# MasonMcGill/multipath-nn

Hardware: AMD Instinct MI355X
Metric: images/sec training CIFAR-10 actor-net (higher is better)
Workload: dtype f32; 1 GPU; cifar10-ac: ac_chain(k_cpt=0) 8-block actor-routed chain, 32x32x3, 10 classes; global_batch=128, per_gpu_batch=128, parallelism=dp1, rccl_ranks=1, hip_graph=True, steps_per_graph=4, streams=1, clock_warmup_steps=96

## Files before the change

include/mpnn_hip.h:

```cpp
#ifndef MPNN_HIP_H
#define MPNN_HIP_H

#ifdef __cplusplus
extern "C" {
#endif

#define MPNN_MAX_NODES 128
#define MPNN_MAX_SINKS 4

#define MPNN_E_SHAPE   (-1)
#define MPNN_E_ARG     (-2)

#define MPNN_BN_SLOTS 16

#define MPNN_ACT_IDENTITY 0
#define MPNN_ACT_BN_BATCH 1
#define MPNN_ACT_BN_MOVING 2
#define MPNN_ACT_RELU 3

typedef struct {
    const float  *x;
    const double *sum;
    const float  *gamma, *beta, *m_avg, *v_avg;
    float eps;
    int   cnt;
    int   C;
    int   shift;
    int   mode;
    int   nslot;
} mpnn_act;

int mpnn_bn_relu_fwd(const mpnn_act *a, float *y, long n_pix, void *stream);

int mpnn_pack_weights(const float *params, float *packs, const int *desc,
                      int n_desc, void *stream);

int mpnn_step_begin(const float *params, float *packs, const int *desc, int n_desc,
                    void *zero, long zero_bytes, void *stream);

typedef struct {
    mpnn_act a;
    const float *v;  int Cv;
    const float *wa_pack;  const float *wv_pack;
    const float *bias;
    float  *out;
    float  *pool_out;
    double *out_sum;
    int out_nslot;
    int n, H, W, Cout;
    const int *idx;
    const int *cnt;
} mpnn_conv_fwd_args;
int mpnn_msconv_fwd(const mpnn_conv_fwd_args *args, void *stream);
int mpnn_msconv_fwd_group(const mpnn_conv_fwd_args *args, const mpnn_conv_fwd_args *dev_args, int count,
                          void *stream);
int mpnn_msconv_fwd_group_rep(const mpnn_conv_fwd_args *args, const mpnn_conv_fwd_args *dev_args, int count,
                              int reps, int share, void *stream);

typedef struct {
    const float *s;
    mpnn_act bn;
    const double *red;
    int red_nslot;
} mpnn_bn_ctx;
int mpnn_bn_bwd_reduce(const float *dy, const mpnn_bn_ctx *ctx, float *dz,
                       double *red_out, long n_pix, void *stream);
int mpnn_bn_bwd_apply(float *dz_inout, const mpnn_bn_ctx *ctx, long n_pix,
                      void *stream);

typedef struct {
    const float *g;  int Cg;
    const mpnn_bn_ctx *g_ctx;
    const float *w_pack;
    const float *dy_extra;
    const mpnn_bn_ctx *prev;
    float  *out;
    double *red_out;
    int n, H, W, Cout;
    int accumulate;
} mpnn_dgrad_horz_args;
int mpnn_msconv_dgrad_horz(const mpnn_dgrad_horz_args *args, void *stream);

typedef struct {
    const float *g;  int Cg;
    const mpnn_bn_ctx *g_ctx;
    const float *w_pack;
    const mpnn_bn_ctx *fine;
    int fine_has_dz;
    float *dz_g_fine;
    int n, H, W, Cout;
} mpnn_dgrad_vert_args;
int mpnn_msconv_dgrad_vert(const mpnn_dgrad_vert_args *args, void *stream);
int mpnn_msconv_dgrad_pair(const mpnn_dgrad_horz_args *horz, const mpnn_dgrad_vert_args *vert,
                           void *stream);

typedef struct {
    mpnn_act a;
    const float *v;  int Cv;
    const float *g;
    const mpnn_bn_ctx *g_ctx;
    float *dwa;  float *dwv;  float *db;
    long split_stride;
    int n, H, W, Cout;
    int n_split;
} mpnn_wgrad_args;
int mpnn_msconv_wgrad(const mpnn_wgrad_args *args, void *stream);
int mpnn_msconv_bwd_scale(const mpnn_dgrad_horz_args *horz, const mpnn_dgrad_vert_args *vert,
                          const mpnn_wgrad_args *wgrad, void *stream);
#define MPNN_BWD_LEVEL_MAX 4
typedef struct {
    const mpnn_dgrad_horz_args *horz;
    const mpnn_dgrad_vert_args *vert;
    const mpnn_wgrad_args *wgrad;
    int wg_horz, wg_vert;
} mpnn_bwd_member;
int mpnn_msconv_bwd_level_record_size(void);
int mpnn_msconv_bwd_level_slots(const int *H, const int *W, const int *Cout, int count);
int mpnn_msconv_bwd_level_prepare(const mpnn_bwd_member *members, int count, void *host_records);
int mpnn_msconv_bwd_level(const mpnn_bwd_member *members, int count, const void *dev_records, void *stream);
int mpnn_msconv_bwd_level_prepare_rep(const mpnn_bwd_member *members, int count, int reps, void *host_records);
int mpnn_msconv_bwd_level_rep(const mpnn_bwd_member *members, int count, int reps, const void *dev_records, void *stream);
int mpnn_wgrad_tiles(int n, int H, int W);
#define MPNN_SLAB_ITEM 1024
int mpnn_slab_reduce(const float *slabs, float *grads, const int *table, int n_items,
                     void *stream);

int mpnn_msconv_gen_check(int H, int W, int Cin, int Cv, int Cout, int kh, int kw, int kvh, int kvw);
int mpnn_msconv_gen_tiles(int n, int H, int W);
int mpnn_msconv_fwd_gen(const mpnn_conv_fwd_args *args, int kh, int kw, int kvh, int kvw, void *stream);
int mpnn_msconv_dgrad_horz_gen(const mpnn_dgrad_horz_args *args, int kh, int kw, void *stream);
int mpnn_msconv_dgrad_vert_gen(const mpnn_dgrad_vert_args *args, int kvh, int kvw, void *stream);
int mpnn_msconv_wgrad_gen(const mpnn_wgrad_args *args, int kh, int kw, int kvh, int kvw, void *stream);

int mpnn_msconv_hw_check(int H, int W, int Cin, int Cv, int Cout, int kh, int kw, int kvh, int kvw);
int mpnn_msconv_hw_tiles(int n, int H, int W);
int mpnn_msconv_fwd_hw(const mpnn_conv_fwd_args *args, int kh, int kw, int kvh, int kvw, void *stream);
int mpnn_msconv_dgrad_horz_hw(const mpnn_dgrad_horz_args *args, int kh, int kw, void *stream);
int mpnn_msconv_dgrad_vert_hw(const mpnn_dgrad_vert_args *args, int kvh, int kvw, void *stream);
int mpnn_msconv_wgrad_hw(const mpnn_wgrad_args *args, int kh, int kw, int kvh, int kvw, void *stream);

int mpnn_msconv_ch_check(int H, int W, int Cin, int Cv, int Cout, int kh, int kw, int kvh, int kvw);
int mpnn_msconv_fwd_ch(const mpnn_conv_fwd_args *args, int kh, int kw, int kvh, int kvw, void *stream);
int mpnn_msconv_dgrad_horz_ch(const mpnn_dgrad_horz_args *args, int kh, int kw, void *stream);
int mpnn_msconv_dgrad_vert_ch(const mpnn_dgrad_vert_args *args, int kvh, int kvw, void *stream);
int mpnn_msconv_wgrad_ch(const mpnn_wgrad_args *args, int kh, int kw, int kvh, int kvw, void *stream);

typedef struct {
    mpnn_act a;  const float *w;  const float *bias;  float *out;
    int n, H, W, Cout;  int supp;
} mpnn_conv_nhwc_fwd_args;
int mpnn_conv_nhwc_fwd(const mpnn_conv_nhwc_fwd_args *args, void *stream);
typedef struct {
    const float *g;  int Cg;  const float *w;
    const float *relu_src;
    double *scratch;
    float *dx;
    int n, H, W, Cin;  int supp;
} mpnn_conv_nhwc_dgrad_args;
int mpnn_conv_nhwc_dgrad(const mpnn_conv_nhwc_dgrad_args *args, void *stream);
typedef struct {
    mpnn_act a;  const float *g;  float *dw;  float *db;
    long split_stride;  int n_split;
    int n, H, W, Cout;  int supp;
} mpnn_conv_nhwc_wgrad_args;
int mpnn_conv_nhwc_wgrad(const mpnn_conv_nhwc_wgrad_args *args, void *stream);

typedef struct {
    mpnn_act a;  int HW;
    const float *w[2];  const float *b[2];  float *y[2];  int M[2];
    const float *k_cpt;  float alpha_cpt;  int extra_col[2];
    int n;
    float *kpart;  int *kcnt;
} mpnn_lin_fwd_args;
#define MPNN_LIN_KSLICES 8
int mpnn_lin_fwd(const mpnn_lin_fwd_args *dev_table, int count, int n_max, void *stream);
int mpnn_lin_fwd_ks(const mpnn_lin_fwd_args *dev_table, int count, int n_max, int k_max, void *stream);

typedef struct {
    mpnn_act a;  int HW;
    const float *w[2];  const float *dy[2];  int M[2];
    float *dw[2];  float *db[2];
    float *dx;
    const float *k_cpt;  float alpha_cpt;  int extra_col[2];
    int n;
    float *dz_out;  double *red_out;  int red_nslot;
    float *kpart;  int *kcnt;
} mpnn_lin_bwd_args;
#define MPNN_LIN_RSPLIT 8
#define MPNN_LIN_RS_TILE 2080
int mpnn_lin_bwd(const mpnn_lin_bwd_args *dev_table, int count, int n_max, int k_max,
                 void *stream);
int mpnn_lin_bwd_rs(const mpnn_lin_bwd_args *dev_table, int count, int n_max, int k_max,
                    void *stream);

typedef struct {
    const float *z;  const float *y;  int n_cls;  float eps_ce;
    float *c_err;  float *d_cor;
    const float *h1;  int R;  int n_sinks;
    const float *g1, *b1;  float *m1, *v1;
    const float *w2, *bias2;
    const float *g2, *b2;  float *m2, *v2;
    const float *w3, *bias3;
    float *h2;  float *r;  int r_stride;
    float *bn_save;
    float bn_eps, bn_decay;
    int mode;
    int n;
    float *clear_f;  int n_clear_f;  double *clear_d;  int n_clear_d;
    int R2;
    const float *hyp_src;  float *hyp_dst;
    float bn_eps2, bn_decay2;
} mpnn_exit_tail_args;
int mpnn_exit_tail_fwd(const mpnn_exit_tail_args *dev_table, int count, int n_max,
                       void *stream);

typedef struct {
    mpnn_exit_tail_args f;
    const float *w_cerr;
    const float *dr;
    float *dz;
    float *dh1;
    float *dg1, *db1, *dw2, *dbias2, *dg2, *db2, *dw3, *dbias3;
    float *dh2;
} mpnn_exit_tail_bwd_args;
int mpnn_exit_tail_bwd(const mpnn_exit_tail_bwd_args *dev_table, int count, int n_max,
                       void *stream);

typedef struct {
    mpnn_act a;  int HW;
    const float *w_head, *b_head;  int n_cls;
    const float *y;  float eps_ce;  float *c_err, *d_cor;
    const float *w1, *b1;  int R;  int n_sinks;
    int extra_col;  const float *k_cpt;  float alpha_cpt;
    const float *g1, *be1, *m1, *v1;  const float *w2, *bias2;
    const float *g2, *be2, *m2, *v2;  const float *w3, *bias3;
    float bn_eps;
    float *r;  int r_stride;
    const int *idx;  const int *cnt;  int n;
    int *child_idx[MPNN_MAX_SINKS];  int *child_cnt[MPNN_MAX_SINKS];
    int R2;
    float *z, *h1;
    float bn_eps2;
    int *cls;  float *conf;
    float *p_cls;  int p_stride;
} mpnn_exit_ev_args;
int mpnn_exit_ev(const mpnn_exit_ev_args *dev_table, int count, int n_max, void *stream);
int mpnn_exit_ev_check(const mpnn_exit_ev_args *host_record);

#define MPNN_PREFIX_MAX 64
typedef struct {
    int n, count, n_front, pad_;
    int parent[MPNN_PREFIX_MAX], parent_sink[MPNN_PREFIX_MAX], n_sinks[MPNN_PREFIX_MAX], r_stride[MPNN_PREFIX_MAX];
    float *r[MPNN_PREFIX_MAX];
    float *c_err[MPNN_PREFIX_MAX];
    float *d_cor[MPNN_PREFIX_MAX];
    int front_parent[MPNN_PREFIX_MAX], front_sink[MPNN_PREFIX_MAX];
    int *front_idx[MPNN_PREFIX_MAX];
    int *front_cnt[MPNN_PREFIX_MAX];
} mpnn_ev_prefix_args;
int mpnn_ev_prefix_walk(const mpnn_ev_prefix_args *host_rec, const mpnn_ev_prefix_args *dev_rec, void *stream);

typedef struct {
    int n, n_nodes, n_leaves, n_cls;
    const float *p_ev;
    const long long *node_ops;
    const int *leaf_node;
    const int *leaf_cls;  const float *leaf_conf;
    const float *leaf_p;
    int leaf_stride, p_stride;
// ... 112 lines not shown
```

multipath-nn_amd/csrc/bwd_bodies.h:

```cpp
#pragma once
#include "conv_kernel.h"

struct WgP {
    ConvP c;
    const float *g;
    const float *g_s;  mpnn_act g_bn;  const double *g_red;  int g_nslot;  int g_on;
    float *dwa, *dwv, *db;
    long split_stride;
    int n_tiles;
};

template <int GK> struct WGeom;
template <> struct WGeom<0> { static constexpr int PS = 113; };
template <> struct WGeom<1> { static constexpr int PS = 113; };
template <> struct WGeom<2> { static constexpr int PS = 145; };

template <int GK, int OT, int PART, bool SMALLC = false>
__device__ __forceinline__ void wgrad_body(const WgP &p, f32x4 *tile, float *gt, float *cA,
                                           const int bx, const int by, const int bz, const int gx) {
    static_assert(!SMALLC || (PART == 0 && OT == 1), "SMALLC: the image chunk of a 16-channel group");
    using G = Geom<GK>;
    constexpr int PS = WGeom<GK>::PS, R = G::R, HR = G::TH + 2;
    constexpr int GS = OT * 16 + 4;
    constexpr int XN = XItems<GK>::N;
    const ConvP &c = p.c;
    const int tid = threadIdx.x, lane = tid & 63;
    const int wid = __builtin_amdgcn_readfirstlane(tid >> 6);
    const int g = lane >> 4, li = lane & 15;
    const int nchA = (c.a.C + 15) >> 4;
    constexpr int part = PART;
    const int ch = part ? by - nchA : by;
    const int C = part ? c.Cv : c.a.C;
    const int co0 = bz * OT * 16;
    int np = (C - ch * 16 + 3) >> 2;
    np = np > 4 ? 4 : np;
    const bool bias_wave = wid == 1 && by == 0;
    const bool xa = c.xcd != 0 && (c.n & 31) == 0 && (gx & 7) == 0;
    const int xcd_id = blockIdx.x & 7;
    const int tpi = GK == 0 ? (c.W >> 4) * (c.H >> 2) : 1;
    const int sq0 = xa ? (bx >> 3) : bx, sqd = xa ? (gx >> 3) : gx, sqn = xa ? (p.n_tiles >> 3) : p.n_tiles;
    trace_stamp(0);

    constexpr bool NINE = OT == 1 || OT == 4;
    f32x4 acc[NINE ? 1 : 3][OT];
    f32x4 acc9[(NINE && !SMALLC) ? 9 : 1];
    [[maybe_unused]] f32x4 accS[2] = {f32x4{0.f, 0.f, 0.f, 0.f}, f32x4{0.f, 0.f, 0.f, 0.f}};
    [[maybe_unused]] int offS[2];
    [[maybe_unused]] bool onS[2];
    if constexpr (SMALLC) {
#pragma unroll
        for (int nt = 0; nt < 2; ++nt) {
            const int idx = nt * 16 + li, n9 = 9 * c.a.C;
            onS[nt] = idx < n9;
            const int ic = onS[nt] ? idx : 0, tap = ic / c.a.C, cc = ic - tap * c.a.C;
            offS[nt] = ((tap / 3) * R + (tap % 3)) * 4 + cc;
        }
    }
    float bsum = 0.f;
#pragma unroll
    for (int ti = 0; ti < (NINE ? 1 : 3); ++ti)
#pragma unroll
        for (int nt = 0; nt < OT; ++nt) acc[ti][nt] = f32x4{0.f, 0.f, 0.f, 0.f};
#pragma unroll
    for (int tap = 0; tap < ((NINE && !SMALLC) ? 9 : 1); ++tap) acc9[tap] = f32x4{0.f, 0.f, 0.f, 0.f};
    const float *tf = (const float *)tile;
    const int a_lane = (li >> 2) * PS * 4 + (li & 3);
    const float one_hot = li == 0 ? 1.f : 0.f;
    int tap_off[3];
#pragma unroll
    for (int ti = 0; ti < 3; ++ti) {
        const int tap = min(wid + 4 * ti, 8);
        tap_off[ti] = (tap / 3) * R + (tap % 3);
    }

    [[maybe_unused]] int slot9[4];
#pragma unroll
    for (int j = 0; j < 4; ++j) {
        int img, ty, tx;
        mtile_pix<GK>(wid, 4 * g + j, img, ty, tx);
        slot9[j] = (img * HR + ty) * R + tx;
    }

    if (part == 0 && c.a.mode != MPNN_ACT_IDENTITY) {
        for (int cc = tid; cc < c.a.C; cc += 256) {
            const BnC k = bn_coef(c.a, cc);
            cA[cc * 3] = k.m; cA[cc * 3 + 1] = k.gamma * k.rstd; cA[cc * 3 + 2] = k.beta;
        }
    }

    float *cG = cA + 128 * 3;
    if (p.g_on && p.g_bn.mode == MPNN_ACT_BN_BATCH) {
        for (int cc = tid - 128; cc >= 0 && cc < OT * 16; cc += 256) bn_bwd_row(p.g_bn, p.g_red, p.g_nslot, co0 + cc, false, cG + cc * 5);
    } else if (p.g_on) {
        const double inv = 1.0 / (double)p.g_bn.cnt;
        for (int cc = tid - 128; cc >= 0 && cc < OT * 16; cc += 256) {
            const int co = co0 + cc;
            const BnC k = bn_coef(p.g_bn, co);
            float *e = cG + cc * 5;
            e[0] = k.m; e[1] = k.rstd; e[2] = k.gamma * k.rstd;
            double r0, r1;
            slot_sum2(p.g_red, 2 * c.Cout, co, c.Cout + co, p.g_nslot, r0, r1);
            e[3] = (float)(r0 * inv); e[4] = (float)(r1 * inv);
        }
    }

    if constexpr (XItems<GK>::INTERIOR) zero_halo(tile, 4 * PS, tid, 256);
    __syncthreads();
    trace_stamp(1);
    f32x4 xr[XN][1], gr[OT], gs[OT];
    int on0;
    unsigned inbS;
    ItemK<GK> ik;
    item_consts<GK, PS>(ik, tid);
    int g_geo[OT], g_lds[OT], g_c4[OT];
#pragma unroll
    for (int k = 0; k < OT; ++k) {
        const int i = tid + k * 256;
        const int q = i % (OT * 4), pi = i / (OT * 4);
        int img, ty, tx;
        mtile_pix<GK>(pi >> 4, pi & 15, img, ty, tx);
        g_geo[k] = (img << 16) | (ty << 8) | tx;
        g_lds[k] = pi * GS + q * 4;
        g_c4[k] = q * 4;
    }
    const int xc = ch * 16 + ik.q * 4;
    const bool xq_in = ik.q < np;
    const int sh = PART == 0 ? c.a.shift : 0;
    const int xC = PART == 0 ? c.a.C : c.Cv;
    const float *const xsrc = PART == 0 ? c.a.x : c.v;
    auto request = [&](int t) {
        int n0, y0, x0;
        tile_origin<GK>(c, xa ? xcd_tile<GK>(t, xcd_id, tpi) : t, n0, y0, x0);
        on0 = n0;
        unsigned inb = 0;
#pragma unroll
        for (int k = 0; k < XN; ++k) {
            const int n = n0 + (ik.geo[k] >> 16), y = y0 + ((ik.geo[k] >> 8) & 255) - 1, x = x0 + (ik.geo[k] & 255) - 1;
            const bool ok = ((ik.ok >> k) & 1) && xq_in && n < c.n &&
                            (XItems<GK>::INTERIOR || ((unsigned)y < (unsigned)c.H && (unsigned)x < (unsigned)c.W));
            inb |= (ok ? 1u : 0u) << k;
            const unsigned pix = ok ? (((unsigned)n * (c.H << sh) + (y << sh)) * (c.W << sh) + (x << sh)) * xC : 0u;
            if (PART == 1 || (xC & 3) == 0) {
                xr[k][0] = *(const f32x4 *)((const char *)xsrc + (pix + (ok ? xc : 0)) * 4u);
            } else {
#pragma unroll
                for (int j = 0; j < 4; ++j) xr[k][0][j] = xsrc[pix + (ok && xc + j < xC ? xc + j : 0)];
            }
        }
        inbS = inb;
#pragma unroll
        for (int k = 0; k < OT; ++k) {
            const int n = n0 + (g_geo[k] >> 16);
            const bool live = n < c.n;
            const unsigned off = live ? (((unsigned)n * c.H + y0 + ((g_geo[k] >> 8) & 255)) * c.W + x0 + (g_geo[k] & 255)) * c.Cout + co0 + g_c4[k] : 0u;
            gr[k] = *(const f32x4 *)((const char *)p.g + off * 4u);
            if (p.g_on) gs[k] = *(const f32x4 *)((const char *)p.g_s + off * 4u);
        }
    };
    auto tile_step = [&](int t) {
        const int o_n0 = on0;
        const unsigned inb = inbS;
        lds_barrier();
#pragma unroll
        for (int k = 0; k < XN; ++k) {
            const bool live = (inb >> k) & 1;
            f32x4 v = xr[k][0];
            if (PART == 0) {
                if (c.a.mode != MPNN_ACT_IDENTITY) {
#pragma unroll
                    for (int j = 0; j < 4; ++j) {
                        const float *cc = cA + (xc + j) * 3;
                        const float tv = fmaxf((v[j] - cc[0]) * cc[1] + cc[2], 0.f);
                        v[j] = (xc + j < xC) ? tv : 0.f;
                    }
                } else if (xC & 3) {
#pragma unroll
                    for (int j = 0; j < 4; ++j) v[j] = (xc + j < xC) ? v[j] : 0.f;
                }
            }
#pragma unroll
            for (int j = 0; j < 4; ++j) v[j] = live ? v[j] : 0.f;
            if ((ik.ok >> k) & 1) tile[ik.slot[k]] = v;
        }
#pragma unroll
        for (int k = 0; k < OT; ++k) {
            f32x4 v = {0.f, 0.f, 0.f, 0.f};
            if (o_n0 + (g_geo[k] >> 16) < c.n) {
                v = gr[k];
                if (p.g_on) {
#pragma unroll
// ... 2 lines not shown
                        const float xh = (gs[k][j] - e[0]) * e[1];
                        v[j] = e[2] * (v[j] - e[3] - xh * e[4]);
                    }
                }
            }
            *(f32x4 *)(gt + g_lds[k]) = v;
        }
        lds_barrier();
        if (t == sq0) trace_stamp(2);
        if (t + sqd < sqn) request(t + sqd);
        if constexpr (SMALLC) {
            float gq[4], xq[4][2];
#pragma unroll
            for (int j = 0; j < 4; ++j) {
                gq[j] = gt[(wid * 16 + 4 * g + j) * GS + li];
#pragma unroll
                for (int nt = 0; nt < 2; ++nt) xq[j][nt] = tf[slot9[j] * 4 + offS[nt]];
            }
#pragma unroll
            for (int j = 0; j < 4; ++j) {
                bsum += gq[j];
#pragma unroll
                for (int nt = 0; nt < 2; ++nt)
                    accS[nt] = __builtin_amdgcn_mfma_f32_16x16x4f32(gq[j], onS[nt] ? xq[j][nt] : 0.f, accS[nt], 0, 0, 0);
            }
        } else
        if constexpr (NINE) {
#pragma unroll
            for (int kk = 0; kk < (OT == 4 ? 4 : 1); ++kk) {
                const int kc = OT == 4 ? kk : wid;
                float bq[4], aq[4][9];
                if constexpr (OT == 4) {
#pragma unroll
                    for (int j = 0; j < 4; ++j) {
                        int img, ty, tx;
                        mtile_pix<GK>(kk, 4 * g + j, img, ty, tx);
                        const int slot = (img * HR + ty) * R + tx;
                        bq[j] = gt[(kk * 16 + 4 * g + j) * GS + wid * 16 + li];
#pragma unroll
                        for (int tap = 0; tap < 9; ++tap) aq[j][tap] = tf[(slot + (tap / 3) * R + (tap % 3)) * 4 + a_lane];
                    }
                } else {
#pragma unroll
                    for (int j = 0; j < 4; ++j) {
                        bq[j] = gt[(kc * 16 + 4 * g + j) * GS + li];
#pragma unroll
                        for (int tap = 0; tap < 9; ++tap) aq[j][tap] = tf[(slot9[j] + (tap / 3) * R + (tap % 3)) * 4 + a_lane];
                    }
                }
#pragma unroll
                for (int j = 0; j < 4; ++j) {
                    bsum += bq[j];
#pragma unroll
                    for (int tap = 0; tap < 9; ++tap)
                        acc9[tap] = __builtin_amdgcn_mfma_f32_16x16x4f32(aq[j][tap], bq[j], acc9[tap], 0, 0, 0);
                }
            }
        } else {
#pragma unroll
        for (int kc = 0; kc < 4; ++kc) {
            float bq[4][OT], aq[4][3];
#pragma unroll
            for (int j = 0; j < 4; ++j) {
                int img, ty, tx;
                mtile_pix<GK>(kc, 4 * g + j, img, ty, tx);
                const int slot = (img * HR + ty) * R + tx;
#pragma unroll
                for (int nt = 0; nt < OT; ++nt) bq[j][nt] = gt[(kc * 16 + 4 * g + j) * GS + nt * 16 + li];
#pragma unroll
                for (int ti = 0; ti < 3; ++ti) aq[j][ti] = tf[(slot + tap_off[ti]) * 4 + a_lane];
                if (bias_wave) aq[j][2] = one_hot;
            }
#pragma unroll
            for (int j = 0; j < 4; ++j)
#pragma unroll
                for (int ti = 0; ti < 3; ++ti)
#pragma unroll
                    for (int nt = 0; nt < OT; ++nt)
                        acc[ti][nt] = __builtin_amdgcn_mfma_f32_16x16x4f32(aq[j][ti], bq[j][nt], acc[ti][nt], 0, 0, 0);
        }
        }
    };
    if (sq0 < sqn) request(sq0);
    for (int t = sq0; t < sqn; t += sqd) tile_step(t);

    trace_stamp(4);
    mfma_drain();
    const size_t soff = (size_t)bx * p.split_stride;
    float *dw = (part ? p.dwv : p.dwa) + soff;
    if constexpr (NINE && OT == 4) {
#pragma unroll
        for (int tap = 0; tap < 9; ++tap)
#pragma unroll
            for (int r = 0; r < 4; ++r) {
                const int cin = ch * 16 + g * 4 + r;
                if (cin < C) dw[((size_t)tap * C + cin) * c.Cout + co0 + wid * 16 + li] = acc9[tap][r];
            }
        if (by == 0) {
            float b = bsum;
            b += __shfl_xor(b, 16);
            b += __shfl_xor(b, 32);
            if (g == 0) p.db[soff + co0 + wid * 16 + li] = b;
        }
    } else if constexpr (SMALLC) {
        f32x4 *part4 = tile;
        float *partf = (float *)tile;
        lds_barrier();
#pragma unroll
        for (int nt = 0; nt < 2; ++nt) part4[(wid * 2 + nt) * 64 + lane] = accS[nt];
        lds_barrier();
        {
            const int r = wid, n9 = 9 * C;
#pragma unroll
            for (int nt = 0; nt < 2; ++nt) {
                float v = 0.f;
#pragma unroll
                for (int w = 0; w < 4; ++w) v += partf[((w * 2 + nt) * 64 + lane) * 4 + r];
                const int idx = nt * 16 + li, co = 4 * g + r;
                if (idx < n9) dw[(size_t)idx * c.Cout + co0 + co] = v;
            }
        }
        if (by == 0) {
            float b = bsum;
            b += __shfl_xor(b, 16);
            b += __shfl_xor(b, 32);
            lds_barrier();
            if (g == 0) partf[wid * 16 + li] = b;
            lds_barrier();
            if (tid < 16) p.db[soff + co0 + tid] = (partf[tid] + partf[16 + tid]) + (partf[32 + tid] + partf[48 + tid]);
        }
    } else if constexpr (NINE) {
        f32x4 *part4 = tile;
        float *partf = (float *)tile;
        const int cl = (tid >> 4) & 15, tl = tid >> 8;
        (void)tl;
#pragma unroll
        for (int rd = 0; rd < 3; ++rd) {
            lds_barrier();
#pragma unroll
            for (int q = 0; q < 3; ++q) part4[(wid * 3 + q) * 64 + lane] = acc9[rd * 3 + q];
            lds_barrier();
            const int cin = ch * 16 + cl;
#pragma unroll
            for (int q = 0; q < 3; ++q) {
                float v = 0.f;
#pragma unroll
                for (int w = 0; w < 4; ++w) v += partf[((w * 3 + q) * 64 + (cl >> 2) * 16 + li) * 4 + (cl & 3)];
                if (cin < C) dw[((size_t)(rd * 3 + q) * C + cin) * c.Cout + co0 + li] = v;
            }
        }
        if (by == 0) {
            float b = bsum;
            b += __shfl_xor(b, 16);
            b += __shfl_xor(b, 32);
            lds_barrier();
            if (g == 0) partf[wid * 16 + li] = b;
            lds_barrier();
            if (tid < 16) p.db[soff + co0 + tid] = (partf[tid] + partf[16 + tid]) + (partf[32 + tid] + partf[48 + tid]);
        }
    } else {
#pragma unroll
    for (int ti = 0; ti < 3; ++ti) {
        const int tap = wid + 4 * ti;
        if (tap >= 9) continue;
#pragma unroll
        for (int r = 0; r < 4; ++r) {
// ... 25 lines not shown
```

multipath-nn_amd/csrc/common.h:

```cpp
#pragma once
#include <hip/hip_runtime.h>
#include <cstdlib>
#include "mpnn_hip.h"

typedef float f32x4 __attribute__((ext_vector_type(4)));

constexpr int MPNN_OCC = 4;

#define MPNN_LAUNCH_CHECK() do { hipError_t e_ = hipGetLastError(); \
    if (e_ != hipSuccess) return (int)e_; } while (0)

extern int mpnn_reserved_cus_g;

static int resident_slots(const void *kernel, int dyn_lds, int threads = 256, int max_per_cu = 0) {
    struct Entry { const void *fn; int lds, per_cu, cus, cap; };
    static Entry cache[64];
    static int n_cached = 0;
    int per_cu = 0, cus = 256;
    bool hit = false;
    for (int i = 0; i < n_cached && !hit; ++i)
        if (cache[i].fn == kernel && cache[i].lds == dyn_lds && cache[i].cap == max_per_cu) {
            per_cu = cache[i].per_cu; cus = cache[i].cus; hit = true;
        }
    if (!hit) {
// ... 3 lines not shown
        hipFuncAttributes fa;
        if (hipFuncGetAttributes(&fa, kernel) == hipSuccess) {
            const size_t lds = fa.sharedSizeBytes + (size_t)dyn_lds;
            if (lds > 0) {
                const int by_lds = (int)((160u * 1024u) / ((lds + 1279) / 1280 * 1280));
                if (by_lds >= 1 && by_lds < per_cu) per_cu = by_lds;
            }
        }
        if (hipGetDevice(&dev) == hipSuccess) {
            int v = 0;
            if (hipDeviceGetAttribute(&v, hipDeviceAttributeMultiprocessorCount, dev) == hipSuccess && v > 0) cus = v;
        }
        if (max_per_cu > 0 && per_cu > max_per_cu) per_cu = max_per_cu;
        if (n_cached < 64) cache[n_cached++] = Entry{kernel, dyn_lds, per_cu, cus, max_per_cu};
    }
    const int free_cus = cus - mpnn_reserved_cus_g;
    return per_cu * (free_cus < 8 ? 8 : free_cus);
}

#define MPNN_TRACE_SLOTS 12
#ifdef MPNN_TRACE
static __device__ unsigned long long *mpnn_trace_buf_ = nullptr;
__device__ __forceinline__ void trace_stamp(int k) {
    unsigned long long *b = mpnn_trace_buf_;
    if (b && threadIdx.x == 0)
        b[(size_t)((blockIdx.z * gridDim.y + blockIdx.y) * gridDim.x + blockIdx.x) * MPNN_TRACE_SLOTS + k] = __builtin_amdgcn_s_memrealtime();
}
__device__ __forceinline__ void trace_note(int k, unsigned long long v) {
    unsigned long long *b = mpnn_trace_buf_;
    if (b && threadIdx.x == 0) b[(size_t)((blockIdx.z * gridDim.y + blockIdx.y) * gridDim.x + blockIdx.x) * MPNN_TRACE_SLOTS + k] = v;
}
static inline int mpnn_trace_install(void *buf) {
    return (int)hipMemcpyToSymbol(HIP_SYMBOL(mpnn_trace_buf_), &buf, sizeof(buf));
}
#else
__device__ __forceinline__ void trace_stamp(int) {}
__device__ __forceinline__ void trace_note(int, unsigned long long) {}
static inline int mpnn_trace_install(void *) { return MPNN_E_ARG; }
#endif

struct BnC { float m, rstd, gamma, beta; };

__device__ __forceinline__ double ld_slot(const double *base, int C2, int s, unsigned off) {
    const char *row = (const char *)(base + (size_t)s * C2);
    return *(const double *)(row + off);
}
__device__ __forceinline__ void slot_sum2(const double *base, int C2, int i0, int i1, int nslot, double &a, double &b) {
    double t0 = 0.0, t1 = 0.0;
    const unsigned o0 = (unsigned)i0 * 8u, o1 = (unsigned)i1 * 8u;
#pragma unroll 8
    for (int s = 0; s < nslot; ++s) { t0 += ld_slot(base, C2, s, o0); t1 += ld_slot(base, C2, s, o1); }
    a = t0; b = t1;
}
__device__ __forceinline__ double slot_sum(const double *base, int C2, int idx, int nslot) {
    double t = 0.0;
    const unsigned o = (unsigned)idx * 8u;
#pragma unroll 8
    for (int s = 0; s < nslot; ++s) t += ld_slot(base, C2, s, o);
    return t;
}

__device__ __forceinline__ BnC bn_coef(const mpnn_act &b, int c) {
    BnC k;
    k.gamma = b.mode == MPNN_ACT_RELU ? 1.f : b.gamma[c];
    k.beta = b.mode == MPNN_ACT_RELU ? 0.f : b.beta[c];
    if (b.mode == MPNN_ACT_BN_BATCH) {
        const double inv = 1.0 / (double)b.cnt;
        double s1, s2;
        slot_sum2(b.sum, 2 * b.C, c, b.C + c, b.nslot, s1, s2);
        const double mean = s1 * inv;
        double var = s2 * inv - mean * mean;
        var = var < 0.0 ? 0.0 : var;
        k.m = (float)mean;
        k.rstd = rsqrtf((float)var + b.eps);
    } else if (b.mode == MPNN_ACT_RELU) {
        k.m = 0.f;  k.rstd = 1.f;  k.gamma = 1.f;  k.beta = 0.f;
    } else {
        k.m = b.m_avg[c];
        k.rstd = rsqrtf(b.v_avg[c] + b.eps);
    }
    return k;
}

__device__ __forceinline__ void bn_bwd_row(const mpnn_act &b, const double *red, int red_nslot, int c, bool want_beta, float *e) {
    const int C2 = 2 * b.C, ns = b.nslot, rn = red ? red_nslot : 0;
    const float gamma = b.gamma[c], beta = b.beta[c];
    const unsigned o0 = (unsigned)c * 8u, o1 = (unsigned)(b.C + c) * 8u;
    double s1 = 0.0, s2 = 0.0, r0 = 0.0, r1 = 0.0;
    if (ns == 8 && (rn == 8 || rn == 0)) {
        double a0[8], a1[8], q0[8], q1[8];
#pragma unroll
        for (int s = 0; s < 8; ++s) { a0[s] = ld_slot(b.sum, C2, s, o0); a1[s] = ld_slot(b.sum, C2, s, o1); }
        if (rn) {
#pragma unroll
            for (int s = 0; s < 8; ++s) { q0[s] = ld_slot(red, C2, s, o0); q1[s] = ld_slot(red, C2, s, o1); }
        } else {
#pragma unroll
            for (int s = 0; s < 8; ++s) { q0[s] = 0.0; q1[s] = 0.0; }
        }
#pragma unroll
        for (int s = 0; s < 8; ++s) { s1 += a0[s]; s2 += a1[s]; }
        if (rn) {
#pragma unroll
            for (int s = 0; s < 8; ++s) { r0 += q0[s]; r1 += q1[s]; }
        }
    } else {
        slot_sum2(b.sum, C2, c, b.C + c, ns, s1, s2);
        if (rn) slot_sum2(red, C2, c, b.C + c, rn, r0, r1);
    }
    const double inv = 1.0 / (double)b.cnt;
    const double mean = s1 * inv;
    double var = s2 * inv - mean * mean;
    var = var < 0.0 ? 0.0 : var;
    const float rstd = rsqrtf((float)var + b.eps);
    e[0] = (float)mean; e[1] = rstd; e[2] = gamma * rstd;
    if (want_beta) { e[3] = beta; e[4] = 0.f; }
    else { e[3] = (float)(r0 * inv); e[4] = (float)(r1 * inv); }
}

struct BnNoHook { __device__ __forceinline__ void operator()(int, float, int, float) const {} };
template <class F = BnNoHook>
__device__ __forceinline__ void bn_finalize_body(double *__restrict__ sums, double *__restrict__ reds,
                                                 float *__restrict__ state, float *__restrict__ grads,
                                                 const int *__restrict__ t, float decay, int n_img,
                                                 double *__restrict__ sums_keep, F on_grad = F()) {
    const int C = t[3], ns = t[7];
    const double inv = 1.0 / ((double)t[4] * (double)n_img);
    for (int c = threadIdx.x; c < C; c += blockDim.x) {
        const double mean = slot_sum(sums + t[0], 2 * C, c, ns) * inv;
        double var = slot_sum(sums + t[0], 2 * C, C + c, ns) * inv - mean * mean;
        var = var < 0.0 ? 0.0 : var;
        if (t[5] >= 0) {
            float *m = state + t[1] + c, *v = state + t[2] + c;
            *m = decay * *m + (1.f - decay) * (float)mean;
            *v = decay * *v + (1.f - decay) * (float)var;
        }
        if (reds && grads && t[5] >= 0) {
            const float dbeta = (float)slot_sum(reds + t[0], 2 * C, c, ns);
            const float dgamma = (float)slot_sum(reds + t[0], 2 * C, C + c, ns);
            grads[t[6] + c] = dbeta;
            grads[t[5] + c] = dgamma;
            on_grad(t[6] + c, dbeta, t[5] + c, dgamma);
        }
        if (!sums_keep) continue;
        for (int s = 0; s < ns; ++s) {
            const int i0 = t[0] + s * 2 * C + c, i1 = i0 + C;
            sums_keep[i0] = sums[i0];  sums_keep[i1] = sums[i1];
            sums[i0] = 0.0;  sums[i1] = 0.0;
            if (reds) { reds[i0] = 0.0;  reds[i1] = 0.0; }
        }
    }
}

__device__ __forceinline__ void lds_barrier() {
    asm volatile("" ::: "memory");
    __builtin_amdgcn_s_waitcnt(0xC07F);
    __builtin_amdgcn_s_barrier();
    asm volatile("" ::: "memory");
}

__device__ __forceinline__ void mfma_drain() {
    __builtin_amdgcn_sched_barrier(0);
    asm volatile("s_nop 15" ::: "memory");
    __builtin_amdgcn_sched_barrier(0);
}

// ... 49 lines not shown
```

multipath-nn_amd/csrc/conv_dgrad.hip:

```cpp
#include "conv_kernel.h"

static int fill_g_ctx(const mpnn_bn_ctx *c, ConvP &p) {
    if (!c) return 0;
    if (!c->s || !c->red) return MPNN_E_ARG;
    p.ga_on = 1;  p.ga_s = c->s;  p.ga_bn = c->bn;  p.ga_red = c->red;
    p.ga_nslot = c->red_nslot < 1 ? 1 : c->red_nslot;
    return 0;
}

int mpnn_fill_dgrad_horz(const mpnn_dgrad_horz_args *a, ConvP &p) {
    if (!a || !a->g || !a->w_pack || !a->out) return MPNN_E_ARG;
    p.a.x = a->g;  p.a.C = a->Cg;  p.a.mode = MPNN_ACT_IDENTITY;  p.a.shift = 0;
    p.wa = a->w_pack;
    p.n = a->n;  p.H = a->H;  p.W = a->W;  p.Cout = a->Cout;
    p.extra = a->dy_extra;  p.out = a->out;  p.acc_out = a->accumulate ? 1 : 0;
    if (a->prev) {
        if (!a->prev->s || !a->red_out) return MPNN_E_ARG;
        p.sprev = a->prev->s;  p.pbn = a->prev->bn;  p.red_out = a->red_out;
        p.out_nslot = a->prev->red_nslot < 1 ? 1 : a->prev->red_nslot;
    }
    return fill_g_ctx(a->g_ctx, p);
}

int mpnn_fill_dgrad_vert(const mpnn_dgrad_vert_args *a, ConvP &p) {
    if (!a || !a->g || !a->w_pack || !a->fine || !a->fine->s || !a->dz_g_fine) return MPNN_E_ARG;
    p.a.x = a->g;  p.a.C = a->Cg;  p.a.mode = MPNN_ACT_IDENTITY;  p.a.shift = 0;
    p.wa = a->w_pack;
    p.n = a->n;  p.H = a->H;  p.W = a->W;  p.Cout = a->Cout;
    p.out = a->dz_g_fine;  p.sprev = a->fine->s;  p.pbn = a->fine->bn;
    p.red = a->fine_has_dz ? a->fine->red : nullptr;  p.has_dz = a->fine_has_dz;
    p.red_nslot = a->fine->red_nslot < 1 ? 1 : a->fine->red_nslot;
    return fill_g_ctx(a->g_ctx, p);
}

int mpnn_trace_install_dgrad(void *buf) { return mpnn_trace_install(buf); }

extern "C" int mpnn_msconv_dgrad_pair(const mpnn_dgrad_horz_args *h, const mpnn_dgrad_vert_args *v, void *stream) {
    ConvP ph = {}, pv = {};
    int rc = mpnn_fill_dgrad_horz(h, ph);
    if (rc) return rc;
    rc = mpnn_fill_dgrad_vert(v, pv);
    if (rc) return rc;
    if (!h->prev) return MPNN_E_ARG;
    return conv_launch_pair<EPI_DGH_BN, EPI_DGV>(ph, pv, (hipStream_t)stream);
}

extern "C" int mpnn_msconv_dgrad_horz(const mpnn_dgrad_horz_args *a, void *stream) {
    ConvP p = {};
    const int rc = mpnn_fill_dgrad_horz(a, p);
    if (rc) return rc;
    if (a->prev) return conv_launch<EPI_DGH_BN>(p, (hipStream_t)stream);
    return conv_launch<EPI_DGH_RAW>(p, (hipStream_t)stream);
}

extern "C" int mpnn_msconv_dgrad_vert(const mpnn_dgrad_vert_args *a, void *stream) {
    ConvP p = {};
    const int rc = mpnn_fill_dgrad_vert(a, p);
    if (rc) return rc;
    return conv_launch<EPI_DGV>(p, (hipStream_t)stream);
}
```

multipath-nn_amd/csrc/conv_fwd.hip:

```cpp
#include "conv_kernel.h"
#include "conv_strip.h"

__host__ __device__ static inline int fill_fwd(const mpnn_conv_fwd_args *a, ConvP &p);

int mpnn_trace_install_fwd(void *buf) { return mpnn_trace_install(buf); }

extern "C" int mpnn_msconv_fwd(const mpnn_conv_fwd_args *a, void *stream) {
    ConvP p = {};
    const int rc = fill_fwd(a, p);
    if (rc) return rc;
    if (a->idx || a->cnt) return MPNN_E_ARG;
    return conv_launch<EPI_FWD>(p, (hipStream_t)stream);
}

struct FwdGroupP { int gk[4], small[4], gy[4], gx[4], y0[4], w0[4], rh[4]; int n; int xcd; int reps, wpr; };

__host__ __device__ static inline int fill_fwd(const mpnn_conv_fwd_args *a, ConvP &p) {
    if (!a || !a->a.x || !a->wa_pack || !a->out || !a->bias) return MPNN_E_ARG;
    if (a->v && !a->wv_pack) return MPNN_E_ARG;
    p.a = a->a;
    p.v = a->v;  p.Cv = a->v ? a->Cv : 0;
    p.wa = a->wa_pack;  p.wv = a->wv_pack;
    p.n = a->n;  p.H = a->H;  p.W = a->W;  p.Cout = a->Cout;
    p.bias = a->bias;  p.out = a->out;  p.out_sum = a->out_sum;  p.pool_out = a->pool_out;
    p.out_nslot = a->out_nslot < 1 ? 1 : (a->out_nslot > MPNN_BN_SLOTS ? MPNN_BN_SLOTS : a->out_nslot);
    if (a->pool_out && (a->H < 8 || (a->H & 1) || (a->W & 1))) return MPNN_E_SHAPE;
    p.idx = a->idx;
    if (a->idx && !a->cnt) return MPNN_E_ARG;
#if defined(__HIP_DEVICE_COMPILE__)
    if (a->cnt) { const int c = *a->cnt; p.n = c < a->n ? c : a->n; }
#endif
    return 0;
}

template <bool SMALL, bool IDX, bool WIDE = false>
__global__ __launch_bounds__(256, WIDE ? 2 : (SMALL ? 3 : MPNN_OCC)) void fwd_group_k(const mpnn_conv_fwd_args *__restrict__ tab, const FwdGroupP q) {
    extern __shared__ __attribute__((aligned(16))) char smem[];
    int id = blockIdx.x;
    if (q.reps > 1) { const int rep = id / q.wpr; id -= rep * q.wpr; tab += rep * q.n; }
    int m = 0, w0 = 0, gx = q.gx[0], kind = q.gk[0] * 2 + q.small[0];
#pragma unroll
    for (int k = 1; k < 4; ++k)
        if (k < q.n && id >= q.w0[k]) { m = k; w0 = q.w0[k]; gx = q.gx[k]; kind = q.gk[k] * 2 + q.small[k]; }
    const int yy = (id - w0) / gx, bx = (id - w0) - yy * gx;
    ConvP p = {};
    fill_fwd(tab + m, p);
    p.xcd = q.xcd;
    if constexpr (WIDE) {
        if (kind == 2) { p.n_tiles = conv_grid_x<1>(p.n, p.H, p.W); conv_body<1, 2, 1, 2, 2, false, EPI_FWD, 1, false, IDX>(p, bx, yy, gx, smem); }
        else           { p.n_tiles = conv_grid_x<2>(p.n, p.H, p.W); conv_body<2, 2, 1, 2, 2, false, EPI_FWD, 1, false, IDX>(p, bx, yy, gx, smem); }
        return;
    }
    switch (kind) {
        case 0: p.n_tiles = conv_grid_x<0>(p.n, p.H, p.W); conv_body<0, 1, 1, 4, 1, false, EPI_FWD, 1, false, IDX>(p, bx, yy, gx, smem); break;
        case 2: p.n_tiles = conv_grid_x<1>(p.n, p.H, p.W); conv_body<1, 1, 1, 4, 1, false, EPI_FWD, 1, false, IDX>(p, bx, yy, gx, smem); break;
        case 4: p.n_tiles = conv_grid_x<2>(p.n, p.H, p.W); conv_body<2, 1, 1, 4, 1, false, EPI_FWD, 1, false, IDX>(p, bx, yy, gx, smem); break;
        case 6: strip16_body<IDX>(tab[m], bx, yy, gx, q.rh[m], q.xcd, smem); break;
        case 8: stripk_body<IDX>(tab[m], bx, yy, gx, q.rh[m], q.xcd, smem); break;
        default:
            if constexpr (SMALL) {
                if (kind == 9)      stripk_body<IDX, true>(tab[m], bx, yy, gx, q.rh[m], q.xcd, smem);
                else if (kind == 1) { p.n_tiles = conv_grid_x<0>(p.n, p.H, p.W); conv_body<0, 1, 1, 4, 1, true, EPI_FWD, 1, false, IDX>(p, bx, yy, gx, smem); }
                else if (kind == 3) { p.n_tiles = conv_grid_x<1>(p.n, p.H, p.W); conv_body<1, 1, 1, 4, 1, true, EPI_FWD, 1, false, IDX>(p, bx, yy, gx, smem); }
                else                { p.n_tiles = conv_grid_x<2>(p.n, p.H, p.W); conv_body<2, 1, 1, 4, 1, true, EPI_FWD, 1, false, IDX>(p, bx, yy, gx, smem); }
            }
            break;
    }
}

template <int GK, int KS = 2>
__global__ __launch_bounds__(KS * 256) void fwd_ks_k(const mpnn_conv_fwd_args *__restrict__ tab, const int gx, const int xcd) {
    extern __shared__ __attribute__((aligned(16))) char smem[];
    const int id = blockIdx.x, yy = id / gx, bx = id - yy * gx;
    ConvP p = {};
    fill_fwd(tab, p);
    p.xcd = xcd;
    p.n_tiles = conv_grid_x<GK>(p.n, p.H, p.W);
    conv_body<GK, 1, 1, 4, 1, false, EPI_FWD, KS, true>(p, bx, yy, gx, smem);
}

int mpnn_first_conv_launch_rep(const mpnn_conv_fwd_args *a, const mpnn_conv_fwd_args *dev_args, int reps, int share, hipStream_t st);

static int fwd_group_launch(const mpnn_conv_fwd_args *args, const mpnn_conv_fwd_args *dev_args, int count, int reps, int share, void *stream);

extern "C" int mpnn_msconv_fwd_group(const mpnn_conv_fwd_args *args, const mpnn_conv_fwd_args *dev_args, int count,
                                     void *stream) {
    return fwd_group_launch(args, dev_args, count, 1, 1, stream);
}

extern "C" int mpnn_msconv_fwd_group_rep(const mpnn_conv_fwd_args *args, const mpnn_conv_fwd_args *dev_args, int count,
                                         int reps, int share, void *stream) {
    if (reps < 1) return MPNN_E_ARG;
    if (share <= 0) share = reps;
    if (count <= 0) return 0;
    if (!args || count > 4) return MPNN_E_ARG;
    for (int k = 0; k < count; ++k)
        if (args[k].idx || args[k].cnt) return MPNN_E_ARG;
    for (int r = 1; r < reps; ++r)
        for (int k = 0; k < count; ++k) {
            const mpnn_conv_fwd_args &a = args[k], &b = args[r * count + k];
            if (a.n != b.n || a.H != b.H || a.W != b.W || a.Cout != b.Cout || a.a.C != b.a.C || a.a.mode != b.a.mode ||
                a.a.shift != b.a.shift || (a.v != nullptr) != (b.v != nullptr) || a.Cv != b.Cv || a.out_nslot != b.out_nslot ||
                (a.pool_out != nullptr) != (b.pool_out != nullptr) || (a.out_sum != nullptr) != (b.out_sum != nullptr) ||
                a.idx || b.idx || a.cnt || b.cnt) return MPNN_E_ARG;
        }
    return fwd_group_launch(args, dev_args, count, reps, share, stream);
}

static int fwd_group_launch(const mpnn_conv_fwd_args *args, const mpnn_conv_fwd_args *dev_args, int count, int reps, int share, void *stream) {
    if (count <= 0) return 0;
// ... 109 lines not shown
```

multipath-nn_amd/csrc/conv_kernel.h:

```cpp
#pragma once
#include "common.h"
#include <cstdlib>

enum { EPI_FWD = 0, EPI_DGH_BN = 1, EPI_DGH_RAW = 2, EPI_DGV = 3 };

#ifdef MPNN_ABLATE
#define MPNN_DBG(p, bit) ((p).dbg & (bit))
#else
#define MPNN_DBG(p, bit) 0
#endif

struct ConvP {
    mpnn_act a;
    const float *v;  int Cv;
    const float *wa, *wv;
    int n, H, W, Cout;
    const float *bias;  float *out;  double *out_sum;
    float *pool_out;
    const float *extra;
    const float *sprev;  mpnn_act pbn;  double *red_out;
    const double *red;  int has_dz;  int red_nslot;
    int out_nslot;
    const float *ga_s;  mpnn_act ga_bn;  const double *ga_red;  int ga_nslot;  int ga_on;
    int n_tiles;
    int dbg;
    const int *idx;
    int acc_out;
    int xcd;
};

template <int GK>
__device__ __forceinline__ int xcd_tile(int j, int x, int tpi) {
    if (GK == 2) return 8 * j + x;
    const int ij = GK == 0 ? j / tpi : j, inner = GK == 0 ? j - ij * tpi : 0;
    const int n = ((ij >> 2) << 5) + 4 * x + (ij & 3);
    return n * tpi + inner;
}

template <int GK> struct Geom;
template <> struct Geom<0> { static constexpr int TH = 4, TW = 16, IMG = 1, R = 18, P = 112; };
template <> struct Geom<1> { static constexpr int TH = 8, TW = 8,  IMG = 1, R = 10, P = 112; };
template <> struct Geom<2> { static constexpr int TH = 4, TW = 4,  IMG = 4, R = 6,  P = 144; };

template <int GK>
__device__ __forceinline__ void mtile_pix(int m, int i, int &img, int &ty, int &tx) {
    if (GK == 0) { img = 0; ty = m; tx = i; }
    else if (GK == 1) { img = 0; ty = 2 * m + (i >> 3); tx = i & 7; }
    else { img = m; ty = i >> 2; tx = i & 3; }
}

template <int GK>
__device__ __forceinline__ void tile_origin(const ConvP &p, int bid, int &n0, int &y0, int &x0) {
    if (GK == 0) {
        const int tx_n = p.W >> 4, tpi = tx_n * (p.H >> 2);
        n0 = bid / tpi;
        const int rem = bid - n0 * tpi;
        const int ty = rem / tx_n;
        y0 = ty * 4; x0 = (rem - ty * tx_n) * 16;
    } else if (GK == 1) { n0 = bid; y0 = 0; x0 = 0; }
    else { n0 = bid * 4; y0 = 0; x0 = 0; }
}

template <int GK>
__host__ __device__ static inline int conv_grid_x(int n, int H, int W) {
    if (GK == 0) return n * (W >> 4) * (H >> 2);
    if (GK == 1) return n;
    return (n + 3) >> 2;
}

template <int GK> struct XItems {
    using G = Geom<GK>;
    static constexpr bool INTERIOR = GK != 0;
    static constexpr int HR = G::TH + 2, HC = G::TW + 2;
    static constexpr int NHP = INTERIOR ? G::IMG * G::TH * G::TW : G::IMG * HR * HC, NHP8 = (NHP + 7) & ~7;
    static constexpr int N = (NHP8 * 4 + 255) / 256;
};
__device__ __forceinline__ void zero_halo(f32x4 *lds, int count, int tid, int nthreads) {
    for (int i = tid; i < count; i += nthreads) lds[i] = f32x4{0.f, 0.f, 0.f, 0.f};
}
template <int GK, int PS>
__device__ __forceinline__ void zero_ring(f32x4 *lds, int planes, int tid, int nthreads) {
    using G = Geom<GK>;
    constexpr int HR = G::TH + 2, FR = G::IMG * HR * G::R;
    for (int i = tid; i < planes * PS; i += nthreads) {
        const int t = i % PS;
        bool ring = t >= FR;
        if (!ring) {
            const int r = t % (HR * G::R), hy = r / G::R, hx = r - hy * G::R;
            ring = hy == 0 || hy == HR - 1 || hx == 0 || hx > G::TW;
        }
        if (ring) lds[i] = f32x4{0.f, 0.f, 0.f, 0.f};
    }
}

__device__ __forceinline__ int sel_i(int flag, int a, int b) { const int m = -flag; return (a & ~m) | (b & m); }
__device__ __forceinline__ const float *sel_p(int flag, const float *a, const float *b) {
    const long delta = (const char *)b - (const char *)a;
    return (const float *)((const char *)a + (delta & -(long)flag));
}
template <int GK> struct ItemK {
    static constexpr int N = XItems<GK>::N;
    int slot[N];
    int geo[N];
    unsigned ok;
    int q;
};
template <int GK, int PS>
__device__ __forceinline__ void item_consts(ItemK<GK> &ik, int tid) {
    using X = XItems<GK>;
    using G = Geom<GK>;
    ik.ok = 0;
// ... 208 lines not shown
        r.np = (C - r.ch * 16 + 3) >> 2;
    };
    auto gen_tile = [&](UI &r, int t) {
        r.t = t; r.part = 0; r.ch = 0;
        tile_origin<GK>(p, xa ? xcd_tile<GK>(t, xcd_id, tpi) : t, r.n0, r.y0, r.x0);
        if constexpr (IDX) {
#pragma unroll
            for (int j = 0; j < G::IMG; ++j) r.im[j] = p.idx[r.n0 + j < p.n ? r.n0 + j : 0];
            tile_geo<GK, SMALL_A>(tgeo, ik, p, r.n0, r.y0, r.x0, r.im, aC, vC);
        } else
        tile_geo<GK, SMALL_A>(tgeo, ik, p, r.n0, r.y0, r.x0, nullptr, aC, vC);
        r.inb = tgeo.inb;
        set_np(r);
    };
    auto gen_next = [&](UI &r) {
        r.ch += NCH;
        if (r.ch >= (HAS_V ? sel_i(r.part, nchA, nchV) : nchA)) {
            if (HAS_V && !r.part && nchV) { r.part = 1; r.ch = 0; }
            else { gen_tile(r, r.t + sqd); return; }
        }
        set_np(r);
    };
    const bool b_once = upt == 1;
    constexpr int LK = EPI != EPI_FWD ? 2 : (SMALL_A ? 1 : 0);
    auto unit_load = [&](const UI &q, f32x4 (*xq)[XW], f32x4 *bq) {
        const float *src = HAS_V ? sel_p(q.part, aX, vX) : aX, *wp = HAS_V ? sel_p(q.part, wAp, wVp) : wAp;
        const int C = HAS_V ? sel_i(q.part, aC, vC) : aC;
#pragma unroll
        for (int sc = 0; sc < SC; ++sc) {
            const int cs = KSPLIT ? kg : sc;
            ld_items<GK, LK, XW, SMALL_A>(xq + sc * XN, p, tgeo, ik, q.part, (q.ch + cs) * 16, q.np - 4 * cs, src, C, odd_c);
        }
#pragma unroll
        for (int sc = 0; sc < SC; ++sc) {
            const int cs = KSPLIT ? kg : sc;
            const char *wb = (const char *)wp + (size_t)((q.ch + cs) * 16 * p.Cout) * 4;
#pragma unroll
            for (int k = 0; k < BN; ++k) bq[sc * BN + k] = *(const f32x4 *)(wb + ((HAS_V && q.part) ? wofV[k] : wofA[k]));
        }
    };
    auto unit_store = [&](const UI &q, f32x4 (*xq)[XW], f32x4 *bq, int buf, bool with_b) {
#pragma unroll
        for (int sc = 0; sc < SC; ++sc) {
            const int cs = KSPLIT ? kg : sc;
            f32x4 *td = tile[buf] + cs * 4 * P;
            f32x4 (*xs)[XW] = xq + sc * XN;
            const int c0 = (q.ch + cs) * 16, np = q.np - 4 * cs;
            bool done = false;
            if constexpr (EPI == EPI_FWD) {
                if (q.part) { done = true; st_items<GK, 1, XW>(td, xs, p, cA, q.inb, ik, c0, np); }
            }
            if constexpr (EPI != EPI_FWD) {
                if (p.ga_on) { done = true; st_items<GK, 2, XW>(td, xs, p, cA, q.inb, ik, c0, np); }
            }
            if (!done) st_items<GK, 0, XW>(td, xs, p, cA, q.inb, ik, c0, np);
        }
        if (with_b) {
            f32x4 *dst = wtile[(b_once || WtSingle<CT>::v) ? 0 : buf];
#pragma unroll
            for (int sc = 0; sc < SC; ++sc)
#pragma unroll
                for (int k = 0; k < BN; ++k) { const int i = tid + k * 256; if (i < BI) dst[(KSPLIT ? kg : sc) * BI + i] = bq[sc * BN + k]; }
        }
    };

    f32x4 xrA[SC * XN][XW], xrB[SC * XN][XW];
    f32x4 brA[SC * BN], brB[SC * BN];
    f32x4 acc[MT][NT];
    float s1[NT], s2[NT];
#pragma unroll
    for (int nt = 0; nt < NT; ++nt) { s1[nt] = 0.f; s2[nt] = 0.f; }
#pragma unroll
    for (int mt = 0; mt < MT; ++mt)
#pragma unroll
        for (int nt = 0; nt < NT; ++nt) acc[mt][nt] = f32x4{0.f, 0.f, 0.f, 0.f};

    UI cu = {}, n1 = {}, n2 = {};
    constexpr int TABQ = 8;
    [[maybe_unused]] double tabq[TABQ];
    [[maybe_unused]] float tab_g = 1.f, tab_b = 0.f;
    bool tab_late = false;
    if constexpr (EPI == EPI_FWD) {
        const int tot = p.a.nslot * 2 * p.a.C;
        tab_late = p.a.mode == MPNN_ACT_BN_BATCH && tot <= TABQ * 256 && p.a.C <= 256;
        if (tab_late) {
#pragma unroll
            for (int j = 0; j < TABQ; ++j) { const int k = tid + 256 * j; tabq[j] = p.a.sum[k < tot ? k : 0]; }
            const int c = tid < p.a.C ? tid : 0;
            tab_g = p.a.gamma[c]; tab_b = p.a.beta[c];
        }
    }
    if (EPI == EPI_FWD && p.a.mode != MPNN_ACT_IDENTITY && !tab_late) {
        for (int c = tid; c < p.a.C; c += 256) {
            const BnC k = bn_coef(p.a, c);
            cA[c * 3] = k.m; cA[c * 3 + 1] = k.gamma * k.rstd; cA[c * 3 + 2] = k.beta;
        }
    }
    if (EPI != EPI_FWD && p.ga_on) {
        if (p.ga_bn.mode == MPNN_ACT_BN_BATCH) {
            for (int c = tid; c < p.a.C; c += 256) bn_bwd_row(p.ga_bn, p.ga_red, p.ga_nslot, c, false, cA + c * 5);
        } else {
            const double inv = 1.0 / (double)p.ga_bn.cnt;
            for (int c = tid; c < p.a.C; c += 256) {
                const BnC k = bn_coef(p.ga_bn, c);
                float *e = cA + c * 5;
                e[0] = k.m; e[1] = k.rstd; e[2] = k.gamma * k.rstd;
                double r0, r1;
                slot_sum2(p.ga_red, 2 * p.a.C, c, p.a.C + c, p.ga_nslot, r0, r1);
                e[3] = (float)(r0 * inv); e[4] = (float)(r1 * inv);
            }
        }
    }
    if (EPI == EPI_DGH_BN || EPI == EPI_DGV) {
        for (int c = tid - 128; c >= 0 && c < CT; c += 256) {
            float *e = cE + c * 5;
            if (p.pbn.mode == MPNN_ACT_BN_BATCH) {
                bn_bwd_row(p.pbn, EPI == EPI_DGV ? p.red : nullptr, p.red_nslot, co0 + c, EPI == EPI_DGH_BN, e);
                continue;
            }
            const BnC k = bn_coef(p.pbn, co0 + c);
            e[0] = k.m; e[1] = k.rstd; e[2] = k.gamma * k.rstd;
            if (EPI == EPI_DGH_BN) { e[3] = k.beta; e[4] = 0.f; }
            else {
                const double inv = 1.0 / (double)p.pbn.cnt;
                double r0 = 0.0, r1 = 0.0;
                if (p.red) slot_sum2(p.red, 2 * p.pbn.C, co0 + c, p.pbn.C + co0 + c, p.red_nslot, r0, r1);
                e[3] = (float)(r0 * inv); e[4] = (float)(r1 * inv);
            }
        }
    }
    if (!tab_late) __syncthreads();
    trace_stamp(1);
    gen_tile(gen, sq0);
    cu = gen;
    unit_load(cu, xrA, brA);
    if (n_units > 1) {
        gen_next(gen);
        n1 = gen;
        unit_load(n1, xrB, brB);
    }
    if constexpr (EPI == EPI_FWD) {
        if (tab_late) {
            double *scr = (double *)smem;
            const int C = p.a.C, tot = p.a.nslot * 2 * C;
#pragma unroll
            for (int j = 0; j < TABQ; ++j) { const int k = tid + 256 * j; if (k < tot) scr[k] = tabq[j]; }
            __syncthreads();
            if (tid < C) {
                double s1 = 0.0, s2 = 0.0;
                for (int sl = 0; sl < p.a.nslot; ++sl) { s1 += scr[(2 * sl) * C + tid]; s2 += scr[(2 * sl + 1) * C + tid]; }
                const double inv = 1.0 / (double)p.a.cnt, mean = s1 * inv;
                double var = s2 * inv - mean * mean;
                var = var < 0.0 ? 0.0 : var;
                cA[tid * 3] = (float)mean; cA[tid * 3 + 1] = tab_g * rsqrtf((float)var + p.a.eps); cA[tid * 3 + 2] = tab_b;
            }
            __syncthreads();
        }
    }
    if constexpr (XItems<GK>::INTERIOR)
        zero_ring<GK, P>(&tile[0][0], 2 * NCH * 4, threadIdx.x, KSPLIT ? NCH * 256 : 256);
    if (n_units > 0) unit_store(cu, xrA, brA, 0, true);
    __syncthreads();
    trace_stamp(2);

    auto step = [&](const int u, f32x4 (*xn1)[XW], f32x4 *bn1, f32x4 (*xn2)[XW], f32x4 *bn2) {
        const f32x4 *cur = tile[u & 1];
        const bool more = u + 1 < n_units, more2 = u + 2 < n_units;
        const int part = cu.part, t = cu.t, n0 = cu.n0, y0 = cu.y0, x0 = cu.x0;
        const int t2 = n1.t;
        if (more2) {
            gen_next(gen);
            n2 = gen;
            unit_load(n2, xn2, bn2);
        }
        [[maybe_unused]] float e_sv[MT][4][NT][4], e_dz[MT][4][NT][4];
        if constexpr (EPI == EPI_DGV) {
            if ((!more || t2 != t) && !MPNN_DBG(p, 4)) {
#pragma unroll
                for (int mt = 0; mt < MT; ++mt)
#pragma unroll
                    for (int r = 0; r < 4; ++r) {
                        int img, ty, tx;
                        mtile_pix<GK>(wm * MT + mt, g * 4 + r, img, ty, tx);
                        const int n = n0 + img < p.n ? n0 + img : 0, y = y0 + ty, x = x0 + tx;
                        const int W2 = p.W * 2;
#pragma unroll
                        for (int nt = 0; nt < NT; ++nt) {
                            const unsigned i00 = (((unsigned)n * (p.H * 2) + 2 * y) * W2 + 2 * x) * p.Cout + cw + nt * 16;
                            const unsigned ix[4] = {i00, i00 + p.Cout, i00 + (unsigned)W2 * p.Cout, i00 + (unsigned)W2 * p.Cout + p.Cout};
#pragma unroll
                            for (int k = 0; k < 4; ++k) {
                                e_sv[mt][r][nt][k] = p.sprev[ix[k]];
                                e_dz[mt][r][nt][k] = p.has_dz ? p.out[ix[k]] : 0.f;
                            }
                        }
                    }
            }
        }
        [[maybe_unused]] float h_sp[MT][4][NT], h_ex[MT][4][NT];
        if constexpr (EPI == EPI_DGH_BN) {
            if ((!more || t2 != t) && !MPNN_DBG(p, 4)) {
#pragma unroll
                for (int mt = 0; mt < MT; ++mt)
#pragma unroll
                    for (int r = 0; r < 4; ++r) {
                        int img, ty, tx;
                        mtile_pix<GK>(wm * MT + mt, g * 4 + r, img, ty, tx);
                        const int n = n0 + img < p.n ? n0 + img : 0, y = y0 + ty, x = x0 + tx;
#pragma unroll
                        for (int nt = 0; nt < NT; ++nt) {
                            const unsigned idx = (((unsigned)n * p.H + y) * p.W + x) * p.Cout + cw + nt * 16;
                            h_sp[mt][r][nt] = p.sprev[idx];
                            h_ex[mt][r][nt] = p.extra ? p.extra[idx] : 0.f;
                        }
                    }
            }
        }
        if (!MPNN_DBG(p, 1)) {
            const f32x4 *wl = (b_once || WtSingle<CT>::v) ? wtile[0] : wtile[u & 1];
            const int wcol = wn * NT * 16 + li;
            if (SMALL_A && part == 0) {
                const float *tf = (const float *)cur;
                const float *wf = (const float *)wl;
#pragma unroll
                for (int tap = 0; tap < 9; ++tap) {
                    const int dy = tap / 3, dx = tap - dy * 3;
                    float b[NT], a[MT];
#pragma unroll
                    for (int nt = 0; nt < NT; ++nt) b[nt] = wf[((tap * 4) * CT + wcol + nt * 16) * 4 + g];
#pragma unroll
                    for (int mt = 0; mt < MT; ++mt) a[mt] = tf[(slot0[mt] + dy * R + dx) * 4 + g];
#pragma unroll
                    for (int mt = 0; mt < MT; ++mt)
#pragma unroll
                        for (int nt = 0; nt < NT; ++nt)
                            acc[mt][nt] = __builtin_amdgcn_mfma_f32_16x16x4f32(a[mt], b[nt], acc[mt][nt], 0, 0, 0);
                }
            } else {
                f32x4 fa[2][MT], fb[2][NT];
// ... 245 lines not shown
```

multipath-nn_amd/csrc/conv_strip.h:

```cpp
#pragma once
#include "conv_kernel.h"

struct StripSeq { int ij, ys, xs; };

template <bool IDX>
__device__ __forceinline__ void strip16_body(const mpnn_conv_fwd_args &a, const int bx, const int by, const int gx, const int rh,
                                             const int xcd, char *smem) {
    const int tid = threadIdx.x, lane = tid & 63;
    const int wid = __builtin_amdgcn_readfirstlane(tid >> 6);
    const int li = lane & 15, g = lane >> 4;
    const int H = a.H, W = a.W, Co = a.Cout, co0 = by * 16;
    int n_img = a.n;
    if (a.cnt) { const int c = *a.cnt; n_img = c < a.n ? c : a.n; }
    const int xs_n = W >> 4, ys_n = H / rh, tpi = xs_n * ys_n;

    float *cS = (float *)smem;
    const int mode = a.a.mode;
    if (mode != MPNN_ACT_IDENTITY) {
        if (tid < 16) {
            const BnC k = bn_coef(a.a, tid);
            cS[tid * 3] = k.m; cS[tid * 3 + 1] = k.gamma * k.rstd; cS[tid * 3 + 2] = k.beta;
        }
        __syncthreads();
    }
    float cm[4], cs[4], cb[4];
#pragma unroll
    for (int j = 0; j < 4; ++j) {
        cm[j] = mode != MPNN_ACT_IDENTITY ? cS[(4 * g + j) * 3] : 0.f;
        cs[j] = mode != MPNN_ACT_IDENTITY ? cS[(4 * g + j) * 3 + 1] : 1.f;
        cb[j] = mode != MPNN_ACT_IDENTITY ? cS[(4 * g + j) * 3 + 2] : 0.f;
    }
    f32x4 wr[9];
#pragma unroll
    for (int t = 0; t < 9; ++t) wr[t] = *(const f32x4 *)(a.wa_pack + t * 16 * Co + (g * Co + co0 + li) * 4);
    const f32x4 bias4 = *(const f32x4 *)(a.bias + co0 + g * 4);

    const bool xa = xcd != 0 && (a.n & 31) == 0 && (gx & 7) == 0 && !IDX;
    const int xcd_id = blockIdx.x & 7;
    const int jw = xa ? (bx >> 3) * 4 + wid : bx * 4 + wid;
    const int nw = xa ? (gx >> 3) * 4 : gx * 4;
    const int jn = (xa ? (a.n >> 3) : n_img) * tpi;
    auto image = [&](int ij) { return xa ? ((ij >> 2) << 5) + 4 * xcd_id + (ij & 3) : ij; };

    const long row_b = (long)W * 64;
    const int off1 = (li * 16 + g * 4) * 4;
    [[maybe_unused]] float s1[4] = {0.f, 0.f, 0.f, 0.f}, s2[4] = {0.f, 0.f, 0.f, 0.f};
    const bool stats = a.out_sum != nullptr, pool = a.pool_out != nullptr;

    for (int j = jw; j < jn; j += nw) {
        const int ij = j / tpi, rem = j - ij * tpi, ys = rem / xs_n, xs = rem - ys * xs_n;
        const int slot = image(ij);
        const int n = IDX ? a.idx[slot] : slot;
        const int y0 = ys * rh, x0 = xs * 16;
        const bool left = x0 == 0, right = x0 + 16 == W;
        const bool zl = left && li == 0, zr = right && li == 15;
        const int o0 = off1 - 64 + (64 & -(int)zl), o2 = off1 + 64 - (64 & -(int)zr);
        const char *xin = (const char *)a.a.x + (((long)n * H) * W + x0) * 64;
        float *outp = a.out + (((long)n * H) * W + x0 + li) * Co + co0 + g * 4;
        float *poolp = pool ? a.pool_out + (((long)n * (H >> 1)) * (W >> 1) + (x0 >> 1) + (li >> 1)) * Co + co0 + g * 4 : nullptr;

        auto load_row = [&](int y, f32x4 *r) {
            const char *rp = xin + ((unsigned)y < (unsigned)H ? y : 0) * row_b;
            r[0] = *(const f32x4 *)(rp + o0);
            r[1] = *(const f32x4 *)(rp + off1);
            r[2] = *(const f32x4 *)(rp + o2);
        };
        auto prep_row = [&](int y, f32x4 *r) {
            const bool rz = (unsigned)y >= (unsigned)H;
#pragma unroll
            for (int dx = 0; dx < 3; ++dx) {
                const bool z = rz || (dx == 0 && zl) || (dx == 2 && zr);
#pragma unroll
                for (int c = 0; c < 4; ++c) {
                    float v = r[dx][c];
                    if (mode != MPNN_ACT_IDENTITY) v = fmaxf((v - cm[c]) * cs[c] + cb[c], 0.f);
                    r[dx][c] = z ? 0.f : v;
                }
            }
        };
        auto mac3 = [&](f32x4 &up, f32x4 &mid, f32x4 &dn, const f32x4 *r, bool on_up, bool on_mid, bool on_dn) {
#pragma unroll
            for (int dx = 0; dx < 3; ++dx)
#pragma unroll
                for (int c = 0; c < 4; ++c) {
                    if (on_up) up = __builtin_amdgcn_mfma_f32_16x16x4f32(wr[6 + dx][c], r[dx][c], up, 0, 0, 0);
                    if (on_mid) mid = __builtin_amdgcn_mfma_f32_16x16x4f32(wr[3 + dx][c], r[dx][c], mid, 0, 0, 0);
                    if (on_dn) dn = __builtin_amdgcn_mfma_f32_16x16x4f32(wr[dx][c], r[dx][c], dn, 0, 0, 0);
                }
        };
        f32x4 prev_out = {0.f, 0.f, 0.f, 0.f};
        auto finish = [&](f32x4 acc, int y) {
            acc += bias4;
            *(f32x4 *)(outp + (long)y * W * Co) = acc;
            if (stats) {
#pragma unroll
                for (int c = 0; c < 4; ++c) { s1[c] += acc[c]; s2[c] += acc[c] * acc[c]; }
            }
            if (pool) {
                if (y & 1) {
                    f32x4 m;
#pragma unroll
                    for (int c = 0; c < 4; ++c) {
                        const float q = fmaxf(prev_out[c], acc[c]);
                        const float o = __builtin_bit_cast(float, dpp_i<MPNN_DPP_QUAD_XOR1>(__builtin_bit_cast(int, q)));
                        m[c] = fmaxf(q, o);
                    }
                    *(f32x4 *)(poolp + (long)(y >> 1) * (W >> 1) * Co) = m;
                }
                prev_out = acc;
            }
        };

        f32x4 ra[3], rb[3];
        f32x4 A0 = {0.f, 0.f, 0.f, 0.f}, A1 = A0, A2 = A0;
        load_row(y0 - 1, ra);
        auto step = [&](int i, f32x4 *cur, f32x4 *nxt, f32x4 &Adn, f32x4 &Amid, f32x4 &Aup) {
            const int y = y0 - 1 + i;
            if (i + 1 <= rh + 1) load_row(y + 1, nxt);
            prep_row(y, cur);
            const bool on_up = i >= 2, on_mid = i >= 1 && i <= rh, on_dn = i <= rh - 1;
            if (on_dn) Adn = f32x4{0.f, 0.f, 0.f, 0.f};
            if (on_up && on_mid && on_dn) mac3(Aup, Amid, Adn, cur, true, true, true);
            else mac3(Aup, Amid, Adn, cur, on_up, on_mid, on_dn);
            if (on_up) { mfma_drain(); finish(Aup, y0 + i - 2); }
        };
        for (int i = 0; i <= rh + 1; i += 6) {
            step(i, ra, rb, A0, A2, A1);
            if (i + 1 <= rh + 1) step(i + 1, rb, ra, A1, A0, A2);
            if (i + 2 <= rh + 1) step(i + 2, ra, rb, A2, A1, A0);
            if (i + 3 <= rh + 1) step(i + 3, rb, ra, A0, A2, A1);
            if (i + 4 <= rh + 1) step(i + 4, ra, rb, A1, A0, A2);
            if (i + 5 <= rh + 1) step(i + 5, rb, ra, A2, A1, A0);
        }
    }

    if (a.out_sum) {
        double *red = (double *)(smem + 256);
#pragma unroll
        for (int c = 0; c < 4; ++c) {
            double a1 = (double)s1[c], a2 = (double)s2[c];
#pragma unroll
            for (int m = 1; m < 16; m <<= 1) { a1 += __shfl_xor(a1, m); a2 += __shfl_xor(a2, m); }
            if (li == 0) { red[(wid * 16 + g * 4 + c) * 2] = a1; red[(wid * 16 + g * 4 + c) * 2 + 1] = a2; }
        }
        __syncthreads();
        if (tid < 16) {
            double a1 = 0.0, a2 = 0.0;
#pragma unroll
            for (int w = 0; w < 4; ++w) { a1 += red[(w * 16 + tid) * 2]; a2 += red[(w * 16 + tid) * 2 + 1]; }
            const int nslot = a.out_nslot < 1 ? 1 : (a.out_nslot > MPNN_BN_SLOTS ? MPNN_BN_SLOTS : a.out_nslot);
            double *slot = a.out_sum + (size_t)(bx % nslot) * 2 * Co;
            atomicAdd(slot + co0 + tid, a1);
            atomicAdd(slot + Co + co0 + tid, a2);
        }
    }
}

#define MPNN_STRIP_KMAX 3
static inline int strip_lds_bytes(int K) { return 2048 + 1024 + K * 9 * 64 * 16; }

template <bool IDX, bool SMA = false>
__device__ __forceinline__ void stripk_body(const mpnn_conv_fwd_args &a, const int bx, const int by, const int gx, const int rh,
                                            const int xcd, char *smem) {
    const int tid = threadIdx.x, lane = tid & 63;
    const int wid = __builtin_amdgcn_readfirstlane(tid >> 6);
    const int li = lane & 15, g = lane >> 4;
    const int H = a.H, W = a.W, Co = a.Cout, co0 = by * 16;
    const int Ca = a.a.C, Cv = a.v ? a.Cv : 0, KA = SMA ? 1 : Ca >> 4, KV = Cv >> 4, K = KA + KV;
    const int sh = SMA ? a.a.shift : 0;
    int n_img = a.n;
    if (a.cnt) { const int c = *a.cnt; n_img = c < a.n ? c : a.n; }
    const int xs_n = W >> 4, ys_n = H / rh, tpi = xs_n * ys_n;

    double *red = (double *)smem;
    float *cS = (float *)(smem + 2048);
    f32x4 *wl = (f32x4 *)(smem + 2048 + 1024);
    const int mode = a.a.mode;
    if (!SMA && mode != MPNN_ACT_IDENTITY && tid < Ca) {
        const BnC k = bn_coef(a.a, tid);
        cS[tid] = k.m; cS[Ca + tid] = k.gamma * k.rstd; cS[2 * Ca + tid] = k.beta;
    }
    for (int f = tid; f < K * 9 * 64; f += 256) {
        const int l = f & 63, ft = f >> 6, kq = ft / 9, t = ft - kq * 9, fl = l & 15, fg = l >> 4;
        const bool isv = kq >= KA;
        const float *pk = isv ? a.wv_pack : a.wa_pack;
        const int nch = isv ? KV : KA, kk = isv ? kq - KA : kq;
        if (SMA && !isv) {
            const float w = fg < Ca ? pk[(size_t)t * 16 * Co + (co0 + fl) * 4 + fg] : 0.f;
            wl[f] = f32x4{w, 0.f, 0.f, 0.f};
            continue;
        }
        wl[f] = *(const f32x4 *)(pk + (size_t)t * nch * 16 * Co + ((kk * 4 + fg) * Co + co0 + fl) * 4);
    }
    __syncthreads();
    const f32x4 bias4 = *(const f32x4 *)(a.bias + co0 + g * 4);

    const bool xa = xcd != 0 && (a.n & 31) == 0 && (gx & 7) == 0 && !IDX;
    const int xcd_id = blockIdx.x & 7;
    const int jw = xa ? (bx >> 3) * 4 + wid : bx * 4 + wid;
    const int nw = xa ? (gx >> 3) * 4 : gx * 4;
    const int jn = (xa ? (a.n >> 3) : n_img) * tpi;
    auto image = [&](int ij) { return xa ? ((ij >> 2) << 5) + 4 * xcd_id + (ij & 3) : ij; };
    [[maybe_unused]] float s1[4] = {0.f, 0.f, 0.f, 0.f}, s2[4] = {0.f, 0.f, 0.f, 0.f};
    const bool stats = a.out_sum != nullptr, pool = a.pool_out != nullptr;

    for (int j = jw; j < jn; j += nw) {
        const int ij = j / tpi, rem = j - ij * tpi, ys = rem / xs_n, xs = rem - ys * xs_n;
        const int slot = image(ij);
        const int n = IDX ? a.idx[slot] : slot;
        const int y0 = ys * rh, x0 = xs * 16;
        const bool zl = x0 == 0 && li == 0, zr = x0 + 16 == W && li == 15;
        const int pl = li - 1 + (int)zl, pr = li + 1 - (int)zr;
        const long img_px = ((long)n * H) * W + x0;
        float *outp = a.out + (img_px + li) * Co + co0 + g * 4;
        float *poolp = pool ? a.pool_out + (((long)n * (H >> 1)) * (W >> 1) + (x0 >> 1) + (li >> 1)) * Co + co0 + g * 4 : nullptr;

        auto load_unit = [&](int y, int kq, f32x4 *r) {
            const bool isv = kq >= KA;
            if (SMA && !isv) {
                const int yy = (unsigned)y < (unsigned)H ? y : 0, gc = g < Ca ? g : Ca - 1;
                const float *rp = a.a.x + ((((long)n * (H << sh) + ((long)yy << sh)) * (W << sh)) + ((long)x0 << sh)) * Ca + gc;
                r[0] = f32x4{rp[(long)(pl << sh) * Ca], 0.f, 0.f, 0.f};
                r[1] = f32x4{rp[(long)(li << sh) * Ca], 0.f, 0.f, 0.f};
                r[2] = f32x4{rp[(long)(pr << sh) * Ca], 0.f, 0.f, 0.f};
                return;
            }
            const float *src = isv ? a.v : a.a.x;
            const int C = isv ? Cv : Ca, ch = (isv ? kq - KA : kq) * 16 + g * 4;
            const float *rp = src + (img_px + (long)((unsigned)y < (unsigned)H ? y : 0) * W) * C + ch;
            r[0] = *(const f32x4 *)(rp + pl * C);
            r[1] = *(const f32x4 *)(rp + li * C);
            r[2] = *(const f32x4 *)(rp + pr * C);
        };
        auto prep_unit = [&](int y, int kq, f32x4 *r) {
            const bool rz = (unsigned)y >= (unsigned)H;
            const bool bn = !SMA && kq < KA && mode != MPNN_ACT_IDENTITY;
            f32x4 cm = {0.f, 0.f, 0.f, 0.f}, cs = cm, cb = cm;
            if (bn) {
                const int c = kq * 16 + g * 4;
                cm = *(const f32x4 *)(cS + c); cs = *(const f32x4 *)(cS + Ca + c); cb = *(const f32x4 *)(cS + 2 * Ca + c);
            }
#pragma unroll
            for (int dx = 0; dx < 3; ++dx) {
                const bool z = rz || (dx == 0 && zl) || (dx == 2 && zr);
#pragma unroll
                for (int c = 0; c < 4; ++c) {
                    float v = r[dx][c];
                    if (bn) v = fmaxf((v - cm[c]) * cs[c] + cb[c], 0.f);
                    r[dx][c] = z ? 0.f : v;
                }
            }
        };
        auto mac3 = [&](f32x4 &up, f32x4 &mid, f32x4 &dn, const f32x4 *r, int kq, bool on_up, bool on_mid, bool on_dn) {
            const f32x4 *wk = wl + kq * 9 * 64 + lane;
#pragma unroll
            for (int dx = 0; dx < 3; ++dx) {
                const f32x4 w0 = wk[dx * 64], w1 = wk[(3 + dx) * 64], w2 = wk[(6 + dx) * 64];
                auto kstep = [&](int c) {
                    if (on_up) up = __builtin_amdgcn_mfma_f32_16x16x4f32(w2[c], r[dx][c], up, 0, 0, 0);
                    if (on_mid) mid = __builtin_amdgcn_mfma_f32_16x16x4f32(w1[c], r[dx][c], mid, 0, 0, 0);
                    if (on_dn) dn = __builtin_amdgcn_mfma_f32_16x16x4f32(w0[c], r[dx][c], dn, 0, 0, 0);
                };
                kstep(0);
// ... 73 lines not shown
```

multipath-nn_amd/csrc/lin.hip:

```cpp
#include "common.h"

template <int LFW, bool SLICED>
__global__ __launch_bounds__(LFW * 64) void lin_fwd_k(const mpnn_lin_fwd_args *__restrict__ tab, const int n_rec) {
    const mpnn_lin_fwd_args a = tab[SLICED ? blockIdx.y % n_rec : blockIdx.y];
    const int n0 = blockIdx.x * 16;
    if (n0 >= a.n) return;
    const int slice = SLICED ? blockIdx.y / n_rec : 0;
    const int S = (SLICED && a.kpart && a.kcnt) ? min(MPNN_LIN_KSLICES, max(1, (a.HW * a.a.C) >> 8)) : 1;
    if (slice >= S) return;
    trace_stamp(0); trace_note(6, 10);
    constexpr int NT_ = LFW * 64, NO = 512 / (NT_ < 512 ? NT_ : 512);
    __shared__ float cA[128 * 3];
    __shared__ float red[LFW * 2 * 256];
    const int tid = threadIdx.x, lane = tid & 63, g = lane >> 4, li = lane & 15;
    const int wid = __builtin_amdgcn_readfirstlane(tid >> 6);
    const int C = a.a.C, K = a.HW * C;
    const bool bn = a.a.mode != MPNN_ACT_IDENTITY;
    if (bn) {
        for (int c = tid; c < C; c += NT_) {
            const BnC k = bn_coef(a.a, c);
            cA[c * 3] = k.m; cA[c * 3 + 1] = k.gamma * k.rstd; cA[c * 3 + 2] = k.beta;
        }
    }
    __syncthreads();
    trace_stamp(1);
    const int row = n0 + li;
    const bool valid = row < a.n;
    const int M0 = a.w[0] ? a.M[0] : 0, M1 = a.w[1] ? a.M[1] : 0;
    float ep_bias[NO], ep_extra[NO];
    bool ep_on[NO];
    int ep_row[NO], ep_col[NO], ep_M[NO], ep_s[NO];
#pragma unroll
    for (int q = 0; q < NO; ++q) {
        const int o = tid + q * NT_;
        const int e = o & 255, l = e >> 2, r = e & 3;
        ep_bias[q] = 0.f; ep_extra[q] = 0.f;
        ep_s[q] = (o >> 8) & 1;
        ep_M[q] = ep_s[q] ? M1 : M0;
        ep_row[q] = n0 + (l >> 4) * 4 + r; ep_col[q] = l & 15;
        ep_on[q] = o < 512 && ep_M[q] > 0 && ep_row[q] < a.n && ep_col[q] < ep_M[q];
        if (ep_on[q] && S == 1) {
            ep_bias[q] = (ep_s[q] ? a.b[1] : a.b[0])[ep_col[q]];
            if (ep_s[q] ? a.extra_col[1] : a.extra_col[0])
                ep_extra[q] = a.alpha_cpt * a.k_cpt[ep_row[q]] * (ep_s[q] ? a.w[1] : a.w[0])[(size_t)K * ep_M[q] + ep_col[q]];
        }
    }
    f32x4 acc0 = {0, 0, 0, 0}, acc1 = {0, 0, 0, 0};
    constexpr int LF_UN = 4;
    const int nkb_all = K >> 4;
    const int kb_lo = slice * nkb_all / S, nkb = (slice + 1) * nkb_all / S;
    const float *xrow = a.a.x + (size_t)(valid ? row : 0) * K;
    for (int kb = kb_lo + wid * LF_UN; kb < nkb; kb += LFW * LF_UN) {
        f32x4 x[LF_UN];
        float b0[LF_UN][4], b1[LF_UN][4];
#pragma unroll
        for (int u = 0; u < LF_UN; ++u) {
            const int kk = kb + u < nkb ? kb + u : kb;
            const int k = kk * 16 + 4 * g;
            x[u] = *(const f32x4 *)(xrow + k);
#pragma unroll
            for (int j = 0; j < 4; ++j) {
                b0[u][j] = li < M0 ? a.w[0][(size_t)(k + j) * M0 + li] : 0.f;
                b1[u][j] = li < M1 ? a.w[1][(size_t)(k + j) * M1 + li] : 0.f;
            }
        }
#pragma unroll
        for (int u = 0; u < LF_UN; ++u) {
            const bool on = valid && kb + u < nkb;
            const int k = (kb + u) * 16 + 4 * g;
            if (bn) {
                const int c = k % C;
#pragma unroll
                for (int j = 0; j < 4; ++j) {
                    const float *cc = cA + (c + j) * 3;
                    x[u][j] = fmaxf((x[u][j] - cc[0]) * cc[1] + cc[2], 0.f);
                }
            }
#pragma unroll
            for (int j = 0; j < 4; ++j) {
                const float xv = on ? x[u][j] : 0.f;
                acc0 = __builtin_amdgcn_mfma_f32_16x16x4f32(xv, b0[u][j], acc0, 0, 0, 0);
                acc1 = __builtin_amdgcn_mfma_f32_16x16x4f32(xv, b1[u][j], acc1, 0, 0, 0);
            }
        }
    }
    trace_stamp(4);
    mfma_drain();
#pragma unroll
    for (int r = 0; r < 4; ++r) {
        red[(wid * 2 + 0) * 256 + lane * 4 + r] = acc0[r];
        red[(wid * 2 + 1) * 256 + lane * 4 + r] = acc1[r];
    }
    __syncthreads();
    float vsum[NO];
#pragma unroll
    for (int q = 0; q < NO; ++q) {
        const int o = tid + q * NT_, e = o & 255;
        float v = 0.f;
        if (o < 512) {
#pragma unroll
            for (int w = 0; w < LFW; ++w) v += red[(w * 2 + ep_s[q]) * 256 + e];
        }
        vsum[q] = v;
    }
// ... 31 lines not shown
                (ep_s[q] ? a.y[1] : a.y[0])[(size_t)ep_row[q] * ep_M[q] + ep_col[q]] = v;
            }
            if (tid == 0) __hip_atomic_store(a.kcnt + blockIdx.x, 0, __ATOMIC_RELAXED, __HIP_MEMORY_SCOPE_SYSTEM);
        }
    }
    trace_stamp(5);
}

int mpnn_trace_install_lin(void *buf) { return mpnn_trace_install(buf); }

extern "C" int mpnn_lin_fwd(const mpnn_lin_fwd_args *dev_table, int count, int n_max, void *stream) {
    if (count <= 0 || n_max <= 0) return 0;
    if (!dev_table) return MPNN_E_ARG;
    hipLaunchKernelGGL((lin_fwd_k<16, false>), dim3((n_max + 15) / 16, count), dim3(16 * 64), 0, (hipStream_t)stream, dev_table, count);
    MPNN_LAUNCH_CHECK();
    return 0;
}

extern "C" int mpnn_lin_fwd_ks(const mpnn_lin_fwd_args *dev_table, int count, int n_max, int k_max, void *stream) {
    if (count <= 0 || n_max <= 0) return 0;
    if (!dev_table || k_max <= 0) return MPNN_E_ARG;
    int s_max = k_max >> 8;
    s_max = s_max < 1 ? 1 : (s_max > MPNN_LIN_KSLICES ? MPNN_LIN_KSLICES : s_max);
    hipLaunchKernelGGL((lin_fwd_k<4, true>), dim3((n_max + 15) / 16, count * s_max), dim3(4 * 64), 0,
                       (hipStream_t)stream, dev_table, count);
    MPNN_LAUNCH_CHECK();
    return 0;
}

#define LB_ROWS 16
#define LB_DP 36
template <int NP, bool RS>
__global__ __launch_bounds__(256) void lin_bwd_k(const mpnn_lin_bwd_args *__restrict__ tab) {
    constexpr int LB_SUPER = NP * LB_ROWS, LB_NP = NP, LB_GP = NP < 4 ? NP : 4;
    const mpnn_lin_bwd_args &a = tab[blockIdx.y];
    const int C = a.a.C, K = a.HW * C;
    const bool has_extra = a.extra_col[0] || a.extra_col[1];
    const int kext = K + (has_extra ? 1 : 0);
    const int k0 = blockIdx.x * 64;
    if (k0 >= kext) return;
    const int np_all = (a.n + LB_ROWS - 1) / LB_ROWS;
    const int ppw = RS ? (np_all + (int)gridDim.z - 1) / (int)gridDim.z : np_all;
    const int Z = RS ? (np_all + ppw - 1) / max(ppw, 1) : 1;
    const int zi = RS ? (int)blockIdx.z : 0;
    if (zi >= Z) return;
    const int r_lo = zi * ppw * LB_ROWS, r_hi = min(a.n, (zi + 1) * ppw * LB_ROWS);
    trace_stamp(0); trace_note(6, 11);
    __shared__ float dys[LB_SUPER * LB_DP];
    __shared__ __attribute__((aligned(16))) float coef[64 * 4];
    __shared__ float tr[2 * 4 * 64 + 256];
    const int tid = threadIdx.x, lane = tid & 63, g = lane >> 4, li = lane & 15;
    const int wid = __builtin_amdgcn_readfirstlane(tid >> 6);
    const int M0 = a.w[0] ? a.M[0] : 0, M1 = a.w[1] ? a.M[1] : 0;
    const bool bn = a.a.mode != MPNN_ACT_IDENTITY;
    const bool fuse_bn = a.dz_out != nullptr && bn;
    const int fl = wid * 16 + li, f = k0 + fl;
    constexpr int DY_PT = LB_SUPER * 32 / 256;
    float xv[LB_NP][4], dyr[DY_PT];
    auto load_super = [&](int R0) {
        const int nr = min(LB_SUPER, r_hi - R0);
#pragma unroll
        for (int q = 0; q < DY_PT; ++q) {
            const int i = tid + q * 256, rr = i >> 5, col = i & 31, s = col >> 4, m = col & 15;
            const int M = s ? M1 : M0;
            const bool ok = rr < nr && m < M;
            const float *dyp = s ? a.dy[1] : a.dy[0];
            dyr[q] = dyp ? dyp[ok ? (size_t)(R0 + rr) * M + m : 0] : 0.f;
            dyr[q] = ok ? dyr[q] : 0.f;
        }
#pragma unroll
        for (int p = 0; p < LB_NP; ++p)
#pragma unroll
            for (int q = 0; q < 4; ++q) {
                const int rr = LB_ROWS * p + 4 * g + q;
                const bool okx = rr < nr && f < K, oke = rr < nr && f == K && has_extra;
                float v = a.a.x[okx ? (size_t)(R0 + rr) * K + f : 0];
                if (has_extra) { const float e = a.k_cpt[oke ? R0 + rr : 0]; v = oke ? a.alpha_cpt * e : v; }
                xv[p][q] = (okx || oke) ? v : 0.f;
            }
    };
    load_super(r_lo);
    if (tid < 64) {
        f32x4 cf = {0.f, 1.f, 0.f, 0.f};
        if (bn && k0 + tid < K) { const BnC c = bn_coef(a.a, (k0 + tid) % C); cf[0] = c.m; cf[1] = c.gamma * c.rstd; cf[2] = c.beta; cf[3] = c.rstd; }
        ((f32x4 *)coef)[tid] = cf;
    }
    float wv[8];
#pragma unroll
    for (int s = 0; s < 8; ++s) {
        const int set = s >> 2, m = 4 * (s & 3) + g, M = set ? M1 : M0;
        const float *wp = set ? a.w[1] : a.w[0];
        const bool ok = m < M && (f < K || (f == K && (set ? a.extra_col[1] : a.extra_col[0])));
        const float v = wp ? wp[ok ? (size_t)f * M + m : 0] : 0.f;
        wv[s] = ok ? v : 0.f;
    }
    f32x4 accW[2] = {f32x4{0.f, 0.f, 0.f, 0.f}, f32x4{0.f, 0.f, 0.f, 0.f}};
    float r1 = 0.f, r2 = 0.f;
    float dbs = 0.f;
    trace_stamp(1);
    for (int R0 = r_lo; R0 < r_hi; R0 += LB_SUPER) {
        const int nr = min(LB_SUPER, r_hi - R0);
        if (R0 != r_lo) load_super(R0);
        __syncthreads();
#pragma unroll
        for (int q = 0; q < DY_PT; ++q) { const int i = tid + q * 256; dys[(i >> 5) * LB_DP + (i & 31)] = dyr[q]; }
        __syncthreads();
        if (blockIdx.x == 0) {
            const int col = tid & 31, rg = tid >> 5;
            float t = 0.f;
#pragma unroll
            for (int rr = 0; rr < LB_SUPER / 8; ++rr) t += dys[(rg * (LB_SUPER / 8) + rr) * LB_DP + col];
            dbs += t;
        }
        static_assert(LB_SUPER % 8 == 0, "db row groups");
        const f32x4 c = ((const f32x4 *)coef)[fl];
#pragma unroll
        for (int pg = 0; pg < LB_NP; pg += LB_GP) {
            if (LB_ROWS * pg >= nr) break;
            float ady[LB_GP][8], bdy[LB_GP][2][4];
#pragma unroll
            for (int pp = 0; pp < LB_GP; ++pp) {
                const int p = pg + pp;
#pragma unroll
                for (int s = 0; s < 8; ++s) ady[pp][s] = dys[(LB_ROWS * p + li) * LB_DP + 4 * s + g];
#pragma unroll
                for (int mt = 0; mt < 2; ++mt)
#pragma unroll
                    for (int s = 0; s < 4; ++s) bdy[pp][mt][s] = dys[(LB_ROWS * p + 4 * g + s) * LB_DP + 16 * mt + li];
            }
            float xa[LB_GP][4], xh[LB_GP][4];
            f32x4 dx[LB_GP];
#pragma unroll
            for (int pp = 0; pp < LB_GP; ++pp) {
#pragma unroll
                for (int q = 0; q < 4; ++q) {
                    const float xc = xv[pg + pp][q] - c[0];
                    xa[pp][q] = (bn && f < K) ? fmaxf(xc * c[1] + c[2], 0.f) : xv[pg + pp][q];
                    xh[pp][q] = xc * c[3];
                }
                dx[pp] = f32x4{0.f, 0.f, 0.f, 0.f};
            }
#pragma unroll
            for (int s = 0; s < 8; ++s)
#pragma unroll
                for (int pp = 0; pp < LB_GP; ++pp) dx[pp] = __builtin_amdgcn_mfma_f32_16x16x4f32(ady[pp][s], wv[s], dx[pp], 0, 0, 0);
#pragma unroll
            for (int pp = 0; pp < LB_GP; ++pp)
#pragma unroll
                for (int s = 0; s < 4; ++s) {
                    accW[0] = __builtin_amdgcn_mfma_f32_16x16x4f32(xa[pp][s], bdy[pp][0][s], accW[0], 0, 0, 0);
                    accW[1] = __builtin_amdgcn_mfma_f32_16x16x4f32(xa[pp][s], bdy[pp][1][s], accW[1], 0, 0, 0);
                }
            asm volatile("" : "+a"(accW[0]), "+a"(accW[1]));
            mfma_drain();
#pragma unroll
            for (int pp = 0; pp < LB_GP; ++pp)
#pragma unroll
                for (int q = 0; q < 4; ++q) {
                    const int rr = LB_ROWS * (pg + pp) + 4 * g + q;
                    if (rr < nr && f < K) {
                        if (a.dx) a.dx[(size_t)(R0 + rr) * K + f] = dx[pp][q];
                        if (fuse_bn) {
                            const float dz = xa[pp][q] > 0.f ? dx[pp][q] : 0.f;
                            a.dz_out[(size_t)(R0 + rr) * K + f] = dz;
                            r1 += dz; r2 += dz * xh[pp][q];
                        }
// ... 126 lines not shown
```

multipath-nn_amd/csrc/wgrad.hip:

```cpp
#include "bwd_bodies.h"
#include "opt_body.h"

template <int GK, int OT, bool SMALLC = false>
__global__ __launch_bounds__(256) void wgrad_k(const WgP p) {
    constexpr int PS = WGeom<GK>::PS, GS = OT * 16 + 4;
    __shared__ __attribute__((aligned(16))) char smem[4 * PS * 16 + 64 * GS * 4 + (128 * 3 + OT * 16 * 5) * 4];
    f32x4 *tile = (f32x4 *)smem;
    float *gt = (float *)(smem + 4 * PS * 16);
    float *cA = gt + 64 * GS;
    if ((int)blockIdx.y >= ((p.c.a.C + 15) >> 4)) wgrad_body<GK, OT, 1>(p, tile, gt, cA, blockIdx.x, blockIdx.y, blockIdx.z, gridDim.x);
    else                                           wgrad_body<GK, OT, 0, SMALLC>(p, tile, gt, cA, blockIdx.x, blockIdx.y, blockIdx.z, gridDim.x);
}


constexpr int MPNN_OCC_BWD = 3;
template <int GK, int OT, bool HASV, bool SMALLC = false>
__global__ __launch_bounds__(256, (OT == 1 && GK != 2 ? (HASV || GK == 1 ? MPNN_OCC_BWD : MPNN_OCC) : 2)) void bwd_scale_k(const BwdScaleP q) {
    constexpr int CB = ConvSmem<GK, 4, 16>::BYTES;
    constexpr int GS = OT * 16 + 4;
    constexpr int WB = 4 * WGeom<GK>::PS * 16 + 64 * GS * 4 + (128 * 3 + OT * 16 * 5) * 4;
    __shared__ __attribute__((aligned(16))) char smem[CB > WB ? CB : WB];
    const int id = blockIdx.x, wh = q.gyh * q.gxh, wv = q.gyv * q.gxv;
    if (id < wh) {
        const int by = id / q.gxh, bx = id - by * q.gxh;
        conv_body<GK, 1, 1, 4, 1, false, EPI_DGH_BN>(q.h, bx, by, q.gxh, smem);
    } else if (HASV && id < wh + wv) {
        if constexpr (HASV) {
            const int l = id - wh, by = l / q.gxv, bx = l - by * q.gxv;
            conv_body<GK, 1, 1, 4, 1, false, EPI_DGV>(q.v, bx, by, q.gxv, smem);
        }
    } else {
        const int l = id - wh - wv, r = l / q.gxw, bx = l - r * q.gxw;
        const int chunk = r % q.nchw, bz = r / q.nchw;
        f32x4 *tile = (f32x4 *)smem;
        float *gt = (float *)(smem + 4 * WGeom<GK>::PS * 16);
        float *cA = gt + 64 * GS;
        if (chunk >= ((q.w.c.a.C + 15) >> 4)) wgrad_body<GK, OT, 1>(q.w, tile, gt, cA, bx, chunk, bz, q.gxw);
        else                                   wgrad_body<GK, OT, 0, SMALLC>(q.w, tile, gt, cA, bx, chunk, bz, q.gxw);
    }
}


template <int GK>
static int wgrad_launch(const WgP &p, int split, hipStream_t st) {
    const ConvP &c = p.c;
    const int nch = ((c.a.C + 15) >> 4) + (c.v ? ((c.Cv + 15) >> 4) : 0);
    dim3 block(256);
    if (c.Cout % 64 == 0) {
        hipLaunchKernelGGL((wgrad_k<GK, 4>), dim3(split, nch, c.Cout / 64), block, 0, st, p);
    } else if (c.Cout % 32 == 0) {
        hipLaunchKernelGGL((wgrad_k<GK, 2>), dim3(split, nch, c.Cout / 32), block, 0, st, p);
    } else if (c.Cout % 16 == 0) {
        if (c.a.C <= 3) hipLaunchKernelGGL((wgrad_k<GK, 1, true>), dim3(split, nch, c.Cout / 16), block, 0, st, p);
        else hipLaunchKernelGGL((wgrad_k<GK, 1>), dim3(split, nch, c.Cout / 16), block, 0, st, p);
    } else return MPNN_E_SHAPE;
    MPNN_LAUNCH_CHECK();
    return 0;
}

int mpnn_trace_install_wgrad(void *buf) { return mpnn_trace_install(buf); }

extern "C" int mpnn_wgrad_tiles(int n, int H, int W) {
    if (W >= 16 && (W % 16) == 0 && (H % 4) == 0) return conv_grid_x<0>(n, H, W);
    if (W == 8 && H == 8) return conv_grid_x<1>(n, 8, 8);
    if (W == 4 && H == 4) return conv_grid_x<2>(n, 4, 4);
    return MPNN_E_SHAPE;
}

static int fill_wgrad(const mpnn_wgrad_args *a, WgP &p, int &split);

extern "C" int mpnn_msconv_wgrad(const mpnn_wgrad_args *a, void *stream) {
    if (a && a->n <= 0) return 0;
    WgP p = {};
    int split = 1;
    const int rc = fill_wgrad(a, p, split);
    if (rc) return rc;
    hipStream_t st = (hipStream_t)stream;
    if (a->W >= 16) return wgrad_launch<0>(p, split, st);
    if (a->W == 8) return wgrad_launch<1>(p, split, st);
    return wgrad_launch<2>(p, split, st);
}

static int fill_wgrad(const mpnn_wgrad_args *a, WgP &p, int &split) {
    if (!a || !a->a.x || !a->g || !a->dwa || !a->db) return MPNN_E_ARG;
    if (a->v && !a->dwv) return MPNN_E_ARG;
    if (a->a.C > 128 || a->Cv > 128 || (a->Cv & 3)) return MPNN_E_SHAPE;
    if (a->a.C > 4 && (a->a.C & 3)) return MPNN_E_SHAPE;
    const int tiles = mpnn_wgrad_tiles(a->n, a->H, a->W);
    if (tiles < 0) return tiles;
    split = a->n_split < 1 ? 1 : (a->n_split > tiles ? tiles : a->n_split);
    if (split > 1 && a->split_stride <= 0) return MPNN_E_ARG;
    p.c.a = a->a;  p.c.v = a->v;  p.c.Cv = a->v ? a->Cv : 0;
    p.c.n = a->n;  p.c.H = a->H;  p.c.W = a->W;  p.c.Cout = a->Cout;
    p.g = a->g;  p.dwa = a->dwa;  p.dwv = a->dwv;  p.db = a->db;
    p.split_stride = a->split_stride;  p.n_tiles = tiles;
    if (a->g_ctx) {
        if (!a->g_ctx->s || !a->g_ctx->red) return MPNN_E_ARG;
        p.g_on = 1;  p.g_s = a->g_ctx->s;  p.g_bn = a->g_ctx->bn;  p.g_red = a->g_ctx->red;
        p.g_nslot = a->g_ctx->red_nslot < 1 ? 1 : a->g_ctx->red_nslot;
    }
    return 0;
}

int mpnn_fill_dgrad_horz(const mpnn_dgrad_horz_args *a, ConvP &p);
int mpnn_fill_dgrad_vert(const mpnn_dgrad_vert_args *a, ConvP &p);

template <int GK>
static auto bwd_scale_kernel(bool wide, bool hasv, bool smallc = false) -> void (*)(const BwdScaleP) {
    if (smallc && !wide) return hasv ? bwd_scale_k<GK, 1, true, true> : bwd_scale_k<GK, 1, false, true>;
    if (hasv) return wide ? bwd_scale_k<GK, 4, true> : bwd_scale_k<GK, 1, true>;
    return wide ? bwd_scale_k<GK, 4, false> : bwd_scale_k<GK, 1, false>;
}

static int wide_cap(bool wide, long dgrad_items) {
    if (!wide) return 0;
    int dev = 0, cus = 256;
    if (hipGetDevice(&dev) == hipSuccess) {
        int v = 0;
        if (hipDeviceGetAttribute(&v, hipDeviceAttributeMultiprocessorCount, dev) == hipSuccess && v > 0) cus = v;
    }
    return dgrad_items <= cus ? 2 : 0;
}

extern "C" int mpnn_msconv_bwd_scale_slots(int H, int W, int Cout, int has_dgrad, int has_vert, int dgrad_items) {
    (void)has_dgrad;
    const bool wide = (Cout % 64) == 0;
    const int gk = (W >= 16 && (W % 16) == 0 && (H % 4) == 0) ? 0 : (W == 8 && H == 8) ? 1 : (W == 4 && H == 4) ? 2 : -1;
    if (gk < 0 || (Cout % 16)) return MPNN_E_SHAPE;
    const bool hv = has_vert != 0;
    const void *k = gk == 0 ? (const void *)bwd_scale_kernel<0>(wide, hv)
                  : gk == 1 ? (const void *)bwd_scale_kernel<1>(wide, hv) : (const void *)bwd_scale_kernel<2>(wide, hv);
    return resident_slots(k, 0, 256, wide_cap(wide, dgrad_items));
}

template <int GK>
static int bwd_scale_launch(BwdScaleP &q, bool has_h, bool has_v, int split, hipStream_t st) {
    const int tiles = conv_grid_x<GK>(q.w.c.n, q.w.c.H, q.w.c.W);
    q.gyh = has_h ? q.h.Cout / 16 : 0;
    q.gyv = has_v ? q.v.Cout / 16 : 0;
    q.h.n_tiles = q.v.n_tiles = tiles;
    q.h.xcd = q.v.xcd = q.w.c.xcd = 1;
    q.gxw = split;
    q.nchw = ((q.w.c.a.C + 15) >> 4) + (q.w.c.v ? ((q.w.c.Cv + 15) >> 4) : 0);
    const bool wide = (q.w.c.Cout % 64) == 0;
    const int gyw = q.nchw * (q.w.c.Cout / (wide ? 64 : 16));
    void (*kern)(const BwdScaleP) = bwd_scale_kernel<GK>(wide, has_v, q.w.c.a.C <= 3);
    const long slots = resident_slots((const void *)kern, 0, 256, wide_cap(wide, (long)tiles * (q.gyh + q.gyv)));
    long avail = slots - (long)split * gyw;
    if (avail < slots / 4) avail = slots / 4;
    const long units = (q.w.c.Cout + 15) >> 4;
    const long wh = has_h ? (long)q.gyh * units : 0, wv = has_v ? (long)q.gyv * units : 0;
    auto share = [&](long w, int gy) {
        if (!w) return 0;
        long g = avail * w / (wh + wv) / gy;
        if (g < 1) g = 1;
        if (g > tiles) g = tiles;
        return xcd_round((int)g);
    };
    q.gxh = share(wh, q.gyh);
    q.gxv = share(wv, q.gyv);
    const dim3 grid(q.gyh * q.gxh + q.gyv * q.gxv + gyw * q.gxw);
    hipLaunchKernelGGL(kern, grid, dim3(256), 0, st, q);
    MPNN_LAUNCH_CHECK();
    return 0;
}

int mpnn_fill_bwd_scale(const mpnn_dgrad_horz_args *h, const mpnn_dgrad_vert_args *v, const mpnn_wgrad_args *w,
                        BwdScaleP &q, int &split) {
    if (!w) return MPNN_E_ARG;
    int rc = fill_wgrad(w, q.w, split);
    if (rc) return rc;
    if (w->Cout % 16) return MPNN_E_SHAPE;
    if (h) {
        if (!h->prev) return MPNN_E_ARG;
        if ((rc = mpnn_fill_dgrad_horz(h, q.h))) return rc;
        if (h->H != w->H || h->W != w->W || h->n != w->n || (h->Cout % 16) || (h->Cg & 3)) return MPNN_E_ARG;
    }
    if (v) {
// ... 189 lines not shown
```

multipath-nn_amd/lib/_eng_alloc.py:

```python
import ctypes as C
import os

import numpy as np
import torch

from lib import _hip
from lib.layer_types import Chain
from lib.net_types import n_leaves, params_list_rec
from lib._eng_common import (BLOCK_COMPS, CAPTURE_MODE, HEAD_COMPS, OPT_CHUNK, ROUTER_COMPS, BoundInput, _attr, _Block, _kind, _nf,
                             _Node)


class Allocation:

    def _classify(self):
        net = self.net
        self.nodes = []
        index = {}
        for ℓ in net.layers:
            nd = _Node()
            nd.idx, nd.layer, nd.kind = len(self.nodes), ℓ, _kind(ℓ)
            nd.parent, nd.sink_index = -1, 0
            index[id(ℓ)] = nd
            self.nodes.append(nd)
# ... 178 lines not shown
        for k in sorted(blk_end):
            if blk_end[k] - conv_lo >= 0.4 * (conv_hi - conv_lo) and blk_end[k] < conv_hi:
                cut, self.dp_cut_block = blk_end[k], k
                break
        end = off
        self.dp_buckets = {}
        n_buckets = int(os.environ.get('MPNN_DP_BUCKETS', '1'))
        if os.environ.get('MPNN_DP_OVERLAP', '1') == '0':
            n_buckets = 1
        if n_buckets <= 1:
            conv_lo, self.dp_cut_block = 0, None
        elif n_buckets == 2:
            self.dp_cut_block = None
        if conv_lo > self.stat_pad:
            self.dp_buckets['exit'] = (0, conv_lo)
        else:
            conv_lo = 0
        if self.dp_cut_block is not None:
            self.dp_buckets['mid'] = (conv_lo, cut)
            self.dp_buckets['end'] = (cut, end)
        else:
            self.dp_buckets['end'] = (conv_lo, end)
        soff = 0
        for p in self.state_params:
            p.offset = soff
            soff += p.size
        dev = self.dev
        self.P = torch.zeros(off, device=dev)
        self.A = torch.zeros(off, device=dev)
        self.G = torch.zeros(off, device=dev)
        self.S = torch.zeros(max(soff, 1), device=dev)
        self.node_stat = self.G[:n_stat]
        for p in self.trainable:
            p.data = self.P[p.offset:p.offset + p.size]
            p.grad = self.G[p.offset:p.offset + p.size]
            p.accum = self.A[p.offset:p.offset + p.size]
        for p in self.state_params:
            p.data = self.S[p.offset:p.offset + p.size]
        desc, poff, pack_of = [], 0, {}
        for b in self.blocks:
            b.pack = {}
            for i in range(b.L if not self.generic_convs else 0):
                names = ['w_horz_%i' % i] + (['w_vert_%i' % (i - 1)] if i > 0 else [])
                for name in names:
                    p = getattr(b.conv.params, name)
                    ci, co = p.shape[2], p.shape[3]
                    fs = 9 * ((ci + 15) // 16) * 16 * co
                    bs = 9 * ((co + 15) // 16) * 16 * ci if ci % 16 == 0 else 0
                    desc += [p.offset, poff, poff + fs if bs else -1, ci, co, 0]
                    pack_of[id(p)] = (p.offset, ci, co, poff, poff + fs if bs else -1)
                    b.pack[name] = (poff, poff + fs if bs else None)
                    poff += fs + bs
        self.n_pack = len(desc) // 6
        self.packs = torch.zeros(max(poff, 1), device=dev)
        self.pack_desc = torch.tensor(desc, dtype=torch.int32, device=dev)
        seg, eqs, eq_off = [], [], 0
        self._seg_owner = []
        self._opt_info = {}

        for p in self.trainable:
            l2 = np.float32(p.l2).view(np.int32)
            has_eq = bool(p.l2) and p.eq is not None
            pk = pack_of.get(id(p), (0, 0, 0, -1, -1))
            self._opt_info[id(p)] = (int(l2), eq_off if has_eq else -1, pk)
            for s in range(0, p.size, OPT_CHUNK):
                seg += [p.offset + s, min(OPT_CHUNK, p.size - s), p.node, p.is_router, int(l2), eq_off + s if has_eq else -1,
                        pk[0], pk[1], pk[2], pk[3], pk[4], 0]
                self._seg_owner.append(id(p))
            if has_eq:
                eqs.append(np.asarray(p.eq, np.float32).reshape(-1))
                eq_off += p.size
        self.w_eq = torch.from_numpy(np.concatenate(eqs)).to(dev) if eqs else None
        self.n_seg = len(seg) // _hip.SEG_INTS
        seg_off = seg[0::_hip.SEG_INTS]
        self.seg_range = {}
        for name, (lo, hi) in self.dp_buckets.items():
            ks = [k for k, o in enumerate(seg_off) if lo <= o < hi]
            self.seg_range[name] = (ks[0], len(ks)) if ks else (0, 0)
            assert not ks or ks == list(range(ks[0], ks[0] + len(ks)))
        for p in self.trainable:
            p._on_assign = self.invalidate_packs
        self._packs_fresh = False
        self.seg = torch.tensor(seg, dtype=torch.int32, device=dev)
        doff, tab = 0, []
        for b in self.blocks:
            b.sum_off = []
            for i in range(b.L):
                bn = b.bns[i].params
                b.sum_off.append(doff)
                tab += [doff, bn.m_avg.offset, bn.v_avg.offset, b.C[i], b.H[i] * b.W[i],
                        bn.γ.offset if b.has_dz[i] else -1, bn.β.offset, self._nslot(b, i)]
                doff += 2 * b.C[i] * _hip.BN_SLOTS
        nd = max(doff, 1)
        zb = (2 * nd + 4) * 8
        gb = (self.G.numel() * 4 + 15) // 16 * 16
        self._zarena = torch.zeros(zb + gb, dtype=torch.uint8, device=dev)
        z64 = self._zarena[:zb].view(torch.float64)
        self.dsum, self.dred, self.loss = z64[:nd], z64[nd:2 * nd], z64[2 * nd:2 * nd + 4]
        self.dsum_last = torch.zeros(nd, dtype=torch.float64, device=dev)
        n_g = self.G.numel()
        self.G = self._zarena[zb:zb + n_g * 4].view(torch.float32)
        self.node_stat = self.G[:n_stat]
        for p in self.trainable:
            p.grad = self.G[p.offset:p.offset + p.size]
        self.n_bn = len(tab) // 8
        self.bn_table = torch.tensor(tab, dtype=torch.int32, device=dev)
        decays = sorted({float(bn.hypers.d) for b in self.blocks for bn in b.bns})
        if len(decays) > 1:
            raise NotImplementedError('conv BatchNorms with different moving-average decays %r are outside the MI355X '
                                      'hot path (one decay per net)' % (decays,))
        self.bn_decay = decays[0] if decays else 0.9
        nodes, ops = [], []
        for nd in self.nodes:
            nd.depth = 0 if nd.parent < 0 else self.nodes[nd.parent].depth + 1
        order = sorted(range(len(self.nodes)), key=lambda j: (self.nodes[j].depth, j))
        rank = {j: k for k, j in enumerate(order)}
        for nd in self.nodes:
            ℓ = nd.layer
            nodes += [nd.parent, nd.sink_index, len(ℓ.sinks), getattr(nd, 'switch_id', -1),
                      getattr(nd, 'leaf_id', -1), n_leaves(ℓ), nd.depth, rank[nd.idx]]
            ops.append(float(ℓ.n_ops + (ℓ.router.n_ops if ℓ.router is not None else 0)))
        kids = []
        for nd in self.switches:
            row = [self.nodes_by_layer(s).idx for s in nd.layer.sinks]
            kids += row + [0] * (self.max_sinks - len(row))
        self.node_tab = torch.tensor(nodes, dtype=torch.int32, device=dev)
        self.kid_tab = torch.tensor(kids if kids else [0], dtype=torch.int32, device=dev)
        self.node_ops = torch.tensor(ops, dtype=torch.float32, device=dev)
        self.node_ops_host = ops
        self.node_ops_i64 = torch.tensor([int(round(o)) for o in ops], dtype=torch.int64, device=dev)
        self.leaf_node_tab = torch.tensor([nd.idx for nd in self.leaves], dtype=torch.int32, device=dev)
        self.hyp = torch.zeros(_hip.HYP_N, device=dev)
        self._hyp_stage = torch.zeros(_hip.HYP_N)
        self._hyp_ring = [(torch.zeros(_hip.HYP_N).pin_memory(), None) for _ in range(8)]
        self._hyp_slot = -1
        self._hyp_sent = None


    def init_params(self, seed=None):
        rng = np.random.default_rng(seed)
        P = np.zeros(self.n_params, np.float32)
        S = np.zeros(self.S.numel(), np.float32)
        for p in self.net._all_params:
            kind, scale = p.init
            if kind == 'normal':
                v = (scale * rng.standard_normal(p.size)).astype(np.float32)
                if p.eq is not None:
                    v = v + p.eq.reshape(-1)
            elif kind == 'ones':
                v = np.ones(p.size, np.float32)
            else:
                v = np.zeros(p.size, np.float32)
            (P if p.trainable else S)[p.offset:p.offset + p.size] = v
        self.P.copy_(torch.from_numpy(P))
        self.S.copy_(torch.from_numpy(S))
        self.A.zero_()
        self.invalidate_packs()


    def _ensure_capacity(self, n, train=True):
        dev = self.dev
        z = lambda *shape: torch.zeros(shape, device=dev)
        if n > self.n_max:
            biggest = max([b.H[i] * b.W[i] * b.C[i] for b in self.blocks for i in range(b.L)] + [int(np.prod(self.x0_shape))])
            if n * biggest >= 2 ** 30:
                raise ValueError('batch of %d samples: the kernels address an activation tensor with 32-bit byte offsets' % n)
            self.n_max = n
            self._progs.clear()
            self._graphs.clear()
            self._gen = getattr(self, '_gen', 0) + 1
            self.n_max_bwd = 0
            h, w, c0 = self.x0_shape
            self.x0 = z(n, h, w, c0)
            self.y = z(n, self.n_cls)
            self.k_cpt = z(n)
            for b in self.blocks:
                b.s = [z(n, b.H[i], b.W[i], b.C[i]) for i in range(b.L)]
                b.sp = [z(n, b.H[i] // 2, b.W[i] // 2, b.C[i]) for i in range(b.L - 1)]
                if b.has_exit:
                    b.z = z(n, self.n_cls) if b.head is not None else None
                    if b.router is not None:
                        R, R2 = (b.router.comps[k].hypers.n_chan for k in (1, 4))
                        b.R, b.R2 = R, R2
                        b.h1, b.h2 = z(n, R), z(n, R2)
                        b.bn_save = z(2 * R + 2 * R2)
            nn, nl, ns = len(self.nodes), len(self.leaves), max(len(self.switches), 1)
            self.p_tr, self.p_ev = z(nn * n), z(nn * n)
            self.w_cerr = z(nl * n)
            self.dr = z(ns * n * self.max_sinks)
            nb = (len(self.blocks) + 3) // 4 * 4
            n_r, n_l = ns * n * self.max_sinks, nl * n
            self._ev_arena = torch.zeros(32 + 4 * nb + 4 * ((n_r + 2 * n_l + 3) // 4 * 4), dtype=torch.uint8, device=dev)
            self.loss_ev = self._ev_arena[:32].view(torch.float64)
            self.ev_cnt = self._ev_arena[32:32 + 4 * nb].view(torch.int32)
            fl = self._ev_arena[32 + 4 * nb:].view(torch.float32)
            self.r, self.c_err, self.d_cor = fl[:n_r], fl[n_r:n_r + n_l], fl[n_r + n_l:n_r + 2 * n_l]
            for k, b in enumerate(self.blocks):
                b.ev_idx = torch.zeros(n, dtype=torch.int32, device=dev)
                b.ev_cnt = self.ev_cnt[k:k + 1]
            self.pr_cls = torch.zeros(nl * n, dtype=torch.int32, device=dev)
            self.pr_conf = z(nl * n)
            self.pr_p = self.pr_probs = None
            self.res_leaf = torch.zeros(n, dtype=torch.int32, device=dev)
            self.res_cls = torch.zeros(n, dtype=torch.int32, device=dev)
            self.res_conf = z(n)
            self.res_ops = torch.zeros(n, dtype=torch.int64, device=dev)
        if train and n > self.n_max_bwd:
            self.n_max_bwd = n
            self._gen = getattr(self, '_gen', 0) + 1
            self._progs = {k: v for k, v in self._progs.items() if k[0] != 'tr'}
            self._graphs = {k: v for k, v in self._graphs.items() if k[0] not in ('tr', 'trK')}
            for b in self.blocks:
                b.dzg = [z(n, b.H[i], b.W[i], b.C[i]) for i in range(b.L)]
                if b.has_exit:
                    b.dx = z(n, b.H[-1] * b.W[-1] * b.C[-1])
                    b.dzh = z(n, self.n_cls) if b.head is not None else None
                    if b.router is not None:
                        b.dh1 = z(n, b.R)
                        b.dh2 = z(n, b.R2) if (self.generic_exits or n > 128) else None


    @staticmethod
    def _nslot(b, i):
        return 8


    def _bn(self, b, i, with_sum=True):
        bn = b.bns[i].params
        return dict(sum=self.dsum[b.sum_off[i]:] if with_sum else None, gamma=bn.γ.data, beta=bn.β.data,
                    m_avg=bn.m_avg.data, v_avg=bn.v_avg.data, eps=float(b.bns[i].hypers.ϵ),
                    nslot=self._nslot(b, i))


    def _act_of_input(self, b, i, n, mode, fwd=False):
        if b.in_map is None:
            if fwd and getattr(self, 'rgbx_probe', False) and b.in_shift[i] > 0:
                return _hip.act(self.x4[b.in_shift[i]], 4, _hip.ACT_IDENTITY, 0)
            return _hip.act(self.x0, self.x0_shape[2], _hip.ACT_IDENTITY, b.in_shift[i])
        pb, j = b.parent, b.in_map[i]
        return _hip.act(pb.s[j], pb.C[j], mode, 0, self._bn(pb, j), n * pb.H[j] * pb.W[j])


    def _bn_ctx(self, b, i, n, with_red=True):
        ctx = _hip.BnCtx()
        ctx.s = b.s[i].data_ptr()
        ctx.bn = _hip.act(None, b.C[i], _hip.ACT_BN_BATCH, 0, self._bn(b, i), n * b.H[i] * b.W[i])
        ctx.red = self.dred[b.sum_off[i]:].data_ptr() if with_red else None
        ctx.red_nslot = self._nslot(b, i)
        self._keep.append(ctx)
        return ctx
```

multipath-nn_amd/lib/_eng_ksteps.py:

```python
import ctypes as C

import numpy as np
import torch

from lib import _hip
from lib._eng_common import CAPTURE_MODE, BoundInput, copy_record


class KStepGraphs:

    STEPS_MAX = 8


    def run_steps(self, feeds):
        net, K = self.net, len(feeds)
        dyn = bool(getattr(net.hypers, 'dyn_k_cpt', False))
        dp = self.allreduce is not None
        ok = 1 < K <= self.STEPS_MAX and self.use_graph and not self.multi_stream and \
            (not dp or (self.dp_one_graph and self.allreduce_capturable and not self._bucket_opt_on() and getattr(self, '_k_dp_ok', True)))
        if ok:
            xs = [f[net.x0] for f in feeds]
            ys = [f[net.y] for f in feeds]
            bound = all(isinstance(x, BoundInput) and isinstance(y, BoundInput) and x.eng is self and y.eng is self
                        for x, y in zip(xs, ys)) and len({x.n for x in xs} | {y.n for y in ys}) == 1
            same = all(isinstance(x, torch.Tensor) and x.data_ptr() == xs[0].data_ptr() and x.shape == xs[0].shape for x in xs) and \
                isinstance(xs[0], torch.Tensor) and xs[0].data_ptr() == self.x0.data_ptr() and \
                all(isinstance(y, torch.Tensor) and y.data_ptr() == self.y.data_ptr() and y.shape[0] == xs[0].shape[0] for y in ys)
            ok = (bound and self.prologue_slot is not None) or (same and self.prologue is None)
            ok = ok and all(f.get(net.mode, net.mode.default) == 'tr' for f in feeds)
        def one_by_one():
            slots = self.prologue_slot is not None and all(isinstance(f[net.x0], BoundInput) for f in feeds)
            keep_p, keep_g = self.prologue, self.use_graph
            try:
                for j, f in enumerate(feeds):
                    if slots and j > 0:
                        self.prologue, self.use_graph = (lambda st, j=j: self.prologue_slot(st, j)), False
                    self.run(f, True)
            finally:
                self.prologue, self.use_graph = keep_p, keep_g
        if not ok:
            return one_by_one()
        n = int(xs[0].shape[0])
        key = ('trK', n, K, self.bwd_levels, self.fold_clear, self.fuse_opt, self.co_share, dp)
        g = self._graphs.get(key)
        if g is None:
            one_by_one()
            self._graphs[key] = 'warm'
            return
        prog = self.program('tr', n)
        if not (prog.get('fold') and (prog.get('fused_opt') or dp)):
            return one_by_one()
        if len(self._event_keep) > 4096:
            torch.cuda.synchronize()
            self._event_keep.clear()
        if not hasattr(self, '_hypk'):
            self._hypk = torch.zeros(self.STEPS_MAX, _hip.HYP_N, device=self.dev)
            self._hypk_ring = [(torch.zeros(self.STEPS_MAX, _hip.HYP_N).pin_memory(), None) for _ in range(8)]
            self._hypk_slot = -1
        if dyn:
            if getattr(self, '_kck', None) is None or self._kck.shape[1] < self.n_max:
                self._kck = torch.zeros(self.STEPS_MAX, self.n_max, device=self.dev)
                self._kck_ring = [(torch.zeros(self.STEPS_MAX, self.n_max).pin_memory(), None) for _ in range(8)]
                self._kck_slot = -1
                self._graphs = {k: v for k, v in self._graphs.items() if k[0] != 'trK'}
                g = self._graphs.get(key)
                if g is None:
                    one_by_one()
                    self._graphs[key] = 'warm'
                    return
            r = self._kck_slot = (self._kck_slot + 1) % len(self._kck_ring)
            kbuf, kev = self._kck_ring[r]
            if kev is not None:
                kev.synchronize()
            stage, on_dev = [], {}
            for j, f in enumerate(feeds):
                def put_k(dst, src, j=j):
                    if isinstance(src, torch.Tensor) and src.is_cuda:
                        on_dev[j] = src
                    else:
                        src = src if isinstance(src, torch.Tensor) else torch.from_numpy(np.ascontiguousarray(src, dtype=np.float32))
                        kbuf[j, :n].copy_(src.reshape(-1))
                stage.append(self._hyp_values(f, n, put_k).clone())
            hs = torch.stack(stage)
            if not on_dev:
                self._kck[:K, :n].copy_(kbuf[:K, :n], non_blocking=True)
            else:
                for j in range(K):
                    self._kck[j, :n].copy_(on_dev[j].reshape(-1) if j in on_dev else kbuf[j, :n], non_blocking=True)
            kev = torch.cuda.Event()
            kev.record(torch.cuda.current_stream())
            self._kck_ring[r] = (kbuf, kev)
        else:
            hs = torch.stack([self._hyp_values(f, n).clone() for f in feeds])
        if getattr(self, '_hypk_sent', None) is None or self._hypk_sent.shape != hs.shape or not torch.equal(hs, self._hypk_sent):
            r = self._hypk_slot = (self._hypk_slot + 1) % len(self._hypk_ring)
            buf, ev = self._hypk_ring[r]
            if ev is not None:
                ev.synchronize()
            buf[:K].copy_(hs)
            self._hypk[:K].copy_(buf[:K], non_blocking=True)
            ev = torch.cuda.Event()
            ev.record(torch.cuda.current_stream())
            self._hypk_ring[r] = (buf, ev)
            self._hypk_sent = hs
        self._hyp_sent = None
        self._hyp_epoch = getattr(self, '_hyp_epoch', 0) + 1
        if not self._packs_fresh:
            self._pack()
            self._packs_fresh = True
        if g == 'warm':
            torch.cuda.synchronize()
            if not self._acc_clean:
                self._begin(True)
                self._acc_clean = True
            assert [op.what for op in prog['fwd']].count('exit_tail_fwd') == 1

            def step_op(j, op):
                kp = self._kck[j].data_ptr() if dyn else None
                if op.what == 'exit_tail_fwd':
                    recs = [copy_record(r, hyp_src=self._hypk[j].data_ptr(), hyp_dst=self.hyp.data_ptr()) if k == 0 else copy_record(r)
                            for k, r in enumerate(op.host)]
                elif dyn and op.what in ('lin_fwd', 'lin_bwd'):
                    recs = [copy_record(r, k_cpt=kp) if r.k_cpt else copy_record(r) for r in op.host]
                elif dyn and op.what == 'route':
                    c = copy_record(op.host, k_cpt_vec=kp)
                    self._keep.append(c)
# ... 52 lines not shown
```

multipath-nn_amd/lib/_eng_planner.py:

```python
import ctypes as C
import functools
import os

import numpy as np
import torch

from lib import _hip
from lib._eng_common import Launch, _attr


class Planner:

    def _wsplit(self, b, i, n, fused=False):
        H = b.H[i]
        tiles = n * (H // 16) * (H // 4) if H >= 16 else (n if H == 8 else (n + 3) // 4)
        nch = (b.Cin[i] + 15) // 16 + ((b.C[i - 1] + 15) // 16 if i > 0 else 0)
        groups = max(1, b.C[i] // 64) if b.C[i] % 64 == 0 else (b.C[i] // 32 if b.C[i] % 32 == 0 else b.C[i] // 16)
        if fused:
            groups = b.C[i] // 64 if b.C[i] % 64 == 0 else b.C[i] // 16
        budget = 512
        if fused:
            has_dgrad = 1 if (b.in_map is not None or i > 0) else 0
            dg_items = tiles * ((b.parent.C[b.in_map[i]] // 16 if b.parent is not None else 0) + (b.C[i - 1] // 16 if i > 0 else 0))
            slots = self.lib.mpnn_msconv_bwd_scale_slots(b.H[i], b.W[i], b.C[i], has_dgrad, 1 if i > 0 else 0, dg_items)
# ... 98 lines not shown
            tiles = lib.mpnn_wgrad_tiles(n, b.H[i], b.W[i])
            units = b.C[i] // 16
            if b.parent is not None:
                bodies.append((k, 'h', b.parent.C[b.in_map[i]] // 16, tiles, LAT['h'] * units))
            if i > 0:
                bodies.append((k, 'v', b.C[i - 1] // 16, tiles, LAT['v'] * units))
            ot = 4 if b.C[i] % 64 == 0 else 1
            nch = (b.Cin[i] + 15) // 16 + ((b.C[i - 1] + 15) // 16 if i > 0 else 0)
            bodies.append((k, 'w', nch * (b.C[i] // (16 * ot)), tiles, LAT['w%d' % ot]))
        if sum(rows for _, _, rows, _, _ in bodies) > slots:
            return None

        def fit(T):
            gx = []
            for _, _, rows, tiles, lat in bodies:
                per = int(T / lat + 1e-9)
                if per < 1:
                    return None
                gx.append(-(-tiles // per))
            return gx if sum(g * body[2] for g, body in zip(gx, bodies)) <= slots else None
        cands = sorted({lat * j for _, _, _, tiles, lat in bodies for j in range(1, tiles + 1)})
        lo, hi = 0, len(cands) - 1
        while lo < hi:
            mid = (lo + hi) // 2
            if fit(cands[mid]) is not None:
                hi = mid
            else:
                lo = mid + 1
        gx = fit(cands[lo])
        if gx is None:
            return None
        used = sum(g * body[2] for g, body in zip(gx, bodies))
        while True:
            cand = [q for q in range(len(gx)) if gx[q] < bodies[q][3] and used + bodies[q][2] <= slots]
            if not cand:
                break
            q = max(cand, key=lambda q: -(-bodies[q][3] // gx[q]) * bodies[q][4])
            gx[q] += 1
            used += bodies[q][2]
        if os.environ.get('MPNN_PLAN_DEBUG'):
            print('level budget: %d slots, chain %.1f; ' % (slots, cands[lo]) + '; '.join(
                'm%d %s rows %d tiles %d -> gx %d (%d wgs, %d items/wg)' % (k, kind, rows, tiles, g, g * rows, -(-tiles // g))
                for (k, kind, rows, tiles, lat), g in zip(bodies, gx)))
        out = [dict(gxh=0, gxv=0, split=1) for _ in grp]
        for (k, kind, rows, tiles, lat), g in zip(bodies, gx):
            if self.co_share == 1:
                g = self._xcd_round(g)
            if kind == 'w':
                kb, b, i = grp[k]
                g = max(1, min(g, max(1, (12 << 20) // self._w_bytes(b, i))))
            out[k]['gxh' if kind == 'h' else 'gxv' if kind == 'v' else 'split'] = int(g)
        return out


    def program(self, mode, n, routed=False):
        try:
            return self._program(mode, n, routed)
        finally:
            self.lib.mpnn_set_reserved_cus(0)


    def routed_prefix(self, n):
        table = self._ROUTED_PREFIX_GEN if self.generic_convs else self._ROUTED_PREFIX
        for lim, d0 in table:
            if n >= lim:
                return d0
        return table[-1][1]

    _ROUTED_PREFIX = ((6144, 1), (3072, 2), (1536, 3), (640, 4), (0, 6))
    _ROUTED_PREFIX_GEN = ((0, 1),)


    def _program(self, mode, n, routed):
        if routed == 'auto':
            routed = n >= (self.routed_min_batch_gen if self.generic_convs else self.routed_min_batch)
        explicit = routed if (isinstance(routed, int) and not isinstance(routed, bool) and routed >= 1) else None
        routed = bool(routed) and mode != 'tr' and bool(self.switches) and self.net._net_kind != 'sr'
        if routed:
            routed = explicit if explicit is not None else self.routed_prefix(n)
        if mode == 'tr' and self.allreduce is not None and self.multi_stream:
            raise NotImplementedError('data-parallel training runs on the single-stream schedule (MPNN_STREAMS=0)')
        dp = mode == 'tr' and self.allreduce is not None
        reserve = self.dp_reserve_cus if (dp and len(self.dp_buckets) > 1) else 0
        key = (mode, n, self.multi_stream, self.group_fwd, routed, dp, self.bwd_levels, self.fold_clear, reserve, self.fuse_opt, self.co_share)
        if key in self._progs:
            return self._progs[key]
        self._ensure_capacity(n, mode == 'tr')
        if mode != 'tr':
            prog = self._progs[key] = self._program_ev(n, routed) if mode == 'ev' else self._program_pr(n, routed, mode == 'pr+p')
            return prog
        if self.multi_stream and self.generic_convs:
            raise NotImplementedError('the multi-stream schedule has no launches for the general conv kernels (filters other '
                                      'than 3x3, maps other than the tuned squares): such nets run on the single-stream '
                                      'schedule (MPNN_STREAMS=0)')
        if self.multi_stream and any(len(b.children) > 1 for b in self.blocks):
            raise NotImplementedError('the multi-stream schedule serialises nothing between sibling blocks that '
                                      'accumulate into one gradient map: tree nets run on the single-stream schedule')
        prog = self._progs[key] = self._program_tr(n, dp, reserve)
        return prog


    def _program_tr(self, n, dp, reserve):
        sizes = sorted({h for b in self.blocks for h in b.H}, reverse=True)
        sid = {h: (0 if h == sizes[-1] else 1 + k) for k, h in enumerate(sizes)}
        self.n_streams = len(sizes) + 2
        fwd = [Launch(None, 'fork')]
        if self.group_fwd and not self.multi_stream and self._groupable() and \
                all(b.parent is not None or b.in_map is None for b in self.blocks):
            for members in self._wavefront(self.blocks):
                fwd += self._conv_fwd_launches(members, n, 'tr')
        else:
            F = lambda b, i: 'F%d_%d' % (self.blocks.index(b), i)
            for b in self.blocks:
                for i in range(b.L):
                    fwd.append(self._conv_fwd_single(b, i, n, 'tr', None, 'msconv_fwd', stream=sid[b.H[i]],
                                                     waits=[F(b, i - 1)] if i > 0 else [], records=F(b, i)))
        fwd.append(Launch(None, 'join'))
        exit_fwd, bwd, fold = self._exit_launches(n)
        fwd += exit_fwd + [self._route_launch(n, 'tr', self.loss)]
        if dp and 'exit' in self.dp_buckets:
            bwd.append(Launch(None, 'bucket', tag='exit'))
        self.lib.mpnn_set_reserved_cus(reserve)
        convs, fused_opt = self._bwd_launches(n, sid, dp, reserve, fold)
        bwd += convs
        if dp:
            bwd.append(Launch(None, 'bucket', tag='end'))
        return dict(fwd=fwd, bwd=bwd, n=n, mode='tr', fold=fold, fused_opt=fused_opt)


    def _conv_fwd_args(self, b, i, n, mode, rows=None):
        train = mode == 'tr'
        a = _hip.ConvFwdArgs()
        a.a = self._act_of_input(b, i, n, _hip.ACT_BN_BATCH if train else _hip.ACT_BN_MOVING, fwd=train)
        cp = b.conv.params
        if i > 0:
            a.v, a.Cv = b.sp[i - 1].data_ptr(), b.C[i - 1]
            a.wv_pack = getattr(cp, 'w_vert_%i' % (i - 1)).data.data_ptr() if self.generic_convs else \
                self.packs[b.pack['w_vert_%i' % (i - 1)][0]:].data_ptr()
        if i < b.L - 1:
            a.pool_out = b.sp[i].data_ptr()
        a.wa_pack = getattr(cp, 'w_horz_%i' % i).data.data_ptr() if self.generic_convs else \
            self.packs[b.pack['w_horz_%i' % i][0]:].data_ptr()
        a.bias = getattr(b.conv.params, 'b_%i' % i).data.data_ptr()
        a.out = b.s[i].data_ptr()
        a.out_sum = self.dsum[b.sum_off[i]:].data_ptr() if train else None
        a.out_nslot = self._nslot(b, i)
        a.n, a.H, a.W, a.Cout = n, b.H[i], b.W[i], b.C[i]
        if rows is not None:
            a.idx, a.cnt = rows[0].data_ptr(), rows[1].data_ptr()
        return a


    @staticmethod
    def _conv_flops(b, i, n):
        (kh, kw), (kvh, kvw) = b.kh[i], b.kv[i] or (0, 0)
        return 2.0 * n * b.H[i] * b.W[i] * b.C[i] * (kh * kw * b.Cin[i] + (kvh * kvw * b.C[i - 1] if i > 0 else 0))


    def _conv_fwd_single(self, b, i, n, mode, rows, what, **kw):
        a = self._conv_fwd_args(b, i, n, mode, rows)
        self._keep.append(a)
        fl, tag = self._conv_flops(b, i, n), self._conv_tag(b, i)
        if self.generic_convs:
            return Launch(self._gen_fn('fwd'), what, C.byref(a), *b.kh[i], *(b.kv[i] or (0, 0)), flops=fl, tag=tag, **kw)
        return Launch(self.lib.mpnn_msconv_fwd, what, C.byref(a), flops=fl, tag=tag, **kw)


    @staticmethod
    def _conv_tag(b, i):
        hw = 'h%d' % b.H[i] if b.H[i] == b.W[i] else 'h%dx%d' % (b.H[i], b.W[i])
        return '%s %d+%d->%d' % (hw, b.Cin[i], b.C[i - 1] if i > 0 else 0, b.C[i])


    def _wavefront(self, blocks):
        depth = self._depths()
        kidx = {h: k for k, h in enumerate(sorted({h for b in self.blocks for h in b.H}, reverse=True))}
        levels = {}
        for b in blocks:
            for i in range(b.L):
                levels.setdefault(depth[id(b)] + kidx[b.H[i]], []).append((b, i))
        return [levels[d] for d in sorted(levels)]


    def _conv_fwd_launches(self, members, n, mode, rows=lambda b: None):
        lib, out = self.lib, []
        if not self._groupable():
            return [self._conv_fwd_single(b, i, n, mode, rows(b), 'fwd') for b, i in members]
        for c0 in range(0, len(members), 4):
            grp = members[c0:c0 + 4]
            arr = (_hip.ConvFwdArgs * len(grp))(*[self._conv_fwd_args(b, i, n, mode, rows(b)) for b, i in grp])
            dev_arr = _hip.to_device_table(list(arr), self.dev)
            self._keep += [arr, dev_arr]
            fl, tag = sum(self._conv_flops(b, i, n) for b, i in grp), ' | '.join(self._conv_tag(b, i) for b, i in grp)
            if self.co_share > 1:
                out.append(Launch(lib.mpnn_msconv_fwd_group_rep, 'fwd_group', arr, dev_arr.data_ptr(), len(grp), 1, self.co_share,
                                  flops=fl, tag=tag, host=arr))
            else:
                out.append(Launch(lib.mpnn_msconv_fwd_group, 'fwd_group', arr, dev_arr.data_ptr(), len(grp), flops=fl, tag=tag, host=arr))
        return out


    def _depths(self):
        depth = {}
        for b in self.blocks:
            depth[id(b)] = 0 if b.parent is None else depth[id(b.parent)] + 1
        return depth


    def _groupable(self):
        return not self.generic_convs and \
            all(c % 16 == 0 and not (c % 64 == 0 and h >= 16) for b in self.blocks for c, h in zip(b.C, b.H))


    def _exit_launches(self, n):
        lib, keep = self.lib, self._keep
        act_mode = _hip.ACT_BN_BATCH
        ϕ = self.net.hypers
        dyn = bool(getattr(ϕ, 'dyn_k_cpt', False))
        lin_f, lin_b, tail_f, tail_b = [], [], [], []
        MS = self.max_sinks
        kmax = 0
        for b in self.blocks:
            if not b.has_exit:
                continue
            L1 = b.L - 1
            K = b.H[L1] * b.W[L1] * b.C[L1]
            kmax = max(kmax, K)
            lf, lb = _hip.LinFwdArgs(), _hip.LinBwdArgs()
            tf, tb = _hip.ExitTailArgs(), _hip.ExitTailBwdArgs()
            a_in = _hip.act(b.s[L1], b.C[L1], act_mode, 0, self._bn(b, L1), n * b.H[L1] * b.W[L1])
            lf.a, lb.a = a_in, a_in
            lf.HW = lb.HW = b.H[L1] * b.W[L1]
            lf.n = lb.n = tf.n = n
            lf.k_cpt = lb.k_cpt = self.k_cpt.data_ptr()
            lf.alpha_cpt = lb.alpha_cpt = float(_attr(ϕ, 'α_cpt', 0.0))
            if K >= 512 and n <= 512:
                rg = (n + 15) // 16
                kpart = torch.empty(rg * _hip.LIN_KSLICES * 512, device=self.dev)
                kcnt = torch.zeros(rg, dtype=torch.int32, device=self.dev)
                keep += [kpart, kcnt]
                lf.kpart, lf.kcnt = kpart.data_ptr(), kcnt.data_ptr()
            if n <= 512:
                nblk = (K + 1 + 63) // 64
                bpart = torch.empty(nblk * _hip.LIN_RSPLIT * _hip.LIN_RS_TILE, device=self.dev)
                bcnt = torch.zeros(nblk, dtype=torch.int32, device=self.dev)
                keep += [bpart, bcnt]
                lb.kpart, lb.kcnt = bpart.data_ptr(), bcnt.data_ptr()
            lb.dx = b.dx.data_ptr()
            if not b.children and not self.multi_stream and not self.generic_exits:
                lb.dx = None
                lb.dz_out = b.dzg[L1].data_ptr()
                lb.red_out = self.dred[b.sum_off[L1]:].data_ptr()
                lb.red_nslot = self._nslot(b, L1)
            tf.mode = act_mode
            if b.head is not None:
                lt, ce = b.head.layer.comps[1], b.head.layer.comps[3]
                lf.w[0], lf.b[0], lf.y[0], lf.M[0] = lt.params.w.data.data_ptr(), lt.params.b.data.data_ptr(), b.z.data_ptr(), self.n_cls
                lb.w[0], lb.dy[0], lb.M[0] = lf.w[0], b.dzh.data_ptr(), self.n_cls
                lb.dw[0], lb.db[0] = lt.params.w.grad.data_ptr(), lt.params.b.grad.data_ptr()
                leaf = b.head.leaf_id
                tf.z, tf.y, tf.n_cls, tf.eps_ce = b.z.data_ptr(), self.y.data_ptr(), self.n_cls, float(ce.hypers.ϵ)
                tf.c_err = self.c_err[leaf * n:].data_ptr()
                tf.d_cor = self.d_cor[leaf * n:].data_ptr()
                tb.w_cerr = self.w_cerr[leaf * n:].data_ptr()
                tb.dz = b.dzh.data_ptr()
            if b.router is not None:
                rc = b.router.comps
                l1, bn1, l2, bn2, l3 = rc[1], rc[2], rc[4], rc[5], rc[7]
                R, S = b.R, len(b.node.layer.sinks)
                sw = b.node.switch_id
                lf.w[1], lf.b[1], lf.y[1], lf.M[1] = l1.params.w.data.data_ptr(), l1.params.b.data.data_ptr(), b.h1.data_ptr(), R
                lb.w[1], lb.dy[1], lb.M[1] = lf.w[1], b.dh1.data_ptr(), R
                lb.dw[1], lb.db[1] = l1.params.w.grad.data_ptr(), l1.params.b.grad.data_ptr()
                lf.extra_col[1] = lb.extra_col[1] = 1 if dyn else 0
                tf.h1, tf.R, tf.n_sinks, tf.R2 = b.h1.data_ptr(), R, S, b.R2
                tf.g1, tf.b1 = bn1.params.γ.data.data_ptr(), bn1.params.β.data.data_ptr()
                tf.m1, tf.v1 = bn1.params.m_avg.data.data_ptr(), bn1.params.v_avg.data.data_ptr()
                tf.w2, tf.bias2 = l2.params.w.data.data_ptr(), l2.params.b.data.data_ptr()
                tf.g2, tf.b2 = bn2.params.γ.data.data_ptr(), bn2.params.β.data.data_ptr()
                tf.m2, tf.v2 = bn2.params.m_avg.data.data_ptr(), bn2.params.v_avg.data.data_ptr()
                tf.w3, tf.bias3 = l3.params.w.data.data_ptr(), l3.params.b.data.data_ptr()
                tf.h2 = b.h2.data_ptr()
                tf.r, tf.r_stride = self.r[sw * n * MS:].data_ptr(), MS
                tf.bn_save = b.bn_save.data_ptr()
                tf.bn_eps, tf.bn_decay = float(bn1.hypers.ϵ), float(bn1.hypers.d)
                tf.bn_eps2, tf.bn_decay2 = float(bn2.hypers.ϵ), float(bn2.hypers.d)
                tb.dr = self.dr[sw * n * MS:].data_ptr()
                tb.dh1 = b.dh1.data_ptr()
                if getattr(b, 'dh2', None) is not None:
                    tb.dh2 = b.dh2.data_ptr()
                tb.dg1, tb.db1 = bn1.params.γ.grad.data_ptr(), bn1.params.β.grad.data_ptr()
                tb.dw2, tb.dbias2 = l2.params.w.grad.data_ptr(), l2.params.b.grad.data_ptr()
                tb.dg2, tb.db2 = bn2.params.γ.grad.data_ptr(), bn2.params.β.grad.data_ptr()
                tb.dw3, tb.dbias3 = l3.params.w.grad.data_ptr(), l3.params.b.grad.data_ptr()
            tb.f = tf
            lin_f.append(lf); lin_b.append(lb); tail_f.append(tf); tail_b.append(tb)
        n_exit = len(lin_f)
        fold = n_exit > 0 and self.fold_clear
        if not n_exit:
            return [], [], fold
        if fold:
            tail_f[0].clear_f, tail_f[0].n_clear_f = self.node_stat.data_ptr(), self.node_stat.numel()
            tail_f[0].clear_d, tail_f[0].n_clear_d = self.loss.data_ptr(), self.loss.numel()
        t_lf, t_lb = _hip.to_device_table(lin_f, self.dev), _hip.to_device_table(lin_b, self.dev)
        t_tf, t_tb = _hip.to_device_table(tail_f, self.dev), _hip.to_device_table(tail_b, self.dev)
        keep += [t_lf, t_lb, t_tf, t_tb]
        if self.generic_exits:
            lin_fwd = Launch(lib.mpnn_lin_fwd_gen, 'lin_fwd', t_lf.data_ptr(), n_exit, n, host=lin_f)
        elif n <= 512:
            lin_fwd = Launch(lib.mpnn_lin_fwd_ks, 'lin_fwd', t_lf.data_ptr(), n_exit, n, kmax, host=lin_f)
        else:
            lin_fwd = Launch(lib.mpnn_lin_fwd, 'lin_fwd', t_lf.data_ptr(), n_exit, n, host=lin_f)
        gen_tails = self.generic_exits or n > 128
        lin_bwd = lib.mpnn_lin_bwd_gen if self.generic_exits else lib.mpnn_lin_bwd_rs if n <= 512 else lib.mpnn_lin_bwd
# ... 20 lines not shown
        ra.p_tr, ra.p_ev, ra.w_cerr, ra.dr = self.p_tr.data_ptr(), self.p_ev.data_ptr(), self.w_cerr.data_ptr(), self.dr.data_ptr()
        ra.node_stat = self.node_stat.data_ptr() if mode == 'tr' else None
        if mode == 'tr':
            need = (n + 15) // 16 * (len(self.nodes) * 2 + 8)
            if getattr(self, '_stat_part', None) is None or self._stat_part.numel() < need:
                self._stat_part = torch.zeros(need, device=self.dev)
                self._stat_ticket = torch.zeros(4, dtype=torch.int32, device=self.dev)
            ra.stat_part, ra.stat_ticket = self._stat_part.data_ptr(), self._stat_ticket.data_ptr()
            self._keep += [self._stat_part, self._stat_ticket]
        ra.loss = loss.data_ptr()
        ra.n, ra.n_total = n, n
        self._keep.append(ra)
        return Launch(self.lib.mpnn_route, 'route', C.byref(ra), host=ra)


    def _bwd_launches(self, n, sid, dp, reserve, fold):
        lib, keep = self.lib, self._keep
        call = functools.partial(Launch, reserve=reserve)
        Gn = lambda b, i: 'G%d_%d' % (self.blocks.index(b), i)
        bwd = [Launch(None, 'fork')]
        dz_written = set()
        slab_size = 0
        slab_members = []
        slab_params = set()
        levels = []
        cut_kb = self.dp_cut_block if dp else None

        def make_block(kb, b):
            cp = b.conv.params
            L1 = b.L - 1
            pre = []
            if not b.children and (self.multi_stream or not b.has_exit or self.generic_exits):
                ctx = self._bn_ctx(b, L1, n, with_red=False)
                pre.append(call(lib.mpnn_bn_bwd_reduce, 'bn_bwd_reduce', b.dx.data_ptr(), C.byref(ctx),
                                b.dzg[L1].data_ptr(), self.dred[b.sum_off[L1]:].data_ptr(),
                                n * b.H[L1] * b.W[L1], stream=sid[b.H[L1]]))
            g_ctx = None
            if self.multi_stream or self.generic_convs:
                ctx = self._bn_ctx(b, L1, n)
                pre.append(call(lib.mpnn_bn_bwd_apply, 'bn_bwd_apply', b.dzg[L1].data_ptr(), C.byref(ctx),
                                n * b.H[L1] * b.W[L1], stream=sid[b.H[L1]], records=Gn(b, L1)))
            else:
                g_ctx = C.pointer(self._bn_ctx(b, L1, n))

            def vert_args(i):
                a = _hip.DgradVertArgs()
                fine = self._bn_ctx(b, i - 1, n)
                a.g, a.Cg = b.dzg[i].data_ptr(), b.C[i]
                if i == L1 and g_ctx is not None:
                    a.g_ctx = g_ctx
                a.w_pack = getattr(cp, 'w_vert_%i' % (i - 1)).data.data_ptr() if self.generic_convs else \
                    self.packs[b.pack['w_vert_%i' % (i - 1)][1]:].data_ptr()
                a.fine = C.pointer(fine)
                a.fine_has_dz = 1 if b.has_dz[i - 1] else 0
                a.dz_g_fine = b.dzg[i - 1].data_ptr()
                a.n, a.H, a.W, a.Cout = n, b.H[i], b.W[i], b.C[i - 1]
                keep.append(a)
                return a

            def horz_args(i):
                pb, j = b.parent, b.in_map[i]
                a = _hip.DgradHorzArgs()
                a.g, a.Cg = b.dzg[i].data_ptr(), b.C[i]
                if i == L1 and g_ctx is not None:
                    a.g_ctx = g_ctx
                a.w_pack = getattr(cp, 'w_horz_%i' % i).data.data_ptr() if self.generic_convs else \
                    self.packs[b.pack['w_horz_%i' % i][1]:].data_ptr()
                first = (id(pb), j) not in dz_written
                dz_written.add((id(pb), j))
                a.accumulate = 0 if first else 1
                a.dy_extra = pb.dx.data_ptr() if (first and pb.has_exit and j == pb.L - 1) else None
                prev = self._bn_ctx(pb, j, n, with_red=False)
                a.prev = C.pointer(prev)
                a.out = pb.dzg[j].data_ptr()
                a.red_out = self.dred[pb.sum_off[j]:].data_ptr()
                a.n, a.H, a.W, a.Cout = n, b.H[i], b.W[i], pb.C[j]
                keep.append(a)
                return a

            def wgrad_args(i, split=None):
                nonlocal slab_size
                a = _hip.WgradArgs()
                a.a = self._act_of_input(b, i, n, _hip.ACT_BN_BATCH)
                pa = getattr(cp, 'w_horz_%i' % i)
                pv = getattr(cp, 'w_vert_%i' % (i - 1)) if i > 0 else None
                pb = getattr(cp, 'b_%i' % i)
                if i > 0:
                    a.v, a.Cv = b.sp[i - 1].data_ptr(), b.C[i - 1]
                a.g = b.dzg[i].data_ptr()
                if i == L1 and g_ctx is not None:
                    a.g_ctx = g_ctx
                a.n, a.H, a.W, a.Cout = n, b.H[i], b.W[i], b.C[i]
                if split is None:
                    split = self._wsplit_gen(b, i, n) if self.generic_convs else self._wsplit(b, i, n, fused=not self.multi_stream)
                a.n_split = split
                if split == 1:
                    a.dwa, a.db = pa.grad.data_ptr(), pb.grad.data_ptr()
                    a.dwv = pv.grad.data_ptr() if pv is not None else None
                    a.split_stride = 0
                else:
                    sizes = [pa.size, pv.size if pv is not None else 0, pb.size]
                    stride = (sum(sizes) + 3) // 4 * 4
                    off = slab_size
                    slab_size += split * stride
                    rows, ptrs, srows = [], [], []
                    for prm, sz in zip((pa, pv, pb), sizes):
                        if prm is None:
                            continue
                        item = _hip.slab_item_size(split)
                        l2b, eqo, pk = self._opt_info[id(prm)]
                        if pk[1] and pk[1] % 4 == 0:
                            item = min(_hip.SLAB_ITEM, max(item, 4 * pk[2]))
                        for k in range(0, sz, item):
                            cnt = min(item, sz - k)
                            rows += [off + k, prm.offset + k, cnt, split, stride, 0]
                            srows += [prm.offset + k, cnt, prm.node, prm.is_router, l2b, eqo + k if eqo >= 0 else -1,
                                      pk[0], pk[1], pk[2], pk[3], pk[4], 0]
                        slab_params.add(id(prm))
                        ptrs.append((a, {id(pa): 'dwa', id(pb): 'db'}.get(id(prm), 'dwv'), off))
                        off += sz
                    slab_members.append((cut_kb is not None and kb <= cut_kb, rows, ptrs, srows))
                    a.split_stride = stride
                keep.append(a)
                return a

            return pre, vert_args, horz_args, wgrad_args

        fl_v = lambda b, i: 2.0 * n * b.H[i] * b.W[i] * b.kv[i][0] * b.kv[i][1] * b.C[i] * b.C[i - 1]
        fl_h = lambda b, i: 2.0 * n * b.H[i] * b.W[i] * b.kh[i][0] * b.kh[i][1] * b.C[i] * b.parent.C[b.in_map[i]]
        mid = None
        if not self.multi_stream:
            order = [(kb, b, i) for kb, b in enumerate(reversed(self.blocks)) for i in range(b.L - 1, -1, -1)]
            groups = self._bwd_schedule(order, n) if (self.bwd_levels and not self.generic_convs) else [[(m, None)] for m in order]
            fns = {kb: make_block(kb, b) for kb, b in enumerate(reversed(self.blocks))}
            started = set()
            last_cut = max([g for g, grp in enumerate(groups) for (kb, b, i), _ in grp if cut_kb is not None and kb <= cut_kb],
                           default=None)
            rec_bytes = lib.mpnn_msconv_bwd_level_record_size()
            for g, grp in enumerate(groups):
                for (kb, b, i), _ in grp:
                    if kb not in started:
                        started.add(kb)
                        bwd += fns[kb][0]
                built = []
                for (kb, b, i), bud in grp:
                    _, vert_args, horz_args, wgrad_args = fns[kb]
                    h = horz_args(i) if b.parent is not None else None
                    v = vert_args(i) if i > 0 else None
                    w = wgrad_args(i, None if bud is None else bud['split'])
                    fl = self._conv_flops(b, i, n) + (fl_h(b, i) if h is not None else 0) + (fl_v(b, i) if v is not None else 0)
                    built.append((h, v, w, bud, fl, self._conv_tag(b, i)))
                fl, tag = sum(x[4] for x in built), ' | '.join(x[5] for x in built)
                if self.generic_convs:
                    (kb, b, i), _ = grp[0]
                    h, v, w = built[0][:3]
                    kv = b.kv[i] or (0, 0)
                    if h is not None:
                        bwd.append(call(self._gen_fn('dgrad_horz'), 'dgrad_horz', C.byref(h), *b.kh[i], flops=fl_h(b, i), tag=tag))
                    if v is not None:
                        bwd.append(call(self._gen_fn('dgrad_vert'), 'dgrad_vert', C.byref(v), *kv, flops=fl_v(b, i), tag=tag))
                    bwd.append(call(self._gen_fn('wgrad'), 'wgrad', C.byref(w), *b.kh[i], *kv, flops=self._conv_flops(b, i, n),
                                    tag=tag))
                elif len(built) == 1 and built[0][3] is None:
                    h, v, w = built[0][:3]
                    bwd.append(call(lib.mpnn_msconv_bwd_scale, 'bwd_scale', C.byref(h) if h is not None else None,
                                    C.byref(v) if v is not None else None, C.byref(w), flops=fl, tag=tag))
# ... 109 lines not shown
```

multipath-nn_amd/lib/_eng_run.py:

```python
import ctypes as C
import os

import numpy as np
import torch

from lib import _hip
from lib.net_types import n_leaves, params_list_rec
from lib._eng_common import (BLOCK_COMPS, CAPTURE_MODE, HEAD_COMPS, OPT_CHUNK, ROUTER_COMPS, BoundInput, _attr, _Block, _kind, _nf,
                             _Node)


class Runner:


    def ensure_capacity(self, n, train=True):
        return self._ensure_capacity(n, train)

    @property
    def generation(self):
        return getattr(self, '_gen', 0)

    def drop_programs(self):
        self._progs.clear()
        self._graphs.clear()
# ... 253 lines not shown


    def _dispatch(self, prog, train, n):
        if not self.use_graph:
            self._step_eager(prog, train, n)
        else:
            self._run_graphed(prog, train, n)


    def run(self, feed, train, routed=False):
        n, mode = self._enter(feed)
        if train and mode != 'tr':
            raise ValueError("net.train.run needs net.mode: 'tr' in the feed")
        if not train and mode == 'tr':
            self._forward_tr(n)
            self.last_n, self.last_mode = n, mode
            self._bind_views(n)
            return
        prog = self.program(mode, n, routed)
        if train and prog.get('fold') and self._acc_clean and os.environ.get('MPNN_PLAN_DEBUG'):
            torch.cuda.synchronize()
            assert not bool(self.dsum.any()) and not bool(self.dred.any()), 'slot sums not clean at the start of a step'
        self._dispatch(prog, train, n)
        self.last_n, self.last_mode = n, mode
        if train:
            self._last_fold = bool(prog.get('fold'))
        self._bind_views(n)


    def predict(self, x0, routed='auto', probs=False, k_cpt=None, table=None):
        from types import SimpleNamespace as Ns
        net = self.net
        dyn = bool(getattr(net.hypers, 'dyn_k_cpt', False))
        if dyn and k_cpt is None:
            raise ValueError('predict: a dyn_k_cpt net needs k_cpt (one value, or one per image)')
        if not dyn and k_cpt is not None:
            raise ValueError('predict: k_cpt is an input of dyn_k_cpt nets only; this net has a fixed k_cpt')
        if any(nd.kind != 'head' for nd in self.leaves):
            raise NotImplementedError('predict: a leaf without a classifier has no prediction')
        if table is not None:
            x0 = self._decode_into_x0(x0, table)
        feed = {net.x0: x0}
        if dyn:
            feed[net.k_cpt] = k_cpt
        n, _ = self._enter(feed, labels=False)
        self._dispatch(self.program('pr+p' if probs else 'pr', n, routed), False, n)
        self.last_n, self.last_mode = n, 'pr'
        self._bind_views(n)
        return Ns(cls=self.res_cls[:n], leaf=self.res_leaf[:n], conf=self.res_conf[:n], ops=self.res_ops[:n],
                  probs=self.pr_probs[:n] if probs else None)


    def _step_eager(self, prog, train, n):
        self._phase_a(prog, train, n)
        if train and not prog.get('fused_opt') and not (self.allreduce is not None and self._bucket_opt_on()):
            self._opt(n)


    def set_prologue(self, fn, fn_slot=None):
        self.prologue, self.prologue_slot = fn, fn_slot
        self._graphs = {k: v for k, v in self._graphs.items() if k[0] not in ('tr', 'trK')}


    def mark_dirty(self):
        self._acc_clean = False


    def _forward_tr(self, n):
        prog = self.program('tr', n)
        fold = bool(prog.get('fold'))
        if not (fold and self._acc_clean):
            self._begin(True)
        self._acc_clean = False
        self._launch([op for op in prog['fwd'] if op.what not in ('fork', 'join')] if not self.multi_stream else prog['fwd'], 0)
        _hip.check(self.lib.mpnn_bn_finalize(self.dsum.data_ptr(), None, self.S.data_ptr(), None, self.bn_table.data_ptr(),
                                             self.n_bn, self.bn_decay, n, self.dsum_last.data_ptr() if fold else None,
                                             torch.cuda.current_stream().cuda_stream), 'bn_finalize')
        self._last_fold = fold
        self._acc_clean = fold


    def _run_graphed(self, prog, train, n):
        key = (prog['mode'], n, train, prog.get('routed', False), self.bwd_levels, self.fold_clear,
               self.allreduce is not None, self._bucket_opt_on())
        g = self._graphs.get(key)
        if g is None:
            self._step_eager(prog, train, n)
            self._graphs[key] = 'warm'
            return
        dp = train and self.allreduce is not None
        fold = train and bool(prog.get('fold'))
        if g == 'warm':
            torch.cuda.synchronize()
            if fold and not self._acc_clean:
                self._begin(True)
                self._acc_clean = True
            g = None
            if not dp or (self.dp_one_graph and self.allreduce_capturable):
                err = None
                if dp and self.dp_quiesce is not None:
                    self.dp_quiesce()
                try:
                    ga = torch.cuda.CUDAGraph()
                    with torch.cuda.graph(ga, capture_error_mode=CAPTURE_MODE):
                        self._step_eager(prog, train, n)
                    g = ([(ga, None)], 'whole')
                except Exception as e:
                    if not dp:
                        raise
                    err = e
                if dp:
                    torch.cuda.synchronize()
                    ok = self.dp_agree(err is None) if self.dp_agree is not None else err is None
                    if not ok:
                        import warnings
                        warnings.warn('capturing the data-parallel step as one hipGraph failed on some rank (here: %r): '
                                      'every rank falls back to one graph per gradient-bucket section' % (err,))
                        g = None
                        self.dp_one_graph = False
                        self._acc_clean = False
                        if fold:
                            self._begin(True)
                            self._acc_clean = True
            if g is None:
                secs = []
                for k, (ops, bucket) in enumerate(self._sections(prog, train)):
                    gk = torch.cuda.CUDAGraph()
                    with torch.cuda.graph(gk, capture_error_mode=CAPTURE_MODE):
                        if k == 0:
                            if train and self.prologue is not None:
                                self.prologue(torch.cuda.current_stream().cuda_stream)
                            self._clear_if_needed(prog, train)
                        self._launch(ops, k)
                    secs.append((gk, bucket))
                gb = None
                if not self._bucket_opt_on():
                    gb = torch.cuda.CUDAGraph()
                    with torch.cuda.graph(gb, capture_error_mode=CAPTURE_MODE):
                        self._opt(n)
                g = (secs, gb)
            self._graphs[key] = g
        secs, gb = g
        if fold and not self._acc_clean:
            self._begin(True)
        if train:
            self._acc_clean = False
        handles = []
        for gk, bucket in secs:
            gk.replay()
            if bucket is not None:
                h = self._reduce_bucket(bucket)
                if self._bucket_opt_on():
                    self._opt_bucket(n, bucket, h)
                else:
                    handles.append(h)
        if dp and gb != 'whole' and gb is not None:
            self._wait(handles)
            gb.replay()
        if train:
            self._acc_clean = fold
```

multipath-nn_amd/lib/_hip.py:

```python
import ctypes as C
import os

_HERE = os.path.dirname(os.path.abspath(__file__))
LIB_PATH = os.environ.get('MPNN_HIP_LIB') or os.path.join(os.path.dirname(_HERE), 'libmpnn_hip.so')

ACT_IDENTITY, ACT_BN_BATCH, ACT_BN_MOVING, ACT_RELU = 0, 1, 2, 3
NET_SR, NET_ACTOR, NET_CRITIC = 0, 1, 2
HYP_LR, HYP_MU, HYP_TAU, HYP_EPS, HYP_KCPT, HYP_KDEC, HYP_KCRE, HYP_ARTR, HYP_N = 0, 1, 2, 3, 4, 5, 6, 7, 16
MAX_NODES, MAX_SINKS = 128, 4
BN_SLOTS = 16
SEG_INTS = 12
SLAB_ITEM = 1024
LIN_KSLICES = 8
LIN_RSPLIT = 8
LIN_RS_TILE = 2080


def slab_item_size(n_split):
    size = SLAB_ITEM
    while size > 64 and (256 // (size // 4)) * 16 < n_split:
        size //= 2
    return size

P = C.c_void_p


class Act(C.Structure):
    _fields_ = [('x', P), ('sum', P), ('gamma', P), ('beta', P), ('m_avg', P), ('v_avg', P),
                ('eps', C.c_float), ('cnt', C.c_int), ('C', C.c_int), ('shift', C.c_int), ('mode', C.c_int),
                ('nslot', C.c_int)]


class ConvFwdArgs(C.Structure):
    _fields_ = [('a', Act), ('v', P), ('Cv', C.c_int), ('wa_pack', P), ('wv_pack', P), ('bias', P),
                ('out', P), ('pool_out', P), ('out_sum', P), ('out_nslot', C.c_int), ('n', C.c_int), ('H', C.c_int), ('W', C.c_int),
                ('Cout', C.c_int), ('idx', P), ('cnt', P)]


class BnCtx(C.Structure):
    _fields_ = [('s', P), ('bn', Act), ('red', P), ('red_nslot', C.c_int)]


class DgradHorzArgs(C.Structure):
    _fields_ = [('g', P), ('Cg', C.c_int), ('g_ctx', C.POINTER(BnCtx)), ('w_pack', P), ('dy_extra', P),
                ('prev', C.POINTER(BnCtx)),
                ('out', P), ('red_out', P), ('n', C.c_int), ('H', C.c_int), ('W', C.c_int), ('Cout', C.c_int),
                ('accumulate', C.c_int)]


class DgradVertArgs(C.Structure):
    _fields_ = [('g', P), ('Cg', C.c_int), ('g_ctx', C.POINTER(BnCtx)), ('w_pack', P), ('fine', C.POINTER(BnCtx)),
                ('fine_has_dz', C.c_int),
                ('dz_g_fine', P), ('n', C.c_int), ('H', C.c_int), ('W', C.c_int), ('Cout', C.c_int)]


class WgradArgs(C.Structure):
    _fields_ = [('a', Act), ('v', P), ('Cv', C.c_int), ('g', P), ('g_ctx', C.POINTER(BnCtx)), ('dwa', P), ('dwv', P),
                ('db', P),
                ('split_stride', C.c_long), ('n', C.c_int), ('H', C.c_int), ('W', C.c_int), ('Cout', C.c_int), ('n_split', C.c_int)]


BWD_LEVEL_MAX = 4


class BwdMember(C.Structure):
    _fields_ = [('horz', C.POINTER(DgradHorzArgs)), ('vert', C.POINTER(DgradVertArgs)), ('wgrad', C.POINTER(WgradArgs)),
                ('wg_horz', C.c_int), ('wg_vert', C.c_int)]


class LinFwdArgs(C.Structure):
    _fields_ = [('a', Act), ('HW', C.c_int), ('w', P * 2), ('b', P * 2), ('y', P * 2), ('M', C.c_int * 2),
                ('k_cpt', P), ('alpha_cpt', C.c_float), ('extra_col', C.c_int * 2), ('n', C.c_int),
                ('kpart', P), ('kcnt', P)]


class LinBwdArgs(C.Structure):
    _fields_ = [('a', Act), ('HW', C.c_int), ('w', P * 2), ('dy', P * 2), ('M', C.c_int * 2),
                ('dw', P * 2), ('db', P * 2), ('dx', P), ('k_cpt', P), ('alpha_cpt', C.c_float),
                ('extra_col', C.c_int * 2), ('n', C.c_int),
                ('dz_out', P), ('red_out', P), ('red_nslot', C.c_int), ('kpart', P), ('kcnt', P)]


class ExitTailArgs(C.Structure):
    _fields_ = [('z', P), ('y', P), ('n_cls', C.c_int), ('eps_ce', C.c_float), ('c_err', P), ('d_cor', P),
                ('h1', P), ('R', C.c_int), ('n_sinks', C.c_int),
                ('g1', P), ('b1', P), ('m1', P), ('v1', P), ('w2', P), ('bias2', P),
                ('g2', P), ('b2', P), ('m2', P), ('v2', P), ('w3', P), ('bias3', P),
                ('h2', P), ('r', P), ('r_stride', C.c_int), ('bn_save', P),
                ('bn_eps', C.c_float), ('bn_decay', C.c_float), ('mode', C.c_int), ('n', C.c_int),
                ('clear_f', P), ('n_clear_f', C.c_int), ('clear_d', P), ('n_clear_d', C.c_int), ('R2', C.c_int),
                ('hyp_src', P), ('hyp_dst', P), ('bn_eps2', C.c_float), ('bn_decay2', C.c_float)]


class ExitTailBwdArgs(C.Structure):
    _fields_ = [('f', ExitTailArgs), ('w_cerr', P), ('dr', P), ('dz', P), ('dh1', P),
                ('dg1', P), ('db1', P), ('dw2', P), ('dbias2', P), ('dg2', P), ('db2', P),
                ('dw3', P), ('dbias3', P), ('dh2', P)]


class ExitEvArgs(C.Structure):
    _fields_ = [('a', Act), ('HW', C.c_int), ('w_head', P), ('b_head', P), ('n_cls', C.c_int), ('y', P),
                ('eps_ce', C.c_float), ('c_err', P), ('d_cor', P),
                ('w1', P), ('b1', P), ('R', C.c_int), ('n_sinks', C.c_int),
                ('extra_col', C.c_int), ('k_cpt', P), ('alpha_cpt', C.c_float),
                ('g1', P), ('be1', P), ('m1', P), ('v1', P), ('w2', P), ('bias2', P),
                ('g2', P), ('be2', P), ('m2', P), ('v2', P), ('w3', P), ('bias3', P),
                ('bn_eps', C.c_float), ('r', P), ('r_stride', C.c_int),
                ('idx', P), ('cnt', P), ('n', C.c_int),
                ('child_idx', P * 4), ('child_cnt', P * 4), ('R2', C.c_int), ('z', P), ('h1', P), ('bn_eps2', C.c_float),
                ('cls', P), ('conf', P), ('p_cls', P), ('p_stride', C.c_int)]


class ConvNhwcFwdArgs(C.Structure):
    _fields_ = [('a', Act), ('w', P), ('bias', P), ('out', P), ('n', C.c_int), ('H', C.c_int), ('W', C.c_int),
                ('Cout', C.c_int), ('supp', C.c_int)]


class ConvNhwcDgradArgs(C.Structure):
    _fields_ = [('g', P), ('Cg', C.c_int), ('w', P), ('relu_src', P), ('scratch', P), ('dx', P),
                ('n', C.c_int), ('H', C.c_int), ('W', C.c_int), ('Cin', C.c_int), ('supp', C.c_int)]


class ConvNhwcWgradArgs(C.Structure):
    _fields_ = [('a', Act), ('g', P), ('dw', P), ('db', P), ('split_stride', C.c_long), ('n_split', C.c_int),
                ('n', C.c_int), ('H', C.c_int), ('W', C.c_int), ('Cout', C.c_int), ('supp', C.c_int)]


class RouteArgs(C.Structure):
    _fields_ = [('net_type', C.c_int), ('n_nodes', C.c_int), ('n_leaves', C.c_int), ('n_switches', C.c_int),
                ('max_sinks', C.c_int), ('optimistic', C.c_int), ('use_cls_err', C.c_int), ('want_grad', C.c_int),
                ('nodes', P), ('sw_children', P), ('node_ops', P), ('hyp', P), ('k_cpt_vec', P), ('r', P),
                ('c_err', P), ('d_cor', P), ('p_tr', P), ('p_ev', P), ('w_cerr', P), ('dr', P),
                ('node_stat', P), ('loss', P), ('n', C.c_int), ('n_total', C.c_int), ('stat_part', P), ('stat_ticket', P)]


class FinishNet(C.Structure):
    _fields_ = [('slabs', P), ('slab_table', P), ('n_items', C.c_int), ('item_seg', P),
                ('sums', P), ('reds', P), ('state', P), ('bn_table', P), ('n_bn', C.c_int), ('bn_opt', P), ('n_img', C.c_int),
                ('sums_keep', P), ('params', P), ('accum', P), ('grads', P), ('node_stat', P), ('hyp', P), ('talr', C.c_int),
                ('inv_n', C.c_float), ('grad_scale', C.c_float), ('w_eq', P), ('packs', P), ('plain_seg', P), ('n_plain', C.c_int)]


PREFIX_MAX = 64


class EvPrefixArgs(C.Structure):
    _fields_ = [('n', C.c_int), ('count', C.c_int), ('n_front', C.c_int), ('pad_', C.c_int),
                ('parent', C.c_int * PREFIX_MAX), ('parent_sink', C.c_int * PREFIX_MAX), ('n_sinks', C.c_int * PREFIX_MAX),
                ('r_stride', C.c_int * PREFIX_MAX), ('r', P * PREFIX_MAX), ('c_err', P * PREFIX_MAX), ('d_cor', P * PREFIX_MAX),
                ('front_parent', C.c_int * PREFIX_MAX), ('front_sink', C.c_int * PREFIX_MAX),
                ('front_idx', P * PREFIX_MAX), ('front_cnt', P * PREFIX_MAX)]


class EvSelectArgs(C.Structure):
    _fields_ = [('n', C.c_int), ('n_nodes', C.c_int), ('n_leaves', C.c_int), ('n_cls', C.c_int),
                ('p_ev', P), ('node_ops', P), ('leaf_node', P), ('leaf_cls', P), ('leaf_conf', P), ('leaf_p', P),
                ('leaf_stride', C.c_int), ('p_stride', C.c_int),
                ('leaf', P), ('cls', P), ('conf', P), ('probs', P), ('ops', P)]


class AugmentDst(C.Structure):
    _fields_ = [('draw', P), ('x_out', P), ('y_out', P)]

# ... 144 lines not shown
```

multipath-nn_amd/lib/_plan.py:

```python
import os

import torch

from lib import _hip
from lib._eng_common import (BLOCK_COMPS, CAPTURE_MODE, HEAD_COMPS, OPT_CHUNK, ROUTER_COMPS, BoundInput, _attr, _Block, _kind, _nf,
                             _Node)
from lib._eng_alloc import Allocation
from lib._eng_planner import Planner
from lib._eng_eval import EvalPrograms
from lib._eng_run import Runner
from lib._eng_dp import DataParallelSections
from lib._eng_ksteps import KStepGraphs
from lib._eng_inspect import Inspection
from lib._eng_stream import StreamedPredict


class Engine(Allocation, Planner, EvalPrograms, Runner, StreamedPredict, DataParallelSections, KStepGraphs, Inspection):
    def __init__(self, net, device=None, n_max=128):
        self.net = net
        self.lib = _hip.load()
        if not torch.cuda.is_available():
            raise _hip.HipError('no GPU visible: the multipath-nn hot path runs on MI355X only')
        if device is None:
            device = 'cuda:%d' % int(os.environ.get('LOCAL_RANK', '0'))
        self.dev = torch.device(device)
        torch.cuda.set_device(self.dev)
        self.n_max = self.n_max_bwd = 0
        self.use_graph = bool(int(os.environ.get('MPNN_GRAPH', '1')))
        self.multi_stream = bool(int(os.environ.get('MPNN_STREAMS', '0')))
        self.group_fwd = bool(int(os.environ.get('MPNN_FWD_GROUP', '1')))
        self.bwd_levels = bool(int(os.environ.get('MPNN_BWD_LEVELS', '1')))
        self.routed_min_batch = 512
        self.routed_min_batch_gen = 512
        self.fold_clear = bool(int(os.environ.get('MPNN_FOLD_CLEAR', '1')))
        self._acc_clean = False
        self._streams = []
        self._event_keep = []
        self.n_streams = 1
        self.world = 1
        self.allreduce = None
        self.allreduce_capturable = False
        self.dp_agree = None
        self.dp_quiesce = None
        self.dp_one_graph = bool(int(os.environ.get('MPNN_DP_ONE_GRAPH', '1')))
        self.dp_reserve_cus = int(os.environ.get('MPNN_DP_RESERVE_CUS', '0'))
        self.dp_bucket_opt = bool(int(os.environ.get('MPNN_DP_BUCKET_OPT', '0')))
        self._opt_stream = None
        self.prologue = None
        self.prologue_slot = None
        self.fuse_opt = bool(int(os.environ.get('MPNN_FUSE_OPT', '1')))
        self.co_share = 1
        self._keep = []
        self._init_stream_state()
        self._progs = {}
        self._graphs = {}
        self._classify()
        self._alloc_params()
        self.init_params(net.hypers.__dict__.get('seed'))
        self._ensure_capacity(n_max)
        self.last_n = 0
        self.last_mode = 'ev'
```

Baseline: 264,800 images/s.

## Cache per-channel batch-norm coefficient rows once and reuse across kernels

Adds a per-BN-layer buffer of (mean, rstd, gamma*rstd, beta) rows. The first forward consumer (block 0 of the conv, strip or linear kernel) writes it, and later forward, wgrad, dgrad and linear-backward kernels read it instead of recomputing the coefficients from the double-precision slot sums. This is meant to cut redundant slot reductions and rsqrt work in kernel prologues and to let some barriers be deferred or dropped. It relies on the write-before-read ordering that the planner tracks. The path is disabled for data-parallel runs and non-wavefront schedules, and a new MPNN_BN_ROWS switch is added to the graph and program cache keys.

Measured after the change: 265,600 images/s, median of 6. About the same (+0.3%).

```diff
diff --git a/include/mpnn_hip.h b/include/mpnn_hip.h
--- a/include/mpnn_hip.h
+++ b/include/mpnn_hip.h
@@ -50,6 +50,8 @@
     int n, H, W, Cout;
     const int *idx;
     const int *cnt;
+    const float *a_rows;
+    float *a_rows_out;
 } mpnn_conv_fwd_args;
 int mpnn_msconv_fwd(const mpnn_conv_fwd_args *args, void *stream);
 int mpnn_msconv_fwd_group(const mpnn_conv_fwd_args *args, const mpnn_conv_fwd_args *dev_args, int count,
@@ -62,6 +64,7 @@
     mpnn_act bn;
     const double *red;
     int red_nslot;
+    const float *rows;
 } mpnn_bn_ctx;
 int mpnn_bn_bwd_reduce(const float *dy, const mpnn_bn_ctx *ctx, float *dz,
                        double *red_out, long n_pix, void *stream);
@@ -103,6 +106,7 @@
     long split_stride;
     int n, H, W, Cout;
     int n_split;
+    const float *a_rows;
 } mpnn_wgrad_args;
 int mpnn_msconv_wgrad(const mpnn_wgrad_args *args, void *stream);
 int mpnn_msconv_bwd_scale(const mpnn_dgrad_horz_args *horz, const mpnn_dgrad_vert_args *vert,
@@ -171,6 +175,7 @@
     const float *k_cpt;  float alpha_cpt;  int extra_col[2];
     int n;
     float *kpart;  int *kcnt;
+    const float *a_rows;  float *a_rows_out;
 } mpnn_lin_fwd_args;
 #define MPNN_LIN_KSLICES 8
 int mpnn_lin_fwd(const mpnn_lin_fwd_args *dev_table, int count, int n_max, void *stream);
@@ -185,6 +190,7 @@
     int n;
     float *dz_out;  double *red_out;  int red_nslot;
     float *kpart;  int *kcnt;
+    const float *a_rows;
 } mpnn_lin_bwd_args;
 #define MPNN_LIN_RSPLIT 8
 #define MPNN_LIN_RS_TILE 2080
diff --git a/multipath-nn_amd/csrc/bwd_bodies.h b/multipath-nn_amd/csrc/bwd_bodies.h
--- a/multipath-nn_amd/csrc/bwd_bodies.h
+++ b/multipath-nn_amd/csrc/bwd_bodies.h
@@ -81,6 +81,10 @@
         slot9[j] = (img * HR + ty) * R + tx;
     }
 
+    const bool a_late = part == 0 && c.a_rows != nullptr;
+    [[maybe_unused]] f32x4 rowA = {0.f, 0.f, 0.f, 0.f};
+    if (a_late) rowA = rows_load(c.a_rows, tid < c.a.C ? tid : 0);
+    else
     if (part == 0 && c.a.mode != MPNN_ACT_IDENTITY) {
         for (int cc = tid; cc < c.a.C; cc += 256) {
             const BnC k = bn_coef(c.a, cc);
@@ -105,7 +109,7 @@
     }
 
     if constexpr (XItems<GK>::INTERIOR) zero_halo(tile, 4 * PS, tid, 256);
-    __syncthreads();
+    if (a_late) lds_barrier(); else __syncthreads();
     trace_stamp(1);
     f32x4 xr[XN][1], gr[OT], gs[OT];
     int on0;
@@ -274,6 +278,7 @@
         }
     };
     if (sq0 < sqn) request(sq0);
+    if (a_late && tid < c.a.C) { cA[tid * 3] = rowA[0]; cA[tid * 3 + 1] = rowA[2]; cA[tid * 3 + 2] = rowA[3]; }
     for (int t = sq0; t < sqn; t += sqd) tile_step(t);
 
     trace_stamp(4);
diff --git a/multipath-nn_amd/csrc/common.h b/multipath-nn_amd/csrc/common.h
--- a/multipath-nn_amd/csrc/common.h
+++ b/multipath-nn_amd/csrc/common.h
@@ -109,6 +109,29 @@
     return k;
 }
 
+__device__ __forceinline__ f32x4 rows_load(const float *rows, int c) { return ((const f32x4 *)rows)[c]; }
+__device__ __forceinline__ void rows_store(float *rows, int c, float mean, float rstd, float gamma, float beta) {
+    ((f32x4 *)rows)[c] = f32x4{mean, rstd, gamma * rstd, beta};
+}
+__device__ __forceinline__ void bn_bwd_row_rows(const float *rows, const mpnn_act &b, const double *red, int red_nslot, int c,
+                                                bool want_beta, float *e) {
+    const f32x4 r = rows_load(rows, c);
+    e[0] = r[0]; e[1] = r[1]; e[2] = r[2];
+    if (want_beta) { e[3] = r[3]; e[4] = 0.f; return; }
+    const int C2 = 2 * b.C, rn = red ? red_nslot : 0;
+    const unsigned o0 = (unsigned)c * 8u, o1 = (unsigned)(b.C + c) * 8u;
+    double r0 = 0.0, r1 = 0.0;
+    if (rn == 8) {
+        double q0[8], q1[8];
+#pragma unroll
+        for (int s = 0; s < 8; ++s) { q0[s] = ld_slot(red, C2, s, o0); q1[s] = ld_slot(red, C2, s, o1); }
+#pragma unroll
+        for (int s = 0; s < 8; ++s) { r0 += q0[s]; r1 += q1[s]; }
+    } else if (rn) slot_sum2(red, C2, c, b.C + c, rn, r0, r1);
+    const double inv = 1.0 / (double)b.cnt;
+    e[3] = (float)(r0 * inv); e[4] = (float)(r1 * inv);
+}
+
 __device__ __forceinline__ void bn_bwd_row(const mpnn_act &b, const double *red, int red_nslot, int c, bool want_beta, float *e) {
     const int C2 = 2 * b.C, ns = b.nslot, rn = red ? red_nslot : 0;
     const float gamma = b.gamma[c], beta = b.beta[c];
diff --git a/multipath-nn_amd/csrc/conv_dgrad.hip b/multipath-nn_amd/csrc/conv_dgrad.hip
--- a/multipath-nn_amd/csrc/conv_dgrad.hip
+++ b/multipath-nn_amd/csrc/conv_dgrad.hip
@@ -3,7 +3,7 @@
 static int fill_g_ctx(const mpnn_bn_ctx *c, ConvP &p) {
     if (!c) return 0;
     if (!c->s || !c->red) return MPNN_E_ARG;
-    p.ga_on = 1;  p.ga_s = c->s;  p.ga_bn = c->bn;  p.ga_red = c->red;
+    p.ga_on = 1;  p.ga_s = c->s;  p.ga_bn = c->bn;  p.ga_red = c->red;  p.ga_rows = c->rows;
     p.ga_nslot = c->red_nslot < 1 ? 1 : c->red_nslot;
     return 0;
 }
@@ -16,7 +16,7 @@
     p.extra = a->dy_extra;  p.out = a->out;  p.acc_out = a->accumulate ? 1 : 0;
     if (a->prev) {
         if (!a->prev->s || !a->red_out) return MPNN_E_ARG;
-        p.sprev = a->prev->s;  p.pbn = a->prev->bn;  p.red_out = a->red_out;
+        p.sprev = a->prev->s;  p.pbn = a->prev->bn;  p.red_out = a->red_out;  p.pbn_rows = a->prev->rows;
         p.out_nslot = a->prev->red_nslot < 1 ? 1 : a->prev->red_nslot;
     }
     return fill_g_ctx(a->g_ctx, p);
@@ -27,7 +27,7 @@
     p.a.x = a->g;  p.a.C = a->Cg;  p.a.mode = MPNN_ACT_IDENTITY;  p.a.shift = 0;
     p.wa = a->w_pack;
     p.n = a->n;  p.H = a->H;  p.W = a->W;  p.Cout = a->Cout;
-    p.out = a->dz_g_fine;  p.sprev = a->fine->s;  p.pbn = a->fine->bn;
+    p.out = a->dz_g_fine;  p.sprev = a->fine->s;  p.pbn = a->fine->bn;  p.pbn_rows = a->fine->rows;
     p.red = a->fine_has_dz ? a->fine->red : nullptr;  p.has_dz = a->fine_has_dz;
     p.red_nslot = a->fine->red_nslot < 1 ? 1 : a->fine->red_nslot;
     return fill_g_ctx(a->g_ctx, p);
diff --git a/multipath-nn_amd/csrc/conv_fwd.hip b/multipath-nn_amd/csrc/conv_fwd.hip
--- a/multipath-nn_amd/csrc/conv_fwd.hip
+++ b/multipath-nn_amd/csrc/conv_fwd.hip
@@ -26,6 +26,7 @@
     p.out_nslot = a->out_nslot < 1 ? 1 : (a->out_nslot > MPNN_BN_SLOTS ? MPNN_BN_SLOTS : a->out_nslot);
     if (a->pool_out && (a->H < 8 || (a->H & 1) || (a->W & 1))) return MPNN_E_SHAPE;
     p.idx = a->idx;
+    p.a_rows = a->a_rows;  p.a_rows_out = a->a_rows_out;
     if (a->idx && !a->cnt) return MPNN_E_ARG;
 #if defined(__HIP_DEVICE_COMPILE__)
     if (a->cnt) { const int c = *a->cnt; p.n = c < a->n ? c : a->n; }
diff --git a/multipath-nn_amd/csrc/conv_kernel.h b/multipath-nn_amd/csrc/conv_kernel.h
--- a/multipath-nn_amd/csrc/conv_kernel.h
+++ b/multipath-nn_amd/csrc/conv_kernel.h
@@ -27,6 +27,8 @@
     const int *idx;
     int acc_out;
     int xcd;
+    const float *a_rows;  float *a_rows_out;
+    const float *pbn_rows, *ga_rows;
 };
 
 template <int GK>
@@ -401,7 +403,7 @@
     bool tab_late = false;
     if constexpr (EPI == EPI_FWD) {
         const int tot = p.a.nslot * 2 * p.a.C;
-        tab_late = p.a.mode == MPNN_ACT_BN_BATCH && tot <= TABQ * 256 && p.a.C <= 256;
+        tab_late = p.a.mode == MPNN_ACT_BN_BATCH && tot <= TABQ * 256 && p.a.C <= 256 && !p.a_rows;
         if (tab_late) {
 #pragma unroll
             for (int j = 0; j < TABQ; ++j) { const int k = tid + 256 * j; tabq[j] = p.a.sum[k < tot ? k : 0]; }
@@ -409,15 +411,24 @@
             tab_g = p.a.gamma[c]; tab_b = p.a.beta[c];
         }
     }
+    const bool rows_w = EPI == EPI_FWD && p.a_rows_out && p.a.mode == MPNN_ACT_BN_BATCH && bx == 0 && by == 0 && kg == 0;
+    if (EPI == EPI_FWD && p.a.mode == MPNN_ACT_BN_BATCH && p.a_rows) {
+        for (int c = tid; c < p.a.C; c += 256) {
+            const f32x4 r = rows_load(p.a_rows, c);
+            cA[c * 3] = r[0]; cA[c * 3 + 1] = r[2]; cA[c * 3 + 2] = r[3];
+        }
+    } else
     if (EPI == EPI_FWD && p.a.mode != MPNN_ACT_IDENTITY && !tab_late) {
         for (int c = tid; c < p.a.C; c += 256) {
             const BnC k = bn_coef(p.a, c);
             cA[c * 3] = k.m; cA[c * 3 + 1] = k.gamma * k.rstd; cA[c * 3 + 2] = k.beta;
+            if (rows_w) rows_store(p.a_rows_out, c, k.m, k.rstd, k.gamma, k.beta);
         }
     }
     if (EPI != EPI_FWD && p.ga_on) {
         if (p.ga_bn.mode == MPNN_ACT_BN_BATCH) {
-            for (int c = tid; c < p.a.C; c += 256) bn_bwd_row(p.ga_bn, p.ga_red, p.ga_nslot, c, false, cA + c * 5);
+            if (p.ga_rows) { for (int c = tid; c < p.a.C; c += 256) bn_bwd_row_rows(p.ga_rows, p.ga_bn, p.ga_red, p.ga_nslot, c, false, cA + c * 5); }
+            else for (int c = tid; c < p.a.C; c += 256) bn_bwd_row(p.ga_bn, p.ga_red, p.ga_nslot, c, false, cA + c * 5);
         } else {
             const double inv = 1.0 / (double)p.ga_bn.cnt;
             for (int c = tid; c < p.a.C; c += 256) {
@@ -430,11 +441,18 @@
             }
         }
     }
-    if (EPI == EPI_DGH_BN || EPI == EPI_DGV) {
+    [[maybe_unused]] f32x4 rowE = {0.f, 0.f, 0.f, 0.f};
+    bool e_late = false;
+    if constexpr (EPI == EPI_DGH_BN) {
+        e_late = p.pbn.mode == MPNN_ACT_BN_BATCH && p.pbn_rows != nullptr;
+        if (e_late) { const int c = tid - 128; rowE = rows_load(p.pbn_rows, co0 + ((c >= 0 && c < CT) ? c : 0)); }
+    }
+    if ((EPI == EPI_DGH_BN || EPI == EPI_DGV) && !e_late) {
         for (int c = tid - 128; c >= 0 && c < CT; c += 256) {
             float *e = cE + c * 5;
             if (p.pbn.mode == MPNN_ACT_BN_BATCH) {
-                bn_bwd_row(p.pbn, EPI == EPI_DGV ? p.red : nullptr, p.red_nslot, co0 + c, EPI == EPI_DGH_BN, e);
+                if (EPI == EPI_DGV && p.pbn_rows) bn_bwd_row_rows(p.pbn_rows, p.pbn, p.red, p.red_nslot, co0 + c, false, e);
+                else bn_bwd_row(p.pbn, EPI == EPI_DGV ? p.red : nullptr, p.red_nslot, co0 + c, EPI == EPI_DGH_BN, e);
                 continue;
             }
             const BnC k = bn_coef(p.pbn, co0 + c);
@@ -448,7 +466,7 @@
             }
         }
     }
-    if (!tab_late) __syncthreads();
+    if (!tab_late && !(e_late && !p.ga_on)) __syncthreads();
     trace_stamp(1);
     gen_tile(gen, sq0);
     cu = gen;
@@ -471,9 +489,17 @@
                 const double inv = 1.0 / (double)p.a.cnt, mean = s1 * inv;
                 double var = s2 * inv - mean * mean;
                 var = var < 0.0 ? 0.0 : var;
-                cA[tid * 3] = (float)mean; cA[tid * 3 + 1] = tab_g * rsqrtf((float)var + p.a.eps); cA[tid * 3 + 2] = tab_b;
+                const float rstd = rsqrtf((float)var + p.a.eps);
+                cA[tid * 3] = (float)mean; cA[tid * 3 + 1] = tab_g * rstd; cA[tid * 3 + 2] = tab_b;
+                if (rows_w) rows_store(p.a_rows_out, tid, (float)mean, rstd, tab_g, tab_b);
             }
             __syncthreads();
+        }
+    }
+    if constexpr (EPI == EPI_DGH_BN) {
+        if (e_late) {
+            const int c = tid - 128;
+            if (c >= 0 && c < CT) { float *e = cE + c * 5; e[0] = rowE[0]; e[1] = rowE[1]; e[2] = rowE[2]; e[3] = rowE[3]; e[4] = 0.f; }
         }
     }
     if constexpr (XItems<GK>::INTERIOR)
diff --git a/multipath-nn_amd/csrc/conv_strip.h b/multipath-nn_amd/csrc/conv_strip.h
--- a/multipath-nn_amd/csrc/conv_strip.h
+++ b/multipath-nn_amd/csrc/conv_strip.h
@@ -17,9 +17,13 @@
     float *cS = (float *)smem;
     const int mode = a.a.mode;
     if (mode != MPNN_ACT_IDENTITY) {
-        if (tid < 16) {
+        if (tid < 16 && mode == MPNN_ACT_BN_BATCH && a.a_rows) {
+            const f32x4 r = rows_load(a.a_rows, tid);
+            cS[tid * 3] = r[0]; cS[tid * 3 + 1] = r[2]; cS[tid * 3 + 2] = r[3];
+        } else if (tid < 16) {
             const BnC k = bn_coef(a.a, tid);
             cS[tid * 3] = k.m; cS[tid * 3 + 1] = k.gamma * k.rstd; cS[tid * 3 + 2] = k.beta;
+            if (mode == MPNN_ACT_BN_BATCH && a.a_rows_out && bx == 0 && by == 0) rows_store(a.a_rows_out, tid, k.m, k.rstd, k.gamma, k.beta);
         }
         __syncthreads();
     }
@@ -176,9 +180,14 @@
     float *cS = (float *)(smem + 2048);
     f32x4 *wl = (f32x4 *)(smem + 2048 + 1024);
     const int mode = a.a.mode;
+    if (!SMA && mode == MPNN_ACT_BN_BATCH && a.a_rows && tid < Ca) {
+        const f32x4 r = rows_load(a.a_rows, tid);
+        cS[tid] = r[0]; cS[Ca + tid] = r[2]; cS[2 * Ca + tid] = r[3];
+    } else
     if (!SMA && mode != MPNN_ACT_IDENTITY && tid < Ca) {
         const BnC k = bn_coef(a.a, tid);
         cS[tid] = k.m; cS[Ca + tid] = k.gamma * k.rstd; cS[2 * Ca + tid] = k.beta;
+        if (mode == MPNN_ACT_BN_BATCH && a.a_rows_out && bx == 0 && by == 0) rows_store(a.a_rows_out, tid, k.m, k.rstd, k.gamma, k.beta);
     }
     for (int f = tid; f < K * 9 * 64; f += 256) {
         const int l = f & 63, ft = f >> 6, kq = ft / 9, t = ft - kq * 9, fl = l & 15, fg = l >> 4;
diff --git a/multipath-nn_amd/csrc/lin.hip b/multipath-nn_amd/csrc/lin.hip
--- a/multipath-nn_amd/csrc/lin.hip
+++ b/multipath-nn_amd/csrc/lin.hip
@@ -16,10 +16,17 @@
     const int wid = __builtin_amdgcn_readfirstlane(tid >> 6);
     const int C = a.a.C, K = a.HW * C;
     const bool bn = a.a.mode != MPNN_ACT_IDENTITY;
-    if (bn) {
+    if (bn && a.a_rows && a.a.mode == MPNN_ACT_BN_BATCH) {
+        for (int c = tid; c < C; c += NT_) {
+            const f32x4 r = rows_load(a.a_rows, c);
+            cA[c * 3] = r[0]; cA[c * 3 + 1] = r[2]; cA[c * 3 + 2] = r[3];
+        }
+    } else if (bn) {
+        const bool rows_w = a.a_rows_out && a.a.mode == MPNN_ACT_BN_BATCH && blockIdx.x == 0 && slice == 0;
         for (int c = tid; c < C; c += NT_) {
             const BnC k = bn_coef(a.a, c);
             cA[c * 3] = k.m; cA[c * 3 + 1] = k.gamma * k.rstd; cA[c * 3 + 2] = k.beta;
+            if (rows_w) rows_store(a.a_rows_out, c, k.m, k.rstd, k.gamma, k.beta);
         }
     }
     __syncthreads();
@@ -217,6 +224,8 @@
     load_super(r_lo);
     if (tid < 64) {
         f32x4 cf = {0.f, 1.f, 0.f, 0.f};
+        if (bn && k0 + tid < K && a.a_rows && a.a.mode == MPNN_ACT_BN_BATCH) { const f32x4 r = rows_load(a.a_rows, (k0 + tid) % C); cf[0] = r[0]; cf[1] = r[2]; cf[2] = r[3]; cf[3] = r[1]; }
+        else
         if (bn && k0 + tid < K) { const BnC c = bn_coef(a.a, (k0 + tid) % C); cf[0] = c.m; cf[1] = c.gamma * c.rstd; cf[2] = c.beta; cf[3] = c.rstd; }
         ((f32x4 *)coef)[tid] = cf;
     }
diff --git a/multipath-nn_amd/csrc/wgrad.hip b/multipath-nn_amd/csrc/wgrad.hip
--- a/multipath-nn_amd/csrc/wgrad.hip
+++ b/multipath-nn_amd/csrc/wgrad.hip
@@ -94,6 +94,7 @@
     p.c.n = a->n;  p.c.H = a->H;  p.c.W = a->W;  p.c.Cout = a->Cout;
     p.g = a->g;  p.dwa = a->dwa;  p.dwv = a->dwv;  p.db = a->db;
     p.split_stride = a->split_stride;  p.n_tiles = tiles;
+    p.c.a_rows = a->a.mode == MPNN_ACT_BN_BATCH ? a->a_rows : nullptr;
     if (a->g_ctx) {
         if (!a->g_ctx->s || !a->g_ctx->red) return MPNN_E_ARG;
         p.g_on = 1;  p.g_s = a->g_ctx->s;  p.g_bn = a->g_ctx->bn;  p.g_red = a->g_ctx->red;
diff --git a/multipath-nn_amd/lib/_eng_alloc.py b/multipath-nn_amd/lib/_eng_alloc.py
--- a/multipath-nn_amd/lib/_eng_alloc.py
+++ b/multipath-nn_amd/lib/_eng_alloc.py
@@ -284,12 +284,14 @@
             p._on_assign = self.invalidate_packs
         self._packs_fresh = False
         self.seg = torch.tensor(seg, dtype=torch.int32, device=dev)
-        doff, tab = 0, []
+        doff, roff, tab = 0, 0, []
         for b in self.blocks:
-            b.sum_off = []
+            b.sum_off, b.rows_off = [], []
             for i in range(b.L):
                 bn = b.bns[i].params
                 b.sum_off.append(doff)
+                b.rows_off.append(roff)
+                roff += 4 * b.C[i]
                 tab += [doff, bn.m_avg.offset, bn.v_avg.offset, b.C[i], b.H[i] * b.W[i],
                         bn.γ.offset if b.has_dz[i] else -1, bn.β.offset, self._nslot(b, i)]
                 doff += 2 * b.C[i] * _hip.BN_SLOTS
@@ -300,6 +302,7 @@
         z64 = self._zarena[:zb].view(torch.float64)
         self.dsum, self.dred, self.loss = z64[:nd], z64[nd:2 * nd], z64[2 * nd:2 * nd + 4]
         self.dsum_last = torch.zeros(nd, dtype=torch.float64, device=dev)
+        self.bn_rows_buf = torch.zeros(max(roff, 4), dtype=torch.float32, device=dev)
         n_g = self.G.numel()
         self.G = self._zarena[zb:zb + n_g * 4].view(torch.float32)
         self.node_stat = self.G[:n_stat]
@@ -434,6 +437,15 @@
                     nslot=self._nslot(b, i))
 
 
+    def _rows_ptr(self, b, i):
+        return self.bn_rows_buf[b.rows_off[i]:].data_ptr()
+
+
+    def _rows_of(self, b, i):
+        written = getattr(self, '_rows_written', None)
+        return self._rows_ptr(b, i) if written is not None and (id(b), i) in written else None
+
+
     def _act_of_input(self, b, i, n, mode, fwd=False):
         if b.in_map is None:
             if fwd and getattr(self, 'rgbx_probe', False) and b.in_shift[i] > 0:
@@ -449,5 +461,6 @@
         ctx.bn = _hip.act(None, b.C[i], _hip.ACT_BN_BATCH, 0, self._bn(b, i), n * b.H[i] * b.W[i])
         ctx.red = self.dred[b.sum_off[i]:].data_ptr() if with_red else None
         ctx.red_nslot = self._nslot(b, i)
+        ctx.rows = self._rows_of(b, i)
         self._keep.append(ctx)
         return ctx
diff --git a/multipath-nn_amd/lib/_eng_ksteps.py b/multipath-nn_amd/lib/_eng_ksteps.py
--- a/multipath-nn_amd/lib/_eng_ksteps.py
+++ b/multipath-nn_amd/lib/_eng_ksteps.py
@@ -41,7 +41,7 @@
         if not ok:
             return one_by_one()
         n = int(xs[0].shape[0])
-        key = ('trK', n, K, self.bwd_levels, self.fold_clear, self.fuse_opt, self.co_share, dp)
+        key = ('trK', n, K, self.bwd_levels, self.fold_clear, self.fuse_opt, self.co_share, dp, self.bn_rows)
         g = self._graphs.get(key)
         if g is None:
             one_by_one()
diff --git a/multipath-nn_amd/lib/_eng_planner.py b/multipath-nn_amd/lib/_eng_planner.py
--- a/multipath-nn_amd/lib/_eng_planner.py
+++ b/multipath-nn_amd/lib/_eng_planner.py
@@ -204,7 +204,8 @@
             raise NotImplementedError('data-parallel training runs on the single-stream schedule (MPNN_STREAMS=0)')
         dp = mode == 'tr' and self.allreduce is not None
         reserve = self.dp_reserve_cus if (dp and len(self.dp_buckets) > 1) else 0
-        key = (mode, n, self.multi_stream, self.group_fwd, routed, dp, self.bwd_levels, self.fold_clear, reserve, self.fuse_opt, self.co_share)
+        key = (mode, n, self.multi_stream, self.group_fwd, routed, dp, self.bwd_levels, self.fold_clear, reserve, self.fuse_opt, self.co_share,
+               self.bn_rows)
         if key in self._progs:
             return self._progs[key]
         self._ensure_capacity(n, mode == 'tr')
@@ -218,7 +219,10 @@
         if self.multi_stream and any(len(b.children) > 1 for b in self.blocks):
             raise NotImplementedError('the multi-stream schedule serialises nothing between sibling blocks that '
                                       'accumulate into one gradient map: tree nets run on the single-stream schedule')
-        prog = self._progs[key] = self._program_tr(n, dp, reserve)
+        try:
+            prog = self._progs[key] = self._program_tr(n, dp, reserve)
+        finally:
+            self._rows_written = None
         return prog
 
 
@@ -227,8 +231,10 @@
         sid = {h: (0 if h == sizes[-1] else 1 + k) for k, h in enumerate(sizes)}
         self.n_streams = len(sizes) + 2
         fwd = [Launch(None, 'fork')]
-        if self.group_fwd and not self.multi_stream and self._groupable() and \
-                all(b.parent is not None or b.in_map is None for b in self.blocks):
+        wavefront = self.group_fwd and not self.multi_stream and self._groupable() and \
+            all(b.parent is not None or b.in_map is None for b in self.blocks)
+        self._rows_written = set() if (self.bn_rows and wavefront and not dp) else None
+        if wavefront:
             for members in self._wavefront(self.blocks):
                 fwd += self._conv_fwd_launches(members, n, 'tr')
         else:
@@ -270,6 +276,14 @@
         a.n, a.H, a.W, a.Cout = n, b.H[i], b.W[i], b.C[i]
         if rows is not None:
             a.idx, a.cnt = rows[0].data_ptr(), rows[1].data_ptr()
+        pend = getattr(self, '_rows_pending', None)
+        if train and pend is not None and b.in_map is not None:
+            key = (id(b.parent), b.in_map[i])
+            if key in self._rows_written:
+                a.a_rows = self._rows_ptr(b.parent, b.in_map[i])
+            elif key not in pend:
+                a.a_rows_out = self._rows_ptr(b.parent, b.in_map[i])
+                pend.add(key)
         return a
 
 
@@ -310,7 +324,11 @@
             return [self._conv_fwd_single(b, i, n, mode, rows(b), 'fwd') for b, i in members]
         for c0 in range(0, len(members), 4):
             grp = members[c0:c0 + 4]
+            self._rows_pending = set() if (mode == 'tr' and getattr(self, '_rows_written', None) is not None) else None
             arr = (_hip.ConvFwdArgs * len(grp))(*[self._conv_fwd_args(b, i, n, mode, rows(b)) for b, i in grp])
+            if self._rows_pending:
+                self._rows_written |= self._rows_pending
+            self._rows_pending = None
             dev_arr = _hip.to_device_table(list(arr), self.dev)
             self._keep += [arr, dev_arr]
             fl, tag = sum(self._conv_flops(b, i, n) for b, i in grp), ' | '.join(self._conv_tag(b, i) for b, i in grp)
@@ -352,6 +370,13 @@
             tf, tb = _hip.ExitTailArgs(), _hip.ExitTailBwdArgs()
             a_in = _hip.act(b.s[L1], b.C[L1], act_mode, 0, self._bn(b, L1), n * b.H[L1] * b.W[L1])
             lf.a, lb.a = a_in, a_in
+            if getattr(self, '_rows_written', None) is not None and not self.generic_exits:
+                if (id(b), L1) in self._rows_written:
+                    lf.a_rows = self._rows_ptr(b, L1)
+                else:
+                    lf.a_rows_out = self._rows_ptr(b, L1)
+                    self._rows_written.add((id(b), L1))
+                lb.a_rows = self._rows_ptr(b, L1)
             lf.HW = lb.HW = b.H[L1] * b.W[L1]
             lf.n = lb.n = tf.n = n
             lf.k_cpt = lb.k_cpt = self.k_cpt.data_ptr()
@@ -538,6 +563,8 @@
                 nonlocal slab_size
                 a = _hip.WgradArgs()
                 a.a = self._act_of_input(b, i, n, _hip.ACT_BN_BATCH)
+                if b.in_map is not None:
+                    a.a_rows = self._rows_of(b.parent, b.in_map[i])
                 pa = getattr(cp, 'w_horz_%i' % i)
                 pv = getattr(cp, 'w_vert_%i' % (i - 1)) if i > 0 else None
                 pb = getattr(cp, 'b_%i' % i)
diff --git a/multipath-nn_amd/lib/_eng_run.py b/multipath-nn_amd/lib/_eng_run.py
--- a/multipath-nn_amd/lib/_eng_run.py
+++ b/multipath-nn_amd/lib/_eng_run.py
@@ -359,7 +359,7 @@
 
     def _run_graphed(self, prog, train, n):
         key = (prog['mode'], n, train, prog.get('routed', False), self.bwd_levels, self.fold_clear,
-               self.allreduce is not None, self._bucket_opt_on())
+               self.allreduce is not None, self._bucket_opt_on(), self.bn_rows)
         g = self._graphs.get(key)
         if g is None:
             self._step_eager(prog, train, n)
diff --git a/multipath-nn_amd/lib/_hip.py b/multipath-nn_amd/lib/_hip.py
--- a/multipath-nn_amd/lib/_hip.py
+++ b/multipath-nn_amd/lib/_hip.py
@@ -34,11 +34,11 @@
 class ConvFwdArgs(C.Structure):
     _fields_ = [('a', Act), ('v', P), ('Cv', C.c_int), ('wa_pack', P), ('wv_pack', P), ('bias', P),
                 ('out', P), ('pool_out', P), ('out_sum', P), ('out_nslot', C.c_int), ('n', C.c_int), ('H', C.c_int), ('W', C.c_int),
-                ('Cout', C.c_int), ('idx', P), ('cnt', P)]
+                ('Cout', C.c_int), ('idx', P), ('cnt', P), ('a_rows', P), ('a_rows_out', P)]
 
 
 class BnCtx(C.Structure):
-    _fields_ = [('s', P), ('bn', Act), ('red', P), ('red_nslot', C.c_int)]
+    _fields_ = [('s', P), ('bn', Act), ('red', P), ('red_nslot', C.c_int), ('rows', P)]
 
 
 class DgradHorzArgs(C.Structure):
@@ -57,7 +57,8 @@
 class WgradArgs(C.Structure):
     _fields_ = [('a', Act), ('v', P), ('Cv', C.c_int), ('g', P), ('g_ctx', C.POINTER(BnCtx)), ('dwa', P), ('dwv', P),
                 ('db', P),
-                ('split_stride', C.c_long), ('n', C.c_int), ('H', C.c_int), ('W', C.c_int), ('Cout', C.c_int), ('n_split', C.c_int)]
+                ('split_stride', C.c_long), ('n', C.c_int), ('H', C.c_int), ('W', C.c_int), ('Cout', C.c_int), ('n_split', C.c_int),
+                ('a_rows', P)]
 
 
 BWD_LEVEL_MAX = 4
@@ -71,14 +72,15 @@
 class LinFwdArgs(C.Structure):
     _fields_ = [('a', Act), ('HW', C.c_int), ('w', P * 2), ('b', P * 2), ('y', P * 2), ('M', C.c_int * 2),
                 ('k_cpt', P), ('alpha_cpt', C.c_float), ('extra_col', C.c_int * 2), ('n', C.c_int),
-                ('kpart', P), ('kcnt', P)]
+                ('kpart', P), ('kcnt', P), ('a_rows', P), ('a_rows_out', P)]
 
 
 class LinBwdArgs(C.Structure):
     _fields_ = [('a', Act), ('HW', C.c_int), ('w', P * 2), ('dy', P * 2), ('M', C.c_int * 2),
                 ('dw', P * 2), ('db', P * 2), ('dx', P), ('k_cpt', P), ('alpha_cpt', C.c_float),
                 ('extra_col', C.c_int * 2), ('n', C.c_int),
-                ('dz_out', P), ('red_out', P), ('red_nslot', C.c_int), ('kpart', P), ('kcnt', P)]
+                ('dz_out', P), ('red_out', P), ('red_nslot', C.c_int), ('kpart', P), ('kcnt', P),
+                ('a_rows', P)]
 
 
 class ExitTailArgs(C.Structure):
diff --git a/multipath-nn_amd/lib/_plan.py b/multipath-nn_amd/lib/_plan.py
--- a/multipath-nn_amd/lib/_plan.py
+++ b/multipath-nn_amd/lib/_plan.py
@@ -33,6 +33,7 @@
         self.routed_min_batch = 512
         self.routed_min_batch_gen = 512
         self.fold_clear = bool(int(os.environ.get('MPNN_FOLD_CLEAR', '1')))
+        self.bn_rows = bool(int(os.environ.get('MPNN_BN_ROWS', '1')))
         self._acc_clean = False
         self._streams = []
         self._event_keep = []
```
